# AbeelLab/phasm

Measured on AMD Instinct MI355X. Metric: overlaps_per_sec, higher is better.
Workload: dtype u64

## Files before the change

include/phasm_overlap.h:

```cpp
#ifndef PHASM_OVERLAP_H
#define PHASM_OVERLAP_H

#include <stddef.h>
#include <stdint.h>

#ifdef __cplusplus
extern "C" {
#endif

#define PO_ABI_VERSION 4

typedef enum {
    PO_OK = 0,
    PO_ERR_INVALID = 1,
    PO_ERR_NOMEM = 2,
    PO_ERR_HIP = 3,
    PO_ERR_CAPACITY = 4
} po_status;

typedef struct po_handle po_handle;
typedef struct po_result po_result;

typedef struct {
    uint32_t a_idx, b_idx;
// ... 192 lines not shown

typedef struct {
    uint64_t n_edges_in;
    uint64_t n_edges_out;
    uint64_t n_nodes;
    uint64_t n_nodes_removed;
    uint64_t n_candidates;
    uint64_t n_diamonds;
    uint64_t n_rounds;
    uint64_t n_invalid;
    float ms_setup, ms_rounds, ms_emit, ms_total;
} po_diamond_stats;

po_status po_layout_diamonds(po_handle* h, po_result* edges, const po_diamond_params* params, uint8_t* edge_flags_out,
                             po_result** kept_out);
po_status po_get_diamond_stats(const po_handle* h, po_diamond_stats* out);


typedef struct {
    uint32_t reserved;
} po_merge_params;

typedef struct {
    uint64_t n_edges_in;
    uint64_t n_edges_out;
    uint64_t n_nodes;
    uint64_t n_merged;
    uint64_t n_nodes_merged;
    uint64_t max_path_nodes;
    uint64_t n_self_loops;
    uint64_t n_cycle_nodes;
    uint64_t n_rounds;
    uint64_t n_overflow;
    uint64_t n_invalid;
    float ms_links, ms_rank, ms_number, ms_emit, ms_total;
} po_merge_stats;

po_status po_layout_merge(po_handle* h, po_result* edges, const po_merge_params* params, uint8_t* edge_flags_out,
                          po_result** merged_out);
po_status po_get_merge_stats(const po_handle* h, po_merge_stats* out);

po_status po_result_merged_paths(po_result* merged, uint64_t* n_paths, uint64_t* n_members, uint64_t* offsets_out,
                                 uint64_t cap_paths, uint32_t* members_out, int32_t* prefix_out, uint64_t cap_members,
                                 int64_t* lengths_out);


typedef struct {
    uint32_t reserved;
} po_coverage_params;

typedef struct {
    uint64_t read_length_sum;
    int64_t path_length;
} po_edge_coverage;

typedef struct {
    uint64_t n_rows, n_edges;
    uint64_t n_nodes;
    uint64_t n_pairs;
    uint64_t max_set;
    uint64_t n_zero_path;
    uint64_t n_invalid;
    float ms_sets, ms_edges, ms_total;
} po_coverage_stats;

po_status po_layout_coverage(po_handle* h, po_result* graph, po_result* rows, const po_coverage_params* params,
                             po_edge_coverage* coverage_out );
po_status po_get_coverage_stats(const po_handle* h, po_coverage_stats* out);


typedef struct {
    uint32_t reserved;
} po_components_params;

typedef struct {
    uint32_t first_node;
    uint32_t n_nodes;
    uint64_t n_edges;
} po_component;

typedef struct {
    uint64_t n_nodes;
    uint64_t n_edges;
    uint64_t n_components;
    uint64_t n_singletons;
    uint64_t max_component_nodes, max_component_edges;
    uint64_t n_invalid;
    uint32_t n_rounds;
    uint32_t n_batches;
    float ms_rounds, ms_label, ms_total;
} po_components_stats;

po_status po_layout_components(po_handle* h, po_result* graph, const po_components_params* params,
                               uint32_t* node_component_out, uint32_t* edge_component_out, po_component* components_out,
                               uint64_t* n_components_out);
po_status po_get_components_stats(const po_handle* h, po_components_stats* out);


typedef struct {
    uint32_t reserved;
} po_partition_params;

typedef struct {
    uint32_t first_node;
    uint32_t n_nodes;
    uint64_t n_edges;
    uint32_t n_r_in;
    uint32_t n_re_out;
} po_scc;

#define PO_PART_R_IN 1u
#define PO_PART_RE_OUT 2u
#define PO_PART_START 4u
#define PO_PART_SINK 8u

typedef struct {
    uint64_t n_nodes;
    uint64_t n_edges;
    uint64_t n_sccs, n_nonsingleton_sccs, n_singletons;
    uint64_t n_self_loops;
    uint64_t max_scc_nodes, max_scc_edges;
    uint64_t n_trimmed;
    uint64_t n_class[5];
    uint64_t n_invalid;
    uint32_t n_outer;
    uint32_t n_trim_rounds, n_forward_rounds, n_backward_rounds;
    uint32_t n_batches;
    float ms_ranks, ms_rounds, ms_label, ms_total;
} po_partition_stats;

po_status po_layout_partition(po_handle* h, po_result* graph, const po_partition_params* params, uint32_t* node_scc_out,
                              uint8_t* node_flags_out, uint8_t* edge_class_out, po_scc* sccs_out, uint64_t* n_sccs_out);
po_status po_get_partition_stats(const po_handle* h, po_partition_stats* out);

po_status po_graph_from_edges(po_handle* h, const po_edge* edges, uint64_t n_edges, const uint32_t* node_order,
                              uint64_t n_order, po_result** out);

po_status po_result_node_order(po_result* r, uint32_t* nodes_out, uint64_t cap, uint64_t* n_out);

typedef struct {
    uint64_t n_rows;
    float ms_first_contained;
    float ms_rank;
    float ms_total;
} po_node_order_stats;
po_status po_get_node_order_stats(const po_handle* h, po_node_order_stats* out);

uint64_t po_debug_host_ranges(uint64_t* out, uint64_t cap_entries);
uint64_t po_debug_store_words(const po_handle* h, int store, const uint64_t** words);
int po_debug_expand_records(const po_cand* records, uint64_t n, const uint32_t* lengths, uint32_t n_reads, uint32_t paired,
                            po_row* rows_out, uint64_t n_rows_expected);
int po_debug_expand_packed(const uint64_t* records, uint64_t n, uint32_t sh_b, uint32_t sh_p, const uint32_t* lengths, uint32_t n_reads,
                           uint32_t paired, po_row* rows_out, uint64_t n_rows_expected);
int po_debug_fault_backtrace(int fd);
int po_debug_pointer_info(const void* p, int32_t* hip_type, int32_t* hsa_type, uint64_t* base, uint64_t* bytes);

po_status po_get_stats(const po_handle* h, po_stats* out);
const char* po_last_error(const po_handle* h);
int po_abi_version(void);

#ifdef __cplusplus
}
#endif
#endif
```

phasm_amd/_lib.py:

```python
from __future__ import annotations

import ctypes
import os

import numpy as np

HERE = os.path.dirname(os.path.abspath(__file__))
LIB_PATH = os.environ.get("PHASM_LIB") or os.path.join(HERE, "libphasm_overlap.so")

PO_OK, PO_ERR_INVALID, PO_ERR_NOMEM, PO_ERR_HIP, PO_ERR_CAPACITY = range(5)

ROW_DTYPE = np.dtype([("a_idx", "<u4"), ("b_idx", "<u4"), ("astart", "<i4"),
                      ("aend", "<i4"), ("bstart", "<i4"), ("bend", "<i4")])


CAND_DTYPE = np.dtype([("a_idx", "<u4"), ("p", "<u4"), ("b_idx", "<u4"), ("type", "<u4")])


EDGE_DTYPE = np.dtype([("u", "<u4"), ("v", "<u4"), ("weight", "<i4"), ("overlap_len", "<i4")])
COVERAGE_DTYPE = np.dtype([("read_length_sum", "<u8"), ("path_length", "<i8")])
COMPONENT_DTYPE = np.dtype([("first_node", "<u4"), ("n_nodes", "<u4"), ("n_edges", "<u8")])
SCC_DTYPE = np.dtype([("first_node", "<u4"), ("n_nodes", "<u4"), ("n_edges", "<u8"), ("n_r_in", "<u4"), ("n_re_out", "<u4")])
PART_R_IN, PART_RE_OUT, PART_START, PART_SINK = 1, 2, 4, 8

# ... 85 lines not shown
    _fields_ = [("n_rows", ctypes.c_uint64), ("n_edges", ctypes.c_uint64), ("n_nodes", ctypes.c_uint64), ("n_pairs", ctypes.c_uint64),
                ("max_set", ctypes.c_uint64), ("n_zero_path", ctypes.c_uint64), ("n_invalid", ctypes.c_uint64),
                ("ms_sets", ctypes.c_float), ("ms_edges", ctypes.c_float), ("ms_total", ctypes.c_float)]

    def as_dict(self) -> dict:
        return {name: getattr(self, name) for name, _ in self._fields_}


class PoComponentsParams(ctypes.Structure):
    _fields_ = [("reserved", ctypes.c_uint32)]


class PoComponentsStats(ctypes.Structure):
    _fields_ = [("n_nodes", ctypes.c_uint64), ("n_edges", ctypes.c_uint64), ("n_components", ctypes.c_uint64),
                ("n_singletons", ctypes.c_uint64), ("max_component_nodes", ctypes.c_uint64), ("max_component_edges", ctypes.c_uint64),
                ("n_invalid", ctypes.c_uint64), ("n_rounds", ctypes.c_uint32), ("n_batches", ctypes.c_uint32),
                ("ms_rounds", ctypes.c_float), ("ms_label", ctypes.c_float), ("ms_total", ctypes.c_float)]

    def as_dict(self) -> dict:
        return {name: getattr(self, name) for name, _ in self._fields_}


class PoPartitionParams(ctypes.Structure):
    _fields_ = [("reserved", ctypes.c_uint32)]


class PoPartitionStats(ctypes.Structure):
    _fields_ = [("n_nodes", ctypes.c_uint64), ("n_edges", ctypes.c_uint64), ("n_sccs", ctypes.c_uint64),
                ("n_nonsingleton_sccs", ctypes.c_uint64), ("n_singletons", ctypes.c_uint64), ("n_self_loops", ctypes.c_uint64),
                ("max_scc_nodes", ctypes.c_uint64), ("max_scc_edges", ctypes.c_uint64), ("n_trimmed", ctypes.c_uint64),
                ("n_class", ctypes.c_uint64 * 5), ("n_invalid", ctypes.c_uint64), ("n_outer", ctypes.c_uint32),
                ("n_trim_rounds", ctypes.c_uint32), ("n_forward_rounds", ctypes.c_uint32), ("n_backward_rounds", ctypes.c_uint32),
                ("n_batches", ctypes.c_uint32),
                ("ms_ranks", ctypes.c_float), ("ms_rounds", ctypes.c_float), ("ms_label", ctypes.c_float), ("ms_total", ctypes.c_float)]

    def as_dict(self) -> dict:
        d = {name: getattr(self, name) for name, _ in self._fields_}
        d["n_class"] = list(self.n_class)
        return d


class PoNodeOrderStats(ctypes.Structure):
    _fields_ = [("n_rows", ctypes.c_uint64), ("ms_first_contained", ctypes.c_float), ("ms_rank", ctypes.c_float),
                ("ms_total", ctypes.c_float)]

    def as_dict(self) -> dict:
        return {name: getattr(self, name) for name, _ in self._fields_}


class PoStats(ctypes.Structure):
    _fields_ = [
        ("bits_per_base", ctypes.c_uint32), ("kmer", ctypes.c_uint32),
        ("paired", ctypes.c_uint32), ("wide_index", ctypes.c_uint32),
        ("n_reads", ctypes.c_uint64), ("n_eligible", ctypes.c_uint64),
        ("total_bases", ctypes.c_uint64), ("shard_bases", ctypes.c_uint64),
        ("n_tiles", ctypes.c_uint64), ("n_candidates", ctypes.c_uint64),
        ("n_verified", ctypes.c_uint64), ("n_rows", ctypes.c_uint64),
        ("sum_overlap_bases", ctypes.c_uint64), ("verify_bytes_algo", ctypes.c_uint64),
        ("ms_index", ctypes.c_float), ("ms_scan_count", ctypes.c_float),
        ("ms_scan_fill", ctypes.c_float), ("ms_verify", ctypes.c_float),
        ("ms_select", ctypes.c_float), ("ms_emit", ctypes.c_float),
        ("ms_total", ctypes.c_float), ("ms_upload", ctypes.c_float),
        ("ms_scan_probe", ctypes.c_float), ("ms_verify_kernel", ctypes.c_float),
        ("verify_bytes_exec", ctypes.c_uint64), ("dp_steps", ctypes.c_uint64), ("dp_stopped", ctypes.c_uint64),
        ("max_diff", ctypes.c_uint32), ("band", ctypes.c_uint32), ("index_reused", ctypes.c_uint32),
        ("dp_lanes", ctypes.c_uint32), ("upload_bytes", ctypes.c_uint64),
        ("streamed", ctypes.c_uint32), ("n_deferred", ctypes.c_uint32),
        ("fused_tail", ctypes.c_uint32), ("tail_fallback", ctypes.c_uint32),
        ("n_predicted", ctypes.c_uint32), ("home_record_bytes", ctypes.c_uint32),
    ]

    def as_dict(self) -> dict:
        return {name: getattr(self, name) for name, _ in self._fields_}


_P = ctypes.c_void_p
SYMBOLS = [
    ("po_abi_version", ctypes.c_int, []),
    ("po_create", ctypes.c_int, [ctypes.POINTER(_P)]),
    ("po_destroy", None, [_P]),
    ("po_set_device", ctypes.c_int, [_P, ctypes.c_int]),
    ("po_add_sequence", ctypes.c_int, [_P, ctypes.c_char_p, ctypes.c_size_t, ctypes.c_char_p, ctypes.c_size_t]),
    ("po_add_fasta", ctypes.c_int, [_P, ctypes.c_char_p, ctypes.c_int, ctypes.POINTER(ctypes.c_uint64)]),
    ("po_num_sequences", ctypes.c_uint32, [_P]),
    ("po_get_id", ctypes.c_int, [_P, ctypes.c_uint32, ctypes.POINTER(ctypes.c_void_p), ctypes.POINTER(ctypes.c_size_t)]),
    ("po_get_length", ctypes.c_uint32, [_P, ctypes.c_uint32]),
    ("po_upload", ctypes.c_int, [_P]),
    ("po_invalidate", ctypes.c_int, [_P]),
    ("po_upload_piece", ctypes.c_int, [_P, ctypes.c_uint32, ctypes.c_uint32, ctypes.c_void_p, ctypes.c_uint64,
                                       ctypes.POINTER(ctypes.c_uint64), ctypes.POINTER(ctypes.c_int)]),
    ("po_upload_assemble", ctypes.c_int, [_P, ctypes.c_void_p, ctypes.c_uint64, ctypes.c_uint32]),
    ("po_upload_piece_part", ctypes.c_int, [_P, ctypes.c_uint32, ctypes.c_uint32, ctypes.c_uint32, ctypes.c_uint32, ctypes.c_void_p,
                                            ctypes.c_uint64, ctypes.POINTER(ctypes.c_uint64), ctypes.POINTER(ctypes.c_int)]),
    ("po_upload_assemble_parts", ctypes.c_int, [_P, ctypes.c_void_p, ctypes.c_uint64, ctypes.c_uint32, ctypes.c_uint32]),
    ("po_overlaps", ctypes.c_int, [_P, ctypes.c_uint32, ctypes.POINTER(_P)]),
    ("po_overlaps_to_host", ctypes.c_int, [_P, ctypes.c_uint32, ctypes.POINTER(_P)]),
    ("po_overlaps_ex", ctypes.c_int, [_P, ctypes.c_uint32, ctypes.c_uint32, ctypes.c_uint32, ctypes.POINTER(_P)]),
    ("po_overlaps_shard", ctypes.c_int, [_P, ctypes.c_uint32, ctypes.c_uint32, ctypes.c_uint32, ctypes.POINTER(_P)]),
    ("po_candidates_shard", ctypes.c_int, [_P, ctypes.c_uint32, ctypes.c_uint32, ctypes.c_uint32, ctypes.POINTER(_P)]),
    ("po_expand", ctypes.c_int, [_P, ctypes.c_void_p, ctypes.c_uint64, ctypes.POINTER(_P)]),
    ("po_candidates_shard_into", ctypes.c_int, [_P, ctypes.c_uint32, ctypes.c_uint32, ctypes.c_uint32, ctypes.c_void_p,
                                               ctypes.c_uint64, ctypes.POINTER(ctypes.c_int), ctypes.POINTER(_P)]),
    ("po_index_slice_build", ctypes.c_int, [_P, ctypes.c_uint32, ctypes.c_uint32, ctypes.c_uint32, ctypes.POINTER(ctypes.c_uint32),
                                            ctypes.POINTER(ctypes.c_uint32), ctypes.POINTER(ctypes.c_uint64)]),
    ("po_index_chunk_bytes", ctypes.c_uint64, [ctypes.c_uint32, ctypes.c_uint64, ctypes.POINTER(ctypes.c_uint64)]),
    ("po_index_slice_export", ctypes.c_int, [_P, ctypes.c_void_p, ctypes.c_uint64]),
    ("po_candidates_shard_indexed", ctypes.c_int, [_P, ctypes.c_uint32, ctypes.c_uint32, ctypes.c_uint32, ctypes.c_void_p, ctypes.c_uint32,
                                                   ctypes.c_uint32, ctypes.c_uint64, ctypes.c_void_p, ctypes.c_uint64,
                                                   ctypes.POINTER(ctypes.c_int), ctypes.POINTER(_P)]),
    ("po_overlaps_shard_indexed", ctypes.c_int, [_P, ctypes.c_uint32, ctypes.c_uint32, ctypes.c_uint32, ctypes.c_void_p, ctypes.c_uint32,
                                                 ctypes.c_uint32, ctypes.c_uint64, ctypes.POINTER(_P)]),
    ("po_shard_range", ctypes.c_int, [_P, ctypes.c_uint32, ctypes.c_uint32, ctypes.POINTER(ctypes.c_uint32), ctypes.POINTER(ctypes.c_uint32)]),
    ("po_result_count", ctypes.c_uint64, [_P]),
    ("po_result_rows", ctypes.c_void_p, [_P]),
    ("po_result_rows_range", ctypes.c_void_p, [_P, ctypes.c_uint64, ctypes.c_uint64]),
    ("po_result_device_rows", ctypes.c_void_p, [_P]),
    ("po_result_copy_to_device", ctypes.c_int, [_P, ctypes.c_void_p]),
    ("po_result_copy_prefix_to_device", ctypes.c_int, [_P, ctypes.c_void_p, ctypes.c_uint64]),
    ("po_result_free", None, [_P]),
    ("po_write_gfa_edges", ctypes.c_int, [_P, ctypes.c_int, ctypes.POINTER(ctypes.c_uint64)]),
    ("po_write_gfa_segments", ctypes.c_int, [_P, ctypes.c_int, ctypes.POINTER(ctypes.c_uint64)]),
    ("po_add_segment", ctypes.c_int, [_P, ctypes.c_char_p, ctypes.c_size_t, ctypes.c_uint32]),
    ("po_result_from_rows", ctypes.c_int, [_P, ctypes.c_void_p, ctypes.c_uint64, ctypes.POINTER(_P)]),
    ("po_add_gfa", ctypes.c_int, [_P, ctypes.c_char_p, ctypes.POINTER(ctypes.c_uint64), ctypes.POINTER(_P)]),
    ("po_layout_edges", ctypes.c_int, [_P, _P, ctypes.POINTER(PoLayoutParams), ctypes.c_void_p, ctypes.POINTER(_P)]),
    ("po_get_layout_stats", ctypes.c_int, [_P, ctypes.POINTER(PoLayoutStats)]),
    ("po_layout_reduce", ctypes.c_int, [_P, _P, ctypes.POINTER(PoReduceParams), ctypes.c_void_p, ctypes.POINTER(_P)]),
    ("po_get_reduce_stats", ctypes.c_int, [_P, ctypes.POINTER(PoReduceStats)]),
    ("po_layout_tips", ctypes.c_int, [_P, _P, ctypes.POINTER(PoTipsParams), ctypes.c_void_p, ctypes.POINTER(_P)]),
    ("po_get_tips_stats", ctypes.c_int, [_P, ctypes.POINTER(PoTipsStats)]),
    ("po_layout_diamonds", ctypes.c_int, [_P, _P, ctypes.POINTER(PoDiamondParams), ctypes.c_void_p, ctypes.POINTER(_P)]),
    ("po_get_diamond_stats", ctypes.c_int, [_P, ctypes.POINTER(PoDiamondStats)]),
    ("po_layout_merge", ctypes.c_int, [_P, _P, ctypes.POINTER(PoMergeParams), ctypes.c_void_p, ctypes.POINTER(_P)]),
    ("po_get_merge_stats", ctypes.c_int, [_P, ctypes.POINTER(PoMergeStats)]),
    ("po_result_merged_paths", ctypes.c_int, [_P, ctypes.POINTER(ctypes.c_uint64), ctypes.POINTER(ctypes.c_uint64), ctypes.c_void_p,
                                              ctypes.c_uint64, ctypes.c_void_p, ctypes.c_void_p, ctypes.c_uint64, ctypes.c_void_p]),
    ("po_layout_coverage", ctypes.c_int, [_P, _P, _P, ctypes.POINTER(PoCoverageParams), ctypes.c_void_p]),
    ("po_get_coverage_stats", ctypes.c_int, [_P, ctypes.POINTER(PoCoverageStats)]),
    ("po_layout_components", ctypes.c_int, [_P, _P, ctypes.POINTER(PoComponentsParams), ctypes.c_void_p, ctypes.c_void_p, ctypes.c_void_p,
                                            ctypes.POINTER(ctypes.c_uint64)]),
    ("po_get_components_stats", ctypes.c_int, [_P, ctypes.POINTER(PoComponentsStats)]),
    ("po_layout_partition", ctypes.c_int, [_P, _P, ctypes.POINTER(PoPartitionParams), ctypes.c_void_p, ctypes.c_void_p, ctypes.c_void_p,
                                           ctypes.c_void_p, ctypes.POINTER(ctypes.c_uint64)]),
    ("po_get_partition_stats", ctypes.c_int, [_P, ctypes.POINTER(PoPartitionStats)]),
    ("po_graph_from_edges", ctypes.c_int, [_P, ctypes.c_void_p, ctypes.c_uint64, ctypes.c_void_p, ctypes.c_uint64, ctypes.POINTER(_P)]),
    ("po_result_node_order", ctypes.c_int, [_P, ctypes.c_void_p, ctypes.c_uint64, ctypes.POINTER(ctypes.c_uint64)]),
    ("po_get_node_order_stats", ctypes.c_int, [_P, ctypes.POINTER(PoNodeOrderStats)]),
    ("po_get_stats", ctypes.c_int, [_P, ctypes.POINTER(PoStats)]),
    ("po_last_error", ctypes.c_char_p, [_P]),
    ("po_debug_fault_backtrace", ctypes.c_int, [ctypes.c_int]),
    ("po_debug_store_words", ctypes.c_uint64, [_P, ctypes.c_int, ctypes.POINTER(ctypes.c_void_p)]),
    ("po_debug_expand_packed", ctypes.c_int, [ctypes.c_void_p, ctypes.c_uint64, ctypes.c_uint32, ctypes.c_uint32, ctypes.c_void_p, ctypes.c_uint32,
                                              ctypes.c_uint32, ctypes.c_void_p, ctypes.c_uint64]),
    ("po_debug_expand_records", ctypes.c_int, [ctypes.c_void_p, ctypes.c_uint64, ctypes.c_void_p, ctypes.c_uint32, ctypes.c_uint32,
                                               ctypes.c_void_p, ctypes.c_uint64]),
    ("po_debug_host_ranges", ctypes.c_uint64, [ctypes.POINTER(ctypes.c_uint64), ctypes.c_uint64]),
    ("po_debug_pointer_info", ctypes.c_int, [ctypes.c_void_p, ctypes.POINTER(ctypes.c_int32), ctypes.POINTER(ctypes.c_int32),
                                             ctypes.POINTER(ctypes.c_uint64), ctypes.POINTER(ctypes.c_uint64)]),
]

_lib = None


def _preload_torch_hip_runtime() -> None:
    import importlib.util
    if os.environ.get("PHASM_HIP_RUNTIME") == "system":
        return
    try:
        spec = importlib.util.find_spec("torch")
    except (ImportError, ValueError):
        spec = None
    if spec is None or not spec.submodule_search_locations:
        return
    path = os.path.join(list(spec.submodule_search_locations)[0], "lib", "libamdhip64.so")
    if os.path.exists(path):
        try:
            ctypes.CDLL(path, mode=ctypes.RTLD_GLOBAL)
        except OSError:
            pass


def load() -> ctypes.CDLL:
    global _lib
    if _lib is None:
        _preload_torch_hip_runtime()
        if not os.path.exists(LIB_PATH):
            raise ImportError(
                "%s not found: build it with `python -m phasm_amd.build` (hipcc, gfx950). "
                "phasm_amd has no CPU fallback." % LIB_PATH)
        lib = ctypes.CDLL(LIB_PATH)
        for name, restype, argtypes in SYMBOLS:
            fn = getattr(lib, name)
            fn.restype = restype
            fn.argtypes = argtypes
        _lib = lib
    return _lib
```

phasm_amd/csrc/c_api.hip:

```cpp
#include "../../include/phasm_overlap.h"

#include <hip/hip_runtime.h>

#include <dlfcn.h>
#include <execinfo.h>
#include <fcntl.h>
#include <signal.h>
#include <sys/mman.h>
#include <sys/stat.h>
#include <unistd.h>

#include <algorithm>
#include <array>
#include <atomic>
#include <chrono>
#include <cmath>
#include <condition_variable>
#include <cstdio>
#include <cstdlib>
#include <cstring>
#include <deque>
#include <functional>
#include <memory>
#include <mutex>
#include <new>
#include <string>
#include <system_error>
#include <thread>
#include <unordered_map>
#include <vector>

#include "kernels.hip.h"
#include "extend.hip.h"
#include "layout.hip.h"
#include "reduce.hip.h"
#include "tips.hip.h"
#include "diamond.hip.h"
#include "merge.hip.h"
#include "coverage.hip.h"
#include "components.hip.h"
#include "partition.hip.h"

namespace {

enum { RB_CNT, RB_DEG, RB_OFF, RB_CUR, RB_TKEY, RB_TTGT, RB_TEID, RB_CTGT, RB_CW, RB_CEID, RB_CIDPOS, RB_STGT, RB_SEID, RB_STATE,
       RB_FLAG1, RB_FLAGS, RB_KEEP, RB_KOFF, RB_N };
enum { TB_CNT, TB_OUTDEG, TB_OUTSUM, TB_INDEG, TB_INSUM, TB_MARK, TB_CAND, TB_CSTATE, TB_EFLAG, TB_FLAGS, TB_KEEP, TB_KOFF,
       TB_TKEY, TB_TVAL, TB_ALIVE, TB_RCNT, TB_N };
enum { MB_CNT, MB_RCNT, MB_OUTDEG, MB_INDEG, MB_OUTE, MB_INE, MB_LINK, MB_BACK, MB_JB0, MB_JB1, MB_HOPS0, MB_HOPS1, MB_WS0, MB_WS1,
       MB_HKEY, MB_HVAL, MB_HLEN, MB_HSUM, MB_PATHK, MB_LENS, MB_PSUM, MB_NPATH, MB_NPOS, MB_EFLAG, MB_KEEP, MB_KOFF, MB_TMP, MB_LEN,
       MB_N };
enum { VB_CNT, VB_USED, VB_NODEOF, VB_LEN, VB_TABLE, VB_SUM, VB_SETCNT, VB_OFF, VB_CUR, VB_LIST, VB_OUT, VB_N };
enum { RK_CNT, RK_RCNT, RK_KEY, RK_VAL, RK_RANKOF, RK_ENDS, RK_ROOT, RK_INDEX, RK_N };
enum { KB_P, KB_COMP, KB_ECOMP, KB_TABLE, KB_N };
enum { PB_LIVE, PB_SCC, PB_COLOUR, PB_MARK, PB_HASIN, PB_HASOUT, PB_NODESCC, PB_FLAGW, PB_FLAGS, PB_ECLASS, PB_TABLE, PB_N };
constexpr int EV_LAY_N = 38;
enum { EV_EDGES = 0, EV_REDUCE = 4, EV_TIPS = 9, EV_NODE_ORDER = 15, EV_DIAMONDS = 18, EV_MERGE = 22, EV_COVERAGE = 27, EV_COMPONENTS = 30,
       EV_PARTITION = 34 };
static_assert(EV_PARTITION + 4 == EV_LAY_N, "the four events of po_layout_partition are the last of the layout events");
constexpr int TIP_BATCH = 24;

struct DevBuf {
    void* p = nullptr;
    size_t cap = 0;
    bool arena = false;
    template <typename T> T* as() const { return static_cast<T*>(p); }
    void release() {
        if (p && !arena) (void)hipFree(p);
        p = nullptr;
        cap = 0;
        arena = false;
    }
};

struct PinNote {
    uint64_t base, bytes;
    uint32_t kind;
};
std::mutex g_pin_mu;
std::vector<PinNote> g_pins;
uint64_t g_pins_ever = 0;
constexpr size_t PIN_LOG_MAX = 1u << 16;
void pin_note(const void* p, size_t bytes, uint32_t kind) {
    if (!p) return;
    std::lock_guard<std::mutex> lock(g_pin_mu);
    ++g_pins_ever;
    for (PinNote& n : g_pins)
        if (n.base == (uint64_t)(uintptr_t)p && n.bytes == bytes && (n.kind & 0xFFu) == kind) {
            n.kind |= 0x100u;
            return;
        }
    if (g_pins.size() < PIN_LOG_MAX) g_pins.push_back(PinNote{(uint64_t)(uintptr_t)p, (uint64_t)bytes, kind | 0x100u});
}
void pin_drop(const void* p) {
    if (!p) return;
    std::lock_guard<std::mutex> lock(g_pin_mu);
    for (PinNote& n : g_pins)
        if (n.base == (uint64_t)(uintptr_t)p && (n.kind & 0x100u)) n.kind &= ~0x100u;
}

struct HostBuf {
    void* p = nullptr;
    size_t cap = 0;
    void release() {
        if (p) {
            pin_drop(p);
            (void)hipHostFree(p);
        }
        p = nullptr;
        cap = 0;
    }
};

inline int phase_events_env() {
    if (const char* e = getenv("PHASM_PHASE_EVENTS")) {
        const int v = atoi(e);
        return v == 1 ? 1 : v == 2 ? 2 : 0;
    }
    return getenv("PHASM_STREAM_TRACE") ? 1 : -1;
}
enum { EV_START = 0, EV_INDEX, EV_COUNT, EV_FILL, EV_VERIFY, EV_SELECT, EV_EMIT, EV_PROBE0, EV_PROBE1, EV_VER0, EV_VER1, EV_DONE, EV_N };

}

constexpr int PO_MAX_PIECES = 16;

struct RegHeader {
    size_t bytes;
    int registered;
};
constexpr size_t REG_PAGE = 4096;
thread_local bool g_reg_defer = false;
template <class T>
struct RegAlloc {
    using value_type = T;
    RegAlloc() = default;
    template <class U> RegAlloc(const RegAlloc<U>&) {}
    T* allocate(size_t n) {
        const size_t bytes = ((n * sizeof(T) + REG_PAGE - 1) / REG_PAGE) * REG_PAGE;
        void* base = nullptr;
        if (posix_memalign(&base, REG_PAGE, bytes + REG_PAGE) != 0 || !base) throw std::bad_alloc();
        RegHeader* hd = static_cast<RegHeader*>(base);
        hd->bytes = bytes;
        hd->registered = 0;
        char* data = static_cast<char*>(base) + REG_PAGE;
        if (getenv("PHASM_POISON_HOST")) std::memset(data, 0xA5, bytes);
        if (!g_reg_defer) reg_now(data);
        return reinterpret_cast<T*>(data);
    }
    static void reg_now(void* data) {
        RegHeader* hd = reinterpret_cast<RegHeader*>(static_cast<char*>(data) - REG_PAGE);
        if (hd->registered || hd->bytes < (1u << 20) || getenv("PHASM_NO_PIN")) return;
        if (hipHostRegister(data, hd->bytes, hipHostRegisterPortable) == hipSuccess) {
            hd->registered = 1;
            pin_note(data, hd->bytes, 2u);
        } else {
            (void)hipGetLastError();
        }
    }
    template <class U> void construct(U*) noexcept {}
    template <class U, class A0, class... Args> void construct(U* q, A0&& a0, Args&&... args) {
        ::new (static_cast<void*>(q)) U(std::forward<A0>(a0), std::forward<Args>(args)...);
    }
    void deallocate(T* p, size_t) {
        char* base = reinterpret_cast<char*>(p) - REG_PAGE;
        RegHeader* hd = reinterpret_cast<RegHeader*>(base);
        if (hd->registered) {
            pin_drop(p);
            (void)hipHostUnregister(p);
        }
        free(base);
    }
    template <class U> bool operator==(const RegAlloc<U>&) const { return true; }
    template <class U> bool operator!=(const RegAlloc<U>&) const { return false; }
};
using WordStore = std::vector<uint64_t, RegAlloc<uint64_t>>;
inline bool store_is_pinned(const WordStore& w) {
    if (w.capacity() == 0) return false;
    const RegHeader* hd = reinterpret_cast<const RegHeader*>(reinterpret_cast<const char*>(w.data()) - REG_PAGE);
    return hd->registered != 0;
}
constexpr size_t STAGE_MAX = 4u << 20;

struct po_handle {
    int device = 0;
// ... 251 lines not shown
        return fail(h, PO_ERR_NOMEM, "hipMalloc(" + std::to_string(want) + " bytes): " + hipGetErrorString(e));
    }
    b.cap = want;
    if (h && h->poison >= 0 && h->stream) (void)hipMemsetAsync(b.p, h->poison, want, h->stream);
    return PO_OK;
}

po_status ensure_piece(po_handle* h, DevBuf& b, size_t bytes) { return ensure(h, b, bytes, h->ws_scale); }

po_status ensure_host(po_handle* h, HostBuf& b, size_t bytes) {
    if (bytes <= b.cap) return PO_OK;
    AllocTrace tr("hipHostMalloc", bytes);
    b.release();
    const size_t want = bytes + bytes / 16 + 4096;
    hipError_t e = hipHostMalloc(&b.p, want, hipHostMallocDefault);
    if (e != hipSuccess) {
        b.p = nullptr;
        return fail(h, PO_ERR_NOMEM, "hipHostMalloc(" + std::to_string(want) + " bytes): " + hipGetErrorString(e));
    }
    b.cap = want;
    pin_note(b.p, want, 1u);
    return PO_OK;
}

void quiesce_store(po_handle* h) {
    if (!h->dev_ready) return;
    (void)hipSetDevice(h->device);
    (void)hipStreamSynchronize(h->stream);
    if (h->up_stream) (void)hipStreamSynchronize(h->up_stream);
    if (h->rc_stream) (void)hipStreamSynchronize(h->rc_stream);
}

po_status init_device(po_handle* h);

inline bool home_enabled() {
    const char* e = getenv("PHASM_HOME");
    return !(e && atoi(e) == 0);
}

void result_pool_grow(po_handle* h, uint64_t bases = 0) {
    if (!bases) bases = h->total_bases;
    h->pool_bases = bases + bases / 2;
    if (getenv("PHASM_NO_POOL")) return;
    if (!h->dev_ready && init_device(h) != PO_OK) h->err.clear();
    const uint64_t want = std::min<uint64_t>(h->pool_bases / 160 * sizeof(po_row), 4ull << 30);
    if (h->spare_host.cap >= want || h->live_results) return;
    int n = 0;
    if (hipGetDeviceCount(&n) != hipSuccess || n == 0) {
        (void)hipGetLastError();
        h->pool_bases = ~0ull;
        return;
    }
    AllocTrace tr("result pool", want);
    h->spare_host.release();
    if (hipHostMalloc(&h->spare_host.p, want, hipHostMallocPortable) == hipSuccess) {
        h->spare_host.cap = want;
        pin_note(h->spare_host.p, want, 1u);
        if (home_enabled() && h->home_stage.cap < want / 3) (void)ensure_host(h, h->home_stage, want / 3);
        if (h->dev_ready && h->up_stream && h->copy_stream && want >= (16u << 20) && !getenv("PHASM_NO_WARM")) {
            void* w = nullptr;
            const size_t nb = 8u << 20;
            if (hipMalloc(&w, nb) == hipSuccess) {
                (void)hipMemcpyAsync(w, h->spare_host.p, nb, hipMemcpyHostToDevice, h->up_stream);
                (void)hipStreamSynchronize(h->up_stream);
                (void)hipMemcpyAsync(static_cast<char*>(h->spare_host.p) + nb, w, nb, hipMemcpyDeviceToHost, h->copy_stream);
                (void)hipStreamSynchronize(h->copy_stream);
                (void)hipFree(w);
            }
            (void)hipGetLastError();
        }
    } else {
        (void)hipGetLastError();
        h->spare_host.p = nullptr;
        h->pool_bases = ~0ull;
    }
}

#define PO_TRY(expr)                    \
    do {                                \
        po_status s_ = (expr);          \
        if (s_ != PO_OK) return s_;     \
    } while (0)

struct DevKit {
    int device = -1;
    hipStream_t stream = nullptr, copy_stream = nullptr, up_stream = nullptr, rc_stream = nullptr;
    hipEvent_t ev_sets[2][EV_N] = {};
    hipEvent_t ev_up0 = nullptr, ev_up1 = nullptr, ev_meta = nullptr, ev_first = nullptr;
    hipEvent_t ev_piece[PO_MAX_PIECES] = {}, ev_rc[PO_MAX_PIECES] = {}, ev_lay[EV_LAY_N] = {};

    uint64_t* pinned = nullptr;
    uint64_t* pinned_dev = nullptr;
};
static_assert(sizeof(DevKit::ev_lay) == sizeof(po_handle::ev_lay), "a kit carries every layout event of a handle");
std::mutex g_kit_mu;
std::vector<DevKit> g_kits;
constexpr size_t KIT_POOL_MAX = 8;

bool kit_take(po_handle* h) {
    std::lock_guard<std::mutex> lock(g_kit_mu);
    for (size_t i = 0; i < g_kits.size(); ++i) {
        if (g_kits[i].device != h->device) continue;
        const DevKit k = g_kits[i];
        g_kits.erase(g_kits.begin() + (long)i);
        h->stream = k.stream;
        h->copy_stream = k.copy_stream;
        h->up_stream = k.up_stream;
        h->rc_stream = k.rc_stream;
        std::memcpy(h->ev_sets, k.ev_sets, sizeof(k.ev_sets));
        h->ev_up0 = k.ev_up0;
        h->ev_up1 = k.ev_up1;
        h->ev_meta = k.ev_meta;
        h->ev_first = k.ev_first;
        std::memcpy(h->ev_piece, k.ev_piece, sizeof(k.ev_piece));
        std::memcpy(h->ev_rc, k.ev_rc, sizeof(k.ev_rc));
        std::memcpy(h->ev_lay, k.ev_lay, sizeof(k.ev_lay));
        h->pinned = k.pinned;
        h->pinned_dev = k.pinned_dev;
        return true;
    }
    return false;
}

bool kit_give(po_handle* h) {
    if (getenv("PHASM_NO_KIT_POOL") || !h->stream || !h->copy_stream || !h->up_stream || !h->rc_stream || !h->pinned) return false;
    if (hipStreamSynchronize(h->stream) != hipSuccess || hipStreamSynchronize(h->copy_stream) != hipSuccess ||
        hipStreamSynchronize(h->up_stream) != hipSuccess || hipStreamSynchronize(h->rc_stream) != hipSuccess) {
        (void)hipGetLastError();
        return false;
    }
    DevKit k;
    k.device = h->device;
    k.stream = h->stream;
    k.copy_stream = h->copy_stream;
    k.up_stream = h->up_stream;
    k.rc_stream = h->rc_stream;
    std::memcpy(k.ev_sets, h->ev_sets, sizeof(k.ev_sets));
    k.ev_up0 = h->ev_up0;
    k.ev_up1 = h->ev_up1;
    k.ev_meta = h->ev_meta;
    k.ev_first = h->ev_first;
    std::memcpy(k.ev_piece, h->ev_piece, sizeof(k.ev_piece));
    std::memcpy(k.ev_rc, h->ev_rc, sizeof(k.ev_rc));
    std::memcpy(k.ev_lay, h->ev_lay, sizeof(k.ev_lay));
    k.pinned = h->pinned;
    k.pinned_dev = h->pinned_dev;
    std::lock_guard<std::mutex> lock(g_kit_mu);
    if (g_kits.size() >= KIT_POOL_MAX) return false;
    g_kits.push_back(k);
    return true;
}


unsigned cpu_share() {
    static const unsigned share = [] {
        unsigned n = std::thread::hardware_concurrency();
        n = n ? n : 4u;
        long long q = -1, per = 100000;
        if (FILE* f = std::fopen("/sys/fs/cgroup/cpu.max", "r")) {
            char buf[64] = {0};
            if (std::fscanf(f, "%63s %lld", buf, &per) >= 1 && std::strcmp(buf, "max") != 0) q = atoll(buf);
            std::fclose(f);
        } else if (FILE* g = std::fopen("/sys/fs/cgroup/cpu/cpu.cfs_quota_us", "r")) {
            if (std::fscanf(g, "%lld", &q) != 1) q = -1;
            std::fclose(g);
            if (FILE* g2 = std::fopen("/sys/fs/cgroup/cpu/cpu.cfs_period_us", "r")) {
                if (std::fscanf(g2, "%lld", &per) != 1) per = 100000;
                std::fclose(g2);
            }
        }
        if (q > 0 && per > 0) n = std::min<unsigned>(n, (unsigned)std::max<long long>(1, q / per));
        return n;
    }();
    return share;
}

namespace home {

constexpr uint32_t CHUNK = 4096;

struct Job {
    const void* rec = nullptr;
    uint32_t sh_b = 0, sh_p = 0;
    uint64_t n_rec = 0;
    po_row* out = nullptr;
    uint64_t n_rows = 0;
    const volatile uint32_t* flag = nullptr;
    uint32_t want = 0;
    uint32_t paired = 0, bits = 2;
};

struct Pool {
    std::vector<std::thread> thr;
    std::mutex mu;
    std::condition_variable cv_queue;
    std::condition_variable cv_job;
    std::mutex call_mu;
    std::deque<Job> queue;
    std::atomic<uint64_t> submitted{0}, finished{0};
    std::atomic<int> error{0};
    const uint32_t* len = nullptr;
    uint32_t n_reads = 0;
    std::atomic<uint64_t> sum_l{0}, sum_b{0}, sum_e{0};
    Job cur;
    uint64_t job_seq = 0;
    uint32_t n_chunks = 0;
    std::vector<uint64_t> chunk_off;
    std::atomic<uint32_t> next_count{0}, done_count{0}, next_write{0}, done_write{0};
    std::atomic<int> phase{0};
    std::atomic<int> inside{0};
    std::chrono::steady_clock::time_point t0;
    std::vector<std::array<double, 3>> trace;
    bool tracing = false;
};

Pool* g_pool = nullptr;
std::once_flag g_pool_once;

inline void cpu_pause() {
#if defined(__x86_64__) || defined(__i386__)
    __builtin_ia32_pause();
#endif
}

std::atomic<uint32_t> g_spin_limit{4096};
template <class Pred>
inline void spin_until(Pred pred) {
    const uint32_t limit = g_spin_limit.load(std::memory_order_relaxed);
    for (uint32_t n = 0; !pred(); ++n) {
        if (limit == 0 || n < limit) cpu_pause();
        else std::this_thread::yield();
    }
}

inline po::Cand load_rec(const Job& j, uint64_t i) {
    if (!j.sh_b) return static_cast<const po::Cand*>(j.rec)[i];
    return po::unpack_record(static_cast<const uint64_t*>(j.rec)[i], j.sh_b, j.sh_p);
}

inline uint32_t rows_of_rec(const po::Cand& c, uint32_t paired) {
    if (!paired) return (c.type & 1u) + ((c.type >> 1) & 1u);
    return ((c.type & 1u) ? (c.a == (c.b ^ 1u) ? 1u : 2u) : 0u) + ((c.type & 2u) ? 2u : 0u);
}

inline void put_row(uint64_t*& o, uint32_t a, uint32_t b, uint32_t astart, uint32_t aend, uint32_t bend) {
    __builtin_nontemporal_store((uint64_t)a | ((uint64_t)b << 32), o);
    __builtin_nontemporal_store((uint64_t)astart | ((uint64_t)aend << 32), o + 1);
    __builtin_nontemporal_store((uint64_t)bend << 32, o + 2);
    o += 3;
}

bool expand_records(Pool& P, uint64_t lo, uint64_t hi, po_row* out) {
    uint64_t* o = reinterpret_cast<uint64_t*>(out);
    const Job& job = P.cur;
    const uint32_t* len = P.len;
    const uint32_t paired = job.paired, n_reads = P.n_reads, bits = job.bits;
    auto pb = [bits](uint32_t l) -> uint64_t { return bits == 8u ? l : (l >> 2) + ((l & 3u) != 0u); };
    uint64_t sl = 0, sb = 0, se = 0;
    for (uint64_t i = lo; i < hi; ++i) {
        const po::Cand c = load_rec(job, i);
        if (c.a >= n_reads || c.b >= n_reads) return false;
        const uint32_t la = len[c.a], lb = len[c.b];
        se += 2 * pb((c.type & 1u) ? la - c.p : lb);
        if (c.type & 1u) {
            const uint32_t l = la - c.p;
            const bool twin = paired && c.a != (c.b ^ 1u);
            put_row(o, c.a, c.b, c.p, la, l);
            if (twin) put_row(o, c.b ^ 1u, c.a ^ 1u, lb - l, lb, l);
            const uint64_t k = twin ? 2 : 1;
            sl += k * l;
            sb += k * 2 * pb(l);
        }
        if (c.type & 2u) {
            put_row(o, c.a, c.b, c.p, c.p + lb, lb);
            if (paired) put_row(o, c.a ^ 1u, c.b ^ 1u, la - c.p - lb, la - c.p, lb);
            const uint64_t k = paired ? 2 : 1;
            sl += k * lb;
            sb += k * 2 * pb(lb);
        }
    }
    P.sum_l.fetch_add(sl, std::memory_order_relaxed);
    P.sum_b.fetch_add(sb, std::memory_order_relaxed);
    P.sum_e.fetch_add(se, std::memory_order_relaxed);
    return true;
}

void run_phases(Pool& P, bool lead) {
    const uint32_t nc = P.n_chunks;
    for (;;) {
        const uint32_t c = P.next_count.fetch_add(1, std::memory_order_relaxed);
        if (c >= nc) break;
        const uint64_t lo = (uint64_t)c * CHUNK, hi = std::min<uint64_t>(P.cur.n_rec, lo + CHUNK);
        uint64_t n = 0;
        const uint32_t paired = P.cur.paired;
        for (uint64_t i = lo; i < hi; ++i) n += rows_of_rec(load_rec(P.cur, i), paired);
        P.chunk_off[c + 1] = n;
        P.done_count.fetch_add(1, std::memory_order_release);
    }
    if (lead) {
        spin_until([&] { return P.done_count.load(std::memory_order_acquire) >= nc; });
        P.chunk_off[0] = 0;
        for (uint32_t c = 0; c < nc; ++c) P.chunk_off[c + 1] += P.chunk_off[c];
        if (P.chunk_off[nc] != P.cur.n_rows) P.error.store(1);
        P.phase.store(P.error.load() ? 0 : 2, std::memory_order_release);
    } else {
        spin_until([&] { return P.phase.load(std::memory_order_acquire) != 1; });
    }
    if (P.phase.load(std::memory_order_acquire) != 2) return;
    for (;;) {
        const uint32_t c = P.next_write.fetch_add(1, std::memory_order_relaxed);
        if (c >= nc) break;
        const uint64_t lo = (uint64_t)c * CHUNK, hi = std::min<uint64_t>(P.cur.n_rec, lo + CHUNK);
        if (!expand_records(P, lo, hi, P.cur.out + P.chunk_off[c])) P.error.store(2);
#if defined(__x86_64__)
        __builtin_ia32_sfence();
#endif
        P.done_write.fetch_add(1, std::memory_order_release);
    }
}

void helper(Pool* Pp) {
    Pool& P = *Pp;
    uint64_t seen = 0;
    for (;;) {
        {
            std::unique_lock<std::mutex> lock(P.mu);
            P.cv_job.wait(lock, [&] { return P.job_seq != seen; });
            seen = P.job_seq;
        }
        P.inside.fetch_add(1, std::memory_order_acq_rel);
        if (P.phase.load(std::memory_order_acquire) != 0) run_phases(P, false);
        P.inside.fetch_sub(1, std::memory_order_release);
    }
}

void leader(Pool* Pp) {
    Pool& P = *Pp;
    for (;;) {
        Job j;
        {
            std::unique_lock<std::mutex> lock(P.mu);
            P.cv_queue.wait(lock, [&] { return !P.queue.empty(); });
            j = P.queue.front();
            P.queue.pop_front();
        }
        if (j.flag)
            spin_until([&] { return *j.flag == j.want; });
        std::atomic_thread_fence(std::memory_order_acquire);
        const double t_ready = P.tracing ? std::chrono::duration<double, std::micro>(std::chrono::steady_clock::now() - P.t0).count() : 0.0;
        if (P.error.load() == 0 && j.n_rec) {
            spin_until([&] { return P.inside.load(std::memory_order_acquire) == 0; });
            P.cur = j;
            P.n_chunks = (uint32_t)((j.n_rec + CHUNK - 1) / CHUNK);
            if (P.chunk_off.size() < (size_t)P.n_chunks + 1) P.chunk_off.resize((size_t)P.n_chunks + 1);
            P.next_count.store(0);
            P.done_count.store(0);
            P.next_write.store(0);
            P.done_write.store(0);
            P.phase.store(1, std::memory_order_release);
            {
                std::lock_guard<std::mutex> lock(P.mu);
                ++P.job_seq;
            }
            P.cv_job.notify_all();
            run_phases(P, true);
            if (P.phase.load() == 2)
                spin_until([&] { return P.done_write.load(std::memory_order_acquire) >= P.n_chunks; });
            P.phase.store(0, std::memory_order_release);
            std::atomic_thread_fence(std::memory_order_seq_cst);
        }
        if (P.tracing)
            P.trace.push_back({t_ready, std::chrono::duration<double, std::micro>(std::chrono::steady_clock::now() - P.t0).count(), (double)j.n_rows});
        P.finished.fetch_add(1, std::memory_order_release);
    }
}

Pool* pool() {
    std::call_once(g_pool_once, [] {
        Pool* P = new Pool();
        unsigned n = cpu_share();
        n = std::max(1u, std::min(n * 3 / 4, 12u));
        if (const char* e = getenv("PHASM_HOME_THREADS")) n = (unsigned)std::max(1, std::min(64, atoi(e)));
        try {
            P->thr.emplace_back(leader, P);
            P->thr.back().detach();
            for (unsigned i = 1; i < n; ++i) {
                P->thr.emplace_back(helper, P);
                P->thr.back().detach();
            }
        } catch (const std::system_error&) {
        }
        if (P->thr.empty()) {
            delete P;
            P = nullptr;
        }
        g_pool = P;
    });
    return g_pool;
}

void begin(Pool* P, const uint32_t* len, uint32_t n_reads, bool tracing) {
    if (const char* e = getenv("PHASM_HOME_SPIN")) g_spin_limit.store((uint32_t)std::max(0, atoi(e)));
    else g_spin_limit.store(4096);
    P->len = len;
    P->n_reads = n_reads;
    P->error.store(0);
    P->submitted.store(0);
    P->finished.store(0);
    P->sum_l.store(0);
    P->sum_b.store(0);
    P->sum_e.store(0);
    P->tracing = tracing;
    P->trace.clear();
    P->t0 = std::chrono::steady_clock::now();
}

void submit(Pool* P, const Job& j) {
    {
        std::lock_guard<std::mutex> lock(P->mu);
        P->queue.push_back(j);
    }
    P->submitted.fetch_add(1, std::memory_order_release);
    P->cv_queue.notify_one();
}

void wait_all(Pool* P) {
    spin_until([&] { return P->finished.load(std::memory_order_acquire) >= P->submitted.load(std::memory_order_acquire); });
}

}

po_status init_device(po_handle* h) {
    if (h->dev_ready) {
        HIP_TRY(h, hipSetDevice(h->device));
        return PO_OK;
    }
    AllocTrace tr("init_device", 0);
    const auto ti0 = std::chrono::steady_clock::now();
    auto imark = [&](const char* what) {
        if (tr.on) std::fprintf(stderr, "[init] %s at %.1f ms\n", what, std::chrono::duration<double, std::milli>(std::chrono::steady_clock::now() - ti0).count());
    };
    int n = 0;
    hipError_t e = hipGetDeviceCount(&n);
    imark("runtime up (hipGetDeviceCount)");
    if (e != hipSuccess || n == 0)
        return fail(h, PO_ERR_HIP, "no HIP device available (libphasm_overlap has no CPU fallback)");
    if (h->device < 0 || h->device >= n) return fail(h, PO_ERR_INVALID, "device ordinal out of range");
    HIP_TRY(h, hipSetDevice(h->device));
    hipDeviceProp_t prop;
    HIP_TRY(h, hipGetDeviceProperties(&prop, h->device));
    h->n_cu = prop.multiProcessorCount > 0 ? prop.multiProcessorCount : 256;
    h->lds_max = prop.sharedMemPerBlock;
    if (const char* e = getenv("PHASM_POISON")) h->poison = (int)(strtol(e, nullptr, 0) & 0xFF);
    if (!getenv("PHASM_NO_KIT_POOL") && kit_take(h)) {
        h->ev = h->ev_sets[0];
        std::memset(h->pinned, 0, 1024);
        hipLaunchKernelGGL(po::k_fill_u32, dim3(1), dim3(64), 0, h->stream, reinterpret_cast<uint32_t*>(h->pinned_dev + 63), (uint64_t)1, 0u);
        (void)hipGetLastError();
        h->dev_ready = true;
        return PO_OK;
    }
    imark("device selected, properties read");
    HIP_TRY(h, hipStreamCreateWithFlags(&h->stream, hipStreamNonBlocking));
    imark("first stream made");
    for (int i = 0; i < 2 * EV_N; ++i) HIP_TRY(h, hipEventCreate(&h->ev_sets[i / EV_N][i % EV_N]));
    HIP_TRY(h, hipEventCreate(&h->ev_up0));
    HIP_TRY(h, hipEventCreate(&h->ev_up1));
    imark("first events made");
    HIP_TRY(h, hipHostMalloc(reinterpret_cast<void**>(&h->pinned), 1024, hipHostMallocDefault));
    pin_note(h->pinned, 1024, 1u);
    HIP_TRY(h, hipHostGetDevicePointer(reinterpret_cast<void**>(&h->pinned_dev), h->pinned, 0));
    imark("landing zone made");
    if (const char* e = getenv("PHASM_POISON")) h->poison = (int)(strtol(e, nullptr, 0) & 0xFF);
    HIP_TRY(h, hipStreamCreateWithFlags(&h->copy_stream, hipStreamNonBlocking));
    imark("copy stream made");
    HIP_TRY(h, hipStreamCreateWithFlags(&h->up_stream, hipStreamNonBlocking));
    HIP_TRY(h, hipStreamCreateWithFlags(&h->rc_stream, hipStreamNonBlocking));
    imark("other streams made");
    for (int k = 0; k < PO_MAX_PIECES; ++k) {
        HIP_TRY(h, hipEventCreate(&h->ev_piece[k]));
        HIP_TRY(h, hipEventCreateWithFlags(&h->ev_rc[k], hipEventDisableTiming));
    }
    HIP_TRY(h, hipEventCreateWithFlags(&h->ev_first, hipEventDisableTiming));
    HIP_TRY(h, hipEventCreateWithFlags(&h->ev_meta, hipEventDisableTiming));
    imark("streams and events made");
    hipLaunchKernelGGL(po::k_fill_u32, dim3(1), dim3(64), 0, h->stream, reinterpret_cast<uint32_t*>(h->pinned_dev + 63), (uint64_t)1, 0u);
    (void)hipGetLastError();
    imark("first launch queued (code object loaded)");
    if (!getenv("PHASM_NO_WARM")) {
        void* w = nullptr;
        if (hipMalloc(&w, 256) == hipSuccess) {
            uint32_t* wd = static_cast<uint32_t*>(w);
            (void)hipMemcpyAsync(wd, h->pinned + 62, 8, hipMemcpyHostToDevice, h->up_stream);
            hipLaunchKernelGGL(po::k_fill_u32, dim3(1), dim3(64), 0, h->up_stream, wd + 8, (uint64_t)1, 0u);
            (void)hipMemcpyAsync(wd + 16, h->pinned + 62, 8, hipMemcpyHostToDevice, h->stream);
            hipLaunchKernelGGL(po::k_fill_u32, dim3(1), dim3(64), 0, h->rc_stream, wd + 24, (uint64_t)1, 0u);
            hipLaunchKernelGGL(po::k_fill_u32, dim3(1), dim3(64), 0, h->copy_stream, wd + 32, (uint64_t)1, 0u);
            (void)hipMemcpyAsync(h->pinned + 61, wd + 32, 8, hipMemcpyDeviceToHost, h->copy_stream);
            (void)hipMemcpyAsync(h->pinned + 60, wd + 16, 8, hipMemcpyDeviceToHost, h->stream);
            (void)hipStreamSynchronize(h->up_stream);
            (void)hipStreamSynchronize(h->rc_stream);
            (void)hipStreamSynchronize(h->copy_stream);
            (void)hipStreamSynchronize(h->stream);
            (void)hipFree(w);
        }
        (void)hipGetLastError();
        imark("queues and copy paths warmed");
        static const void* const warm_kernels[] = {
            (const void*)po::k_abs_woff, (const void*)po::k_build_tiles, (const void*)po::k_revcomp_store, (const void*)po::k_scatter_first,
            (const void*)po::k_paired_check, (const void*)po::k_call_init, (const void*)po::k_call_reset, (const void*)po::k_table_insert,
            (const void*)po::k_chain_fill, (const void*)po::k_chain_sort_short<uint32_t>, (const void*)po::k_chain_sort_long<uint32_t>,
            (const void*)po::k_table_finalize, (const void*)po::k_ps_reduce<uint32_t>, (const void*)po::k_ps_spine, (const void*)po::k_ps_down<uint32_t>,
            (const void*)po::k_ps_reduce<uint8_t>, (const void*)po::k_ps_down<uint8_t>, (const void*)po::k_ps_chain<uint32_t>,
            (const void*)po::k_ps_chain<uint8_t>, (const void*)po::k_ps_small,
            (const void*)po::k_scan_probe<2, true, true>, (const void*)po::k_scan_probe<2, true, false>, (const void*)po::k_scan_fixup<2, true>,
            (const void*)po::k_scan_fixup<2, false>, (const void*)po::k_scan_fill<2, true>, (const void*)po::k_scan_fill<2, false>,
            (const void*)po::k_read_label, (const void*)po::k_read_sort, (const void*)po::k_read_invert, (const void*)po::k_defer_split,
            (const void*)po::k_verify_a<2, false, true, true>, (const void*)po::k_verify_a<2, false, true, false>,
            (const void*)po::k_verify_a<2, true, true, false>, (const void*)po::k_select_local, (const void*)po::k_tile_rows<true>,
            (const void*)po::k_tile_rows<false>, (const void*)po::k_tail, (const void*)po::k_tail_cands, (const void*)po::k_select,
            (const void*)po::k_emit, (const void*)po::k_verify_flat, (const void*)po::k_deferred_rowcnt, (const void*)po::k_emit_cands,
            (const void*)po::k_wide_insert<2, 1>, (const void*)po::k_wide_insert<2, 16>, (const void*)po::k_wide_chain_fill<2, 1>,
            (const void*)po::k_wide_chain_fill<2, 16>, (const void*)po::k_wide_finalize<2, 1>, (const void*)po::k_wide_finalize<2, 16>,
            (const void*)po::k_chain_sort_short<uint64_t>, (const void*)po::k_chain_sort_long<uint64_t>,
            (const void*)po::k_wide_scan<2, false, true, 1>, (const void*)po::k_wide_scan<2, true, true, 1>,
            (const void*)po::k_wide_scan<2, false, false, 16>, (const void*)po::k_wide_scan<2, true, false, 16>};
        for (const void* k : warm_kernels) {
            hipFuncAttributes fa;
            (void)hipFuncGetAttributes(&fa, k);
        }
        (void)hipGetLastError();
        imark("kernels looked up");
    }
    h->dev_ready = true;
    return PO_OK;
}

struct BaseLut {
    uint8_t v[256];
    BaseLut() {
        std::memset(v, 0x80, sizeof(v));
        v[(unsigned char)'A'] = 0;
        v[(unsigned char)'C'] = 1;
        v[(unsigned char)'G'] = 2;
        v[(unsigned char)'T'] = 3;
    }
};
const BaseLut g_lut;

bool append_packed(po_handle* h, const unsigned char* s, size_t n, int bits) {
    const size_t per = 64 / bits;
    WordStore& store = h->words[h->woff.size() & 1];
    const size_t old_size = store.size();
    const size_t off = (old_size + 1) & ~size_t(1);
    const size_t nw = (n + per - 1) / per;
    store.resize(off + nw + 1, 0);
    uint64_t* w = store.data() + off;
    if (bits == 2) {
        const uint8_t* lut = g_lut.v;
        uint8_t bad = 0;
        const size_t full = n / 32;
        for (size_t k = 0; k < full; ++k) {
            const unsigned char* q = s + k * 32;
            uint64_t acc = 0;
            for (int j = 0; j < 32; ++j) {
                const uint8_t c = lut[q[j]];
                bad |= c;
                acc |= (uint64_t)(c & 3) << (2 * j);
            }
            w[k] = acc;
        }
        if (full * 32 < n) {
            uint64_t acc = 0;
            for (size_t i = full * 32; i < n; ++i) {
                const uint8_t c = lut[s[i]];
                bad |= c;
                acc |= (uint64_t)(c & 3) << (2 * (i & 31));
            }
            w[full] = acc;
        }
        if (bad & 0x80) {
            size_t cnt = 0;
            for (size_t i = 0; i < n; ++i) cnt += lut[s[i]] >> 7;
// ... 684 lines not shown
        h->sl_entries = h->pinned[0];
        if (h->phase_events) (void)hipEventElapsedTime(&S.ms_index, h->ev[EV_START], h->ev[EV_INDEX]);
        return PO_OK;
    }
    if (ext_idx) {
        WA_ext = true;
    }
    if (h->idx_only) {
        h->idx_valid = true;
        h->idx_gen = h->upload_gen;
        h->idx_m = m;
        h->idx_wide = wide;
        h->idx_tbits = tbits;
        h->idx_bits = (uint32_t)BITS;
        h->idx_ww = ww;
        return PO_OK;
    }
    h->idx_valid = !ext_idx;
    h->idx_gen = h->upload_gen;
    h->idx_m = m;
    h->idx_wide = wide;
    h->idx_tbits = tbits;
    h->idx_bits = (uint32_t)BITS;
    h->idx_ww = ww;

    po::ScanArgs A = {};
    A.words = words;
    A.tiles = h->d_tiles.as<po::TileRec>();
    A.tile_begin = tile_begin;
    A.tile_end = tile_end;
    A.m = m;
    A.kmask = kmask;
    A.bloom = bloom;
    A.bloom_log2 = bloom_log2;
    A.table = table;
    A.tbits = tbits;
    A.chain = chain;
    A.len = len;
    A.paired = paired;
    A.selfrep = selfrep;
    A.n_selfrep = reinterpret_cast<uint32_t*>(scalars + 2);
    A.tile_count = h->d_tile_count.as<uint32_t>();
    A.tile_off = tile_off_p;
    A.truemask = h->d_truemask.as<uint32_t>();
#ifdef PO_STAMPS
    PO_TRY(ensure(h, h->d_flag, (size_t)4096 * 64));
    HIP_TRY(h, hipMemsetAsync(h->d_flag.p, 0, (size_t)4096 * 64, st));
    A.dbg = h->d_flag.as<unsigned long long>();
#endif
    uint32_t scan_waves = po::SCAN_BLOCK / 64;
    if (const char* e = getenv("PHASM_SCAN_WAVES")) scan_waves = std::max(1, std::min(16, atoi(e)));
    const uint32_t scan_grid = std::max<uint32_t>(1, std::min<uint32_t>((uint32_t)h->n_cu, cdiv(ntiles, scan_waves)));
    po::WideArgs WA = {};
    WA.words = words;
    WA.tiles = A.tiles;
    WA.tile_begin = tile_begin;
    WA.tile_end = tile_end;
    WA.m = m;
    WA.table = table;
    WA.tbits = tbits;
    WA.chain = h->d_chain.as<uint64_t>();
    WA.n_slices = 1;
    if (WA_ext) {
        WA.table = static_cast<const po::Slot*>(h->ext_index);
        WA.chain = nullptr;
        WA.n_slices = h->ext_slices;
        WA.chunk_slots = h->ext_chunk_slots;
        WA.chain_off_slots = h->ext_chain_off;
    }
    WA.len = len;
    WA.paired = paired;
    WA.tile_count = A.tile_count;
    WA.lane_slot = A.truemask;
    WA.tile_off = A.tile_off;
    if (wide) {
        if (h->pair_events) HIP_TRY(h, hipEventRecord(h->ev[EV_PROBE0], st));
        auto wscan = streamed ? (ww == 4 ? po::k_wide_scan<BITS, false, BITS == 2, 4> : po::k_wide_scan<BITS, false, BITS == 2, 1>)
                     : ww == 16 ? po::k_wide_scan<BITS, false, false, 16> : ww == 4 ? po::k_wide_scan<BITS, false, false, 4> : po::k_wide_scan<BITS, false, false, 1>;
        hipLaunchKernelGGL(wscan, dim3(cdiv(ntiles, 4)), dim3(256), 0, st, WA, po::CandGuard{nullptr, 0u});
        if (h->pair_events) HIP_TRY(h, hipEventRecord(h->ev[EV_PROBE1], st));
    } else {
        const size_t scan_lds = (size_t)scan_waves * po::SCAN_LDS_PER_WAVE + bloom_bytes;
        if (scan_lds > h->lds_max) return fail(h, PO_ERR_HIP, "device LDS too small for the scan kernel");
        constexpr bool CAN_STREAM = BITS == 2;
        auto probe_full = streamed ? po::k_scan_probe<BITS, true, CAN_STREAM> : po::k_scan_probe<BITS, true, false>;
        auto probe_part = streamed ? po::k_scan_probe<BITS, false, CAN_STREAM> : po::k_scan_probe<BITS, false, false>;
        HIP_TRY(h, hipFuncSetAttribute(reinterpret_cast<const void*>(probe_full), hipFuncAttributeMaxDynamicSharedMemorySize, (int)scan_lds));
        HIP_TRY(h, hipFuncSetAttribute(reinterpret_cast<const void*>(probe_part), hipFuncAttributeMaxDynamicSharedMemorySize, (int)scan_lds));
        const uint32_t n_scan_waves = scan_grid * scan_waves;
        PO_TRY(ensure(h, h->d_left, (size_t)n_scan_waves * po::LEFT_CAP * sizeof(uint2)));
        PO_TRY(ensure(h, h->d_left_cnt, (size_t)n_scan_waves * 4));
        PO_TRY(ensure(h, h->d_tile_extra, ((size_t)h->n_tiles + 1) * 4));
        self_clean = streamed && !getenv("PHASM_DEBUG_LEFT") && !getenv("PHASM_PIECE_RESET");
        if (fold_clear && self_clean && h->st_selfclean) {
        } else if (fold_clear) {
            const uint32_t te0 = self_clean ? 0u : tile_begin, ten = self_clean ? h->n_tiles : ntiles;
            hipLaunchKernelGGL(po::k_call_reset, dim3(cdiv(std::max(std::max(n, 16u), std::max(n_scan_waves, ten)), 256)), dim3(256), 0, st,
                               selfrep, n, self_clean ? h->d_scalars.as<unsigned long long>() : scalars, self_clean ? 16u : 8u,
                               h->d_left_cnt.as<uint32_t>(), n_scan_waves, h->d_tile_extra.as<uint32_t>() + te0, ten);
        } else {
            HIP_TRY(h, hipMemsetAsync(h->d_left_cnt.p, 0, (size_t)n_scan_waves * 4, st));
            HIP_TRY(h, hipMemsetAsync(h->d_tile_extra.as<uint32_t>() + tile_begin, 0, (size_t)ntiles * 4, st));
        }
        A.left = h->d_left.as<uint2>();
        A.left_cnt = h->d_left_cnt.as<uint32_t>();
        A.tile_extra = h->d_tile_extra.as<uint32_t>();
        if (h->pair_events) HIP_TRY(h, hipEventRecord(h->ev[EV_PROBE0], st));
        hipLaunchKernelGGL(K == W ? probe_full : probe_part, dim3(scan_grid), dim3(scan_waves * 64), scan_lds, st, A);
        if (h->pair_events) HIP_TRY(h, hipEventRecord(h->ev[EV_PROBE1], st));
        auto fixup = streamed ? po::k_scan_fixup<BITS, CAN_STREAM> : po::k_scan_fixup<BITS, false>;
        hipLaunchKernelGGL(fixup, dim3(n_scan_waves), dim3(256), 0, st, A, n_scan_waves, self_clean ? 1u : 0u);
        if (getenv("PHASM_DEBUG_LEFT")) {
            PO_TRY(ensure_host(h, h->scratch_host, (size_t)n_scan_waves * 4));
            HIP_TRY(h, hipMemcpyAsync(h->scratch_host.p, h->d_left_cnt.p, (size_t)n_scan_waves * 4, hipMemcpyDeviceToHost, st));
            HIP_TRY(h, hipStreamSynchronize(st));
            const uint32_t* lc = static_cast<const uint32_t*>(h->scratch_host.p);
            uint64_t sum = 0;
            uint32_t mx = 0;
            for (uint32_t k = 0; k < n_scan_waves; ++k) sum += lc[k], mx = std::max(mx, lc[k]);
            std::fprintf(stderr, "[left] %u scan waves deferred %llu positions (max %u per wave, cap %d)\n", n_scan_waves,
                         (unsigned long long)sum, mx, (int)po::LEFT_CAP);
        }
    }
    HIP_TRY(h, hipGetLastError());
#ifdef PO_STAMPS
    if (!wide) {
        std::vector<unsigned long long> dbg(4096 * 8);
        HIP_TRY(h, hipMemcpyAsync(dbg.data(), h->d_flag.p, dbg.size() * 8, hipMemcpyDeviceToHost, st));
        HIP_TRY(h, hipStreamSynchronize(st));
        double sum[6] = {0, 0, 0, 0, 0, 0};
        for (size_t w = 0; w < 4096; ++w) for (int k = 0; k < 6; ++k) sum[k] += (double)dbg[w * 8 + k];
        if (sum[5] > 0)
            std::fprintf(stderr, "[stamps] per pass (cycles): wait_rw %.0f  filter %.0f  wait_probe %.0f  consume %.0f  issue %.0f  (passes %.0f)\n",
                         sum[0] / sum[5], sum[1] / sum[5], sum[2] / sum[5], sum[3] / sum[5], sum[4] / sum[5], sum[5]);
    }
#endif
    const int zone = 64 + 16 * (int)(shard & 1u);
    uint32_t cap_c = 0;
    bool async_count = false, pred_order = true;
    if (streamed && h->st_harvest && h->st_pred_valid && !dp && !want_cands && !getenv("PHASM_SYNC_COUNT") && !getenv("PHASM_TAIL_CLASSIC")) {
        uint64_t pred = h->st_pred_cand[shard];
        uint64_t cap = pred + pred / 50 + 256;
        if (const char* e = getenv("PHASM_PRED_SCALE")) cap = pred = (uint64_t)((double)pred * atof(e));
        const uint64_t worst = cap * 4u;
        bool order = pred >= 400000 && (r_end - r_begin) >= 4096;
        if (const char* e = getenv("PHASM_VERIFY_ORDER")) order = atoi(e) != 0;
        pred_order = order;
        auto fits = [](const DevBuf& b, uint64_t bytes) { return b.p && b.cap >= bytes; };
        async_count = pred > 0 && cap < (16u << 20) && cdiv(cap, po::TAIL_TILE) <= po::TAIL_MAX_TILES &&
                      fits(h->d_cand_a, cap * 4) && fits(h->d_cand_p, cap * 4) && fits(h->d_cand_b, cap * 4) && fits(h->d_type, cap) &&
                      fits(h->d_rowcnt, cap) && fits(h->d_row_off, (cap + 1) * 4) &&
                      fits(h->spare_rows, h->home_on ? cap * sizeof(po::Cand) : worst * sizeof(po_row)) &&
                      (!order || (fits(h->d_vlabel, (uint64_t)(r_end - r_begin) * 4) && fits(h->d_vperm, (uint64_t)(r_end - r_begin) * 4) &&
                                  fits(h->d_vrank, (uint64_t)(r_end - r_begin) * 4))) && h->dev_words < 0xFFFFFFF0ull;
        cap_c = (uint32_t)cap;
    }
    volatile uint64_t* count_slot = async_count ? &h->pinned[zone + 8] : &h->pinned[1];
    volatile uint64_t* also_slot = async_count ? &h->pinned[zone + 9] : &h->pinned[8];
    if (ntiles <= po::PS_SMALL_MAX) {
        PO_TRY(prefix_sum_small(h, A.tile_count + tile_begin, wide ? nullptr : A.tile_extra + tile_begin, ntiles,
                                tile_off_p + tile_begin, count_slot,
                                reinterpret_cast<const uint64_t*>(scalars + 2), also_slot, st, reinterpret_cast<uint64_t*>(scalars)));
    } else {
        PO_TRY(prefix_sum<uint32_t>(h, A.tile_count + tile_begin, ntiles, tile_off_p + tile_begin, count_slot,
                                    reinterpret_cast<const uint64_t*>(scalars + 2), also_slot,
                                    wide ? nullptr : A.tile_extra + tile_begin, st, reinterpret_cast<uint64_t*>(scalars)));
    }
    if (h->phase_events) HIP_TRY(h, hipEventRecord(h->ev[EV_COUNT], st));
    po::CandGuard G = {nullptr, 0u};
    uint64_t n_cand64;
    uint32_t n_selfrep_reads;
    if (async_count) {
        n_cand64 = cap_c;
        n_selfrep_reads = 0;
        S.n_predicted = 1;
        G.n_dev = scalars;
        G.cap = cap_c;
    } else {
        if (h->st_pend.valid && h->st_harvest) {
            HIP_TRY(h, hipEventSynchronize(h->st_pend.ev[EV_DONE]));
            PO_TRY(h->st_harvest());
        }
        HIP_TRY(h, hipStreamSynchronize(st));
        n_cand64 = h->pinned[1];
        n_selfrep_reads = (uint32_t)h->pinned[8];
    }
    if (nshards > 1 || streamed || wide || dpE) n_selfrep_reads |= 1u;
    S.n_candidates = n_cand64;
    if (n_cand64 >= 0xFFFFFF00ull)
        return fail(h, PO_ERR_CAPACITY, "candidate count " + std::to_string(n_cand64) + " exceeds one call's capacity (2^32)");
    const uint32_t n_cand = (uint32_t)n_cand64;

    uint64_t n_rows64 = 0;
    po::PairSlot* ptab = nullptr;
    uint32_t pbits = 0;
    uint32_t* n_deferred = reinterpret_cast<uint32_t*>(scalars + 1) + 1;
    const uint32_t* gate = nullptr;
    const uint64_t worst_rows = (uint64_t)n_cand * (paired ? 4u : 2u);
    std::function<po_status()> classic_tail;
    const bool sel_in_verify = (nshards > 1 || streamed || wide) && !dp && !getenv("PHASM_SELECT_KERNEL");
    if (n_cand) {
        PO_TRY(ensure_piece(h, h->d_cand_a, (size_t)n_cand * 4));
        PO_TRY(ensure_piece(h, h->d_cand_p, (size_t)n_cand * 4));
        PO_TRY(ensure_piece(h, h->d_cand_b, (size_t)n_cand * 4));
        PO_TRY(ensure_piece(h, h->d_type, (size_t)n_cand));
        PO_TRY(ensure_piece(h, h->d_rowcnt, (size_t)n_cand));
        PO_TRY(ensure_piece(h, h->d_row_off, ((size_t)n_cand + 1) * 4));
        A.cand_a = h->d_cand_a.as<uint32_t>();
        A.cand_p = h->d_cand_p.as<uint32_t>();
        A.cand_b = h->d_cand_b.as<uint32_t>();
        if (wide) {
            WA.cand_a = A.cand_a;
            WA.cand_p = A.cand_p;
            WA.cand_b = A.cand_b;
            auto wfill = streamed ? (ww == 4 ? po::k_wide_scan<BITS, true, BITS == 2, 4> : po::k_wide_scan<BITS, true, BITS == 2, 1>)
                         : ww == 16 ? po::k_wide_scan<BITS, true, false, 16> : ww == 4 ? po::k_wide_scan<BITS, true, false, 4> : po::k_wide_scan<BITS, true, false, 1>;
            hipLaunchKernelGGL(wfill, dim3(cdiv(ntiles, 4)), dim3(256), 0, st, WA, G);
        } else {
            auto fill = streamed ? po::k_scan_fill<BITS, BITS == 2> : po::k_scan_fill<BITS, false>;
            hipLaunchKernelGGL(fill, dim3(cdiv(ntiles, 4 * po::FILL_TILES)), dim3(256), 0, st, A, G);
        }
        const bool use_order_early = [&]() {
            bool u = n_cand >= 400000 && (r_end - r_begin) >= 4096;
            if (const char* e = getenv("PHASM_VERIFY_ORDER")) u = atoi(e) != 0;
            if (async_count) u = pred_order;
            return u && !dp;
        }();
        const bool defer_needed = streamed && r_end < n;
        if (defer_needed && !use_order_early) {
            hipLaunchKernelGGL(po::k_defer_split, dim3(cdiv(n_cand, 256)), dim3(256), 0, st, A.cand_a, A.cand_p, A.cand_b, n_cand,
                               r_end, h->d_defer.as<po::Cand>(), h->st_defer_cap, h->d_defer.as<uint32_t>() + (size_t)h->st_defer_cap * 4, G);
        }
        HIP_TRY(h, hipGetLastError());
        if (h->phase_events) HIP_TRY(h, hipEventRecord(h->ev[EV_FILL], st));
        if (dp) {
            if (2ull * h->max_len + 64ull >= (1ull << 30))
                return fail(h, PO_ERR_CAPACITY, "po_overlaps_ex: reads of 2^29 bases or more are beyond the DP kernel");
            PO_TRY(ensure(h, h->d_end_a, (size_t)n_cand * 4));
            PO_TRY(ensure(h, h->d_end_b, (size_t)n_cand * 4));
            PO_TRY(ensure(h, h->d_dpcnt, 64));
            HIP_TRY(h, hipMemsetAsync(h->d_dpcnt.p, 0, 64, st));
            po::ExtArgs X = {};
            X.words = words;
            X.woff = woff;
            X.len = len;
            X.cand_a = A.cand_a;
            X.cand_p = A.cand_p;
            X.cand_b = A.cand_b;
            X.n_cand = n_cand;
            X.max_diff = dpE;
            X.band = dpW;
            X.paired = paired;
            X.exc_off = h->n_exc_uploaded ? h->d_exc_off.as<uint32_t>() : nullptr;
            X.exc_pos = h->d_exc_pos.as<uint32_t>();
            X.exc_byte = h->d_exc_byte.as<uint8_t>();
            X.type = h->d_type.as<uint8_t>();
            X.end_a = h->d_end_a.as<uint32_t>();
            X.end_b = h->d_end_b.as<uint32_t>();
            X.counters = h->d_dpcnt.as<unsigned long long>();
            bool lanes = BITS == 2 && dpW <= 15;
            bool bitvec = lanes;
            if (const char* e = getenv("PHASM_DP_KERNEL")) {
                if (!strcmp(e, "wave")) lanes = bitvec = false;
                if (!strcmp(e, "lanes")) bitvec = false;
                if ((!strcmp(e, "lanes") || !strcmp(e, "bits")) && !(BITS == 2 && dpW <= 15))
                    return fail(h, PO_ERR_INVALID, "PHASM_DP_KERNEL=lanes|bits needs 2-bit reads and band <= 15");
            }
            if (const char* e = getenv("PHASM_DP_KERNEL_SOFT"))
                if (!strcmp(e, "lanes")) bitvec = false;
            S.dp_lanes = bitvec ? 2u : lanes ? 1u : 0u;
            if (h->pair_events) HIP_TRY(h, hipEventRecord(h->ev[EV_VER0], st));
            if (lanes) {
                const uint32_t* perm = nullptr;
                bool sorted = n_cand >= 4096;
                if (const char* e = getenv("PHASM_DP_SORT")) sorted = atoi(e) != 0;
                if (sorted) {
                    const uint32_t max_bins = (uint32_t)((std::min<size_t>(h->lds_max, 160 * 1024) - 1024) / 4);
                    const uint32_t max_rows = h->max_len + dpW;
                    uint32_t shift = 0;
                    while ((max_rows >> shift) + 1 > max_bins) ++shift;
                    const uint32_t n_bins = (max_rows >> shift) + 1;
                    const size_t sort_lds = ((size_t)n_bins + po::SORT_BLOCK / 64) * 4;
                    PO_TRY(ensure(h, h->d_vlabel, (size_t)n_cand * 4));
                    PO_TRY(ensure(h, h->d_vrank, (size_t)n_cand * 4));
                    PO_TRY(ensure(h, h->d_vperm, (size_t)n_cand * 4));
                    hipLaunchKernelGGL(po::k_dp_rows, dim3(cdiv(n_cand, 256)), dim3(256), 0, st, A.cand_a, A.cand_p, A.cand_b, len, n_cand,
                                       dpW, h->d_vlabel.as<uint32_t>());
                    if (sort_lds > 48 * 1024)
                        HIP_TRY(h, hipFuncSetAttribute(reinterpret_cast<const void*>(po::k_read_sort),
                                                       hipFuncAttributeMaxDynamicSharedMemorySize, (int)sort_lds));
                    hipLaunchKernelGGL(po::k_read_sort, dim3(1), dim3(po::SORT_BLOCK), sort_lds, st, h->d_vlabel.as<uint32_t>(), n_cand,
                                       shift, n_bins, h->d_vrank.as<uint32_t>());
                    hipLaunchKernelGGL(po::k_read_invert, dim3(cdiv(n_cand, 256)), dim3(256), 0, st, h->d_vrank.as<uint32_t>(), n_cand, 0u,
                                       h->d_vperm.as<uint32_t>());
                    perm = h->d_vperm.as<uint32_t>();
                }
                auto kern = bitvec ? po::k_extend_bits : dpW <= 4 ? po::k_extend_lanes<4> : dpW <= 8 ? po::k_extend_lanes<8> : po::k_extend_lanes<15>;
                hipLaunchKernelGGL(kern, dim3(cdiv(n_cand, 256)), dim3(256), 0, st, X, perm);
            } else {
                hipLaunchKernelGGL((po::k_extend_dp<BITS>), dim3(cdiv(n_cand, 256 / po::WAVE)), dim3(256), 0, st, X);
            }
            if (h->pair_events) HIP_TRY(h, hipEventRecord(h->ev[EV_VER1], st));
            HIP_TRY(h, hipMemcpyAsync(h->pinned + 32, h->d_dpcnt.p, 16, hipMemcpyDeviceToHost, st));
            ver_timed = true;
        } else {
            const uint64_t need_words = ((uint64_t)h->max_len + W - 1) / W + 3;
            const uint32_t lds_words_raw = (uint32_t)std::min<uint64_t>(need_words, 8192 - 1100);
            const uint32_t n_a = r_end - r_begin;
            const uint32_t* perm = nullptr;
            const bool use_order = use_order_early;
            if (use_order) {
                const uint32_t max_bins = (uint32_t)((std::min<size_t>(h->lds_max, 160 * 1024) - 1024) / 4);
                uint32_t shift = 0, n_bins;
                while ((n >> shift) + 1 > max_bins) ++shift;
                n_bins = (n >> shift) + 1;
                const size_t sort_lds = ((size_t)n_bins + po::SORT_BLOCK / 64) * 4;
                PO_TRY(ensure(h, h->d_vlabel, (size_t)n_a * 4));
                PO_TRY(ensure(h, h->d_vperm, (size_t)n_a * 4));
                po::DeferOut dfo = {};
                if (defer_needed) {
                    dfo.cand_p = A.cand_p;
                    dfo.b_limit = r_end;
                    dfo.list = h->d_defer.as<uint4>();
                    dfo.cap = h->st_defer_cap;
                    dfo.counter = h->d_defer.as<uint32_t>() + (size_t)h->st_defer_cap * 4;
                }
                hipLaunchKernelGGL(po::k_read_label, dim3(cdiv((uint64_t)n_a * 16, 256)), dim3(256), 0, st,
                                   h->d_read_tile0.as<uint32_t>(), tile_off_p, A.cand_b, r_begin, n_a, paired,
                                   h->d_vlabel.as<uint32_t>(), dfo, G);
                if (sort_lds > 48 * 1024)
                    HIP_TRY(h, hipFuncSetAttribute(reinterpret_cast<const void*>(po::k_read_sort),
                                                   hipFuncAttributeMaxDynamicSharedMemorySize, (int)sort_lds));
                PO_TRY(ensure(h, h->d_vrank, (size_t)n_a * 4));
                hipLaunchKernelGGL(po::k_read_sort, dim3(1), dim3(po::SORT_BLOCK), sort_lds, st, h->d_vlabel.as<uint32_t>(), n_a,
                                   shift, n_bins, h->d_vrank.as<uint32_t>());
                hipLaunchKernelGGL(po::k_read_invert, dim3(cdiv(n_a, 256)), dim3(256), 0, st, h->d_vrank.as<uint32_t>(), n_a, r_begin,
                                   h->d_vperm.as<uint32_t>());
                perm = h->d_vperm.as<uint32_t>();
            }
            const uint32_t ver_grid = perm ? 8 * ((n_a + 7) / 8) : n_a;
            bool staged = h->dev_words < 0xFFFFFFF0ull;
            if (const char* e = getenv("PHASM_VERIFY_STAGED")) staged = staged && atoi(e) != 0;
            auto verify = paired == 2u ? (staged ? po::k_verify_a<BITS, true, true> : po::k_verify_a<BITS, true, false>)
                                       : (staged ? po::k_verify_a<BITS, false, true> : po::k_verify_a<BITS, false, false>);
            if (streamed) verify = staged ? po::k_verify_a<BITS, false, true, BITS == 2> : po::k_verify_a<BITS, false, false, BITS == 2>;
            const uint32_t lds_words = (lds_words_raw + 1u) & ~1u;
            const size_t ver_lds = (size_t)lds_words * 8 + (size_t)po::VREC_CAP * sizeof(po::VRec) + 16;
            if (ver_lds > 48 * 1024)
                HIP_TRY(h, hipFuncSetAttribute(reinterpret_cast<const void*>(verify), hipFuncAttributeMaxDynamicSharedMemorySize, (int)ver_lds));
            if (h->pair_events) HIP_TRY(h, hipEventRecord(h->ev[EV_VER0], st));
            hipLaunchKernelGGL(verify, dim3(ver_grid), dim3(po::VER_BLOCK), ver_lds, st,
                               words, woff, len, h->d_read_tile0.as<uint32_t>(), tile_off_p, A.cand_p,
                               A.cand_b, r_begin, lds_words, paired_ver,
                               h->n_exc_uploaded ? h->d_exc_off.as<uint32_t>() : nullptr, h->d_exc_pos.as<uint32_t>(),
                               h->d_exc_byte.as<uint8_t>(), h->d_type.as<uint8_t>(), perm, n_a, G,
                               sel_in_verify ? selfrep : nullptr, sel_in_verify ? n_deferred : nullptr);
            if (h->pair_events) HIP_TRY(h, hipEventRecord(h->ev[EV_VER1], st));
            ver_timed = true;
        }
        HIP_TRY(h, hipGetLastError());
#ifdef PO_VSTAMPS
        {
            unsigned long long v[64 * 8], z[64 * 8] = {};
            HIP_TRY(h, hipStreamSynchronize(st));
            HIP_TRY(h, hipMemcpyFromSymbol(v, HIP_SYMBOL(po::g_vstamps), sizeof(v)));
            HIP_TRY(h, hipMemcpyToSymbol(HIP_SYMBOL(po::g_vstamps), z, sizeof(z)));
            double sum[8] = {};
            for (int i = 0; i < 64; ++i) for (int k = 0; k < 8; ++k) sum[k] += (double)v[i * 8 + k];
            if (sum[6] > 0)
                std::fprintf(stderr, "[vstamps] per wave (shader clocks): setup %.0f  wait_b %.0f  lds+cmp %.0f  book+init %.0f  life %.0f | iterations %.1f  group-steps/iteration %.2f  waves %.0f\n",
                             sum[0] / sum[6], sum[1] / sum[6], sum[2] / sum[6], sum[3] / sum[6], sum[4] / sum[6], sum[5] / sum[6], sum[7] / sum[5], sum[6]);
        }
#endif
        if (h->phase_events) HIP_TRY(h, hipEventRecord(h->ev[EV_VERIFY], st));
        if ((nshards > 1 || streamed || wide || dpE) && !sel_in_verify) {
            static_assert(po::SEL_CAP == 512, "k_select_local hashes to 9 bits");
            hipLaunchKernelGGL(po::k_select_local, dim3(cdiv(r_end - r_begin, 256 / po::WAVE)), dim3(256), 0, st,
                               h->d_read_tile0.as<uint32_t>(), tile_off_p, A.cand_p, A.cand_b, h->d_type.as<uint8_t>(),
                               r_begin, r_end - r_begin, selfrep, n_deferred, G);
        }
        const bool home_tail_ok = h->home_on && !want_cands && !dpE && !getenv("PHASM_TAIL_CLASSIC") &&
                                  (!n_selfrep_reads || ((nshards > 1 || streamed || wide) && n_cand < (16u << 20))) &&
                                  cdiv(n_cand, po::TAIL_TILE) <= po::TAIL_MAX_TILES;
        if (home_tail_ok && !async_count && h->spare_rows.cap < (size_t)n_cand * sizeof(po::Cand))
            PO_TRY(ensure(h, h->spare_rows, (size_t)n_cand * sizeof(po::Cand) + (streamed ? 65536 : 0), 1.0, false));
        const bool compact_tail = home_tail_ok && h->spare_rows.p && h->spare_rows.cap >= (size_t)n_cand * sizeof(po::Cand);
        const bool can_tail = compact_tail ||
                              (!want_cands && !dpE && h->spare_rows.p && h->spare_rows.cap >= worst_rows * sizeof(po_row) &&
                               (!n_selfrep_reads || ((nshards > 1 || streamed || wide) && n_cand < (16u << 20))) &&
                               cdiv(n_cand, po::TAIL_TILE) <= (streamed || h->home_on ? po::TAIL_MAX_TILES : 4096u) && !getenv("PHASM_TAIL_CLASSIC"));
        if (async_count && !can_tail) return fail(h, PO_ERR_HIP, "internal: a piece with a predicted candidate count needs the fused tail");
        classic_tail = [&]() -> po_status {
        if (n_selfrep_reads) {
            uint32_t n_sus;
            if ((nshards > 1 || streamed || wide) && n_cand < (4u << 20)) {
                n_sus = n_cand;
                gate = n_deferred;
            } else {
                uint32_t* n_suspect = reinterpret_cast<uint32_t*>(scalars + 2) + 1;
                hipLaunchKernelGGL(po::k_count_suspects, dim3(std::min<uint32_t>(cdiv(n_cand, 256), (uint32_t)h->n_cu * 8)), dim3(256), 0,
                                   st, A.cand_b, h->d_type.as<uint8_t>(), n_cand, selfrep, n_suspect);
                HIP_TRY(h, hipMemcpyAsync(h->pinned + 8, scalars + 2, 8, hipMemcpyDeviceToHost, st));
                HIP_TRY(h, hipStreamSynchronize(st));
                n_sus = (uint32_t)(h->pinned[8] >> 32);
            }
            if (n_sus) {
                pbits = 4;
                while ((1ull << pbits) < 2ull * n_sus) ++pbits;
                PO_TRY(ensure_piece(h, h->d_pair_key, ((size_t)1 << pbits) * sizeof(po::PairSlot)));
                hipLaunchKernelGGL(po::k_fill_gated, dim3((uint32_t)h->n_cu * 8), dim3(256), 0, st, h->d_pair_key.as<uint4>(),
                                   (uint64_t)((size_t)1 << pbits) * sizeof(po::PairSlot) / 16, 0xFFFFFFFFu, gate);
                ptab = h->d_pair_key.as<po::PairSlot>();
                hipLaunchKernelGGL(po::k_select_mark, dim3(cdiv(n_cand, 256)), dim3(256), 0, st, A.cand_a, A.cand_p, A.cand_b,
                                   h->d_type.as<uint8_t>(), n_cand, selfrep, ptab, pbits, gate);
            }
        }
        if (want_cands) PO_TRY(ensure(h, h->d_flag, (size_t)n_cand));
        hipLaunchKernelGGL(po::k_select, dim3(cdiv(n_cand, 256)), dim3(256), 0, st, A.cand_a, A.cand_p, A.cand_b,
                           h->d_type.as<uint8_t>(), n_cand, selfrep, ptab, pbits, paired, h->d_rowcnt.as<uint8_t>(),
                           want_cands ? h->d_flag.as<uint8_t>() : nullptr, gate);
        HIP_TRY(h, hipGetLastError());
        if (!want_cands) {
            PO_TRY(prefix_sum<uint8_t>(h, h->d_rowcnt.as<uint8_t>(), n_cand, h->d_row_off.as<uint32_t>(), &h->pinned[2]));
            if (h->phase_events) HIP_TRY(h, hipEventRecord(h->ev[EV_SELECT], st));
            rows_late = h->spare_rows.p && h->spare_rows.cap >= worst_rows * sizeof(po_row);
            if (!rows_late) {
                HIP_TRY(h, hipStreamSynchronize(st));
                n_rows64 = h->pinned[2];
                if (n_rows64 >= 0xFFFFFF00ull) return fail(h, PO_ERR_CAPACITY, "row count exceeds one call's capacity (2^32)");
            }
        }
        if (want_cands) {
            PO_TRY(prefix_sum<uint8_t>(h, h->d_flag.as<uint8_t>(), n_cand, h->d_row_off.as<uint32_t>(), &h->pinned[3]));
            if (h->phase_events) HIP_TRY(h, hipEventRecord(h->ev[EV_SELECT], st));
            po::Cand* dst;
            uint64_t dst_cap;
            if (res->ext_dst && res->ext_cap && !getenv("PHASM_COMPACT_SYNC")) {
                dst = static_cast<po::Cand*>(res->ext_dst);
                dst_cap = res->ext_cap;
                cands_late = true;
                cands_ext = true;
            } else if (h->spare_cands.p && h->spare_cands.cap >= (size_t)n_cand * sizeof(po::Cand) && !getenv("PHASM_COMPACT_SYNC")) {
                res->d_rows = h->spare_cands;
                h->spare_cands = DevBuf();
                dst = res->d_rows.as<po::Cand>();
                dst_cap = n_cand;
                cands_late = true;
            } else {
                HIP_TRY(h, hipStreamSynchronize(st));
                const uint64_t n_ver = h->pinned[3];
                if (res->ext_dst && n_ver <= res->ext_cap) {
                    dst = static_cast<po::Cand*>(res->ext_dst);
                    res->wrote_ext = true;
                } else {
                    if (h->spare_cands.p && h->spare_cands.cap >= n_ver * sizeof(po::Cand)) {
                        res->d_rows = h->spare_cands;
                        h->spare_cands = DevBuf();
                    }
                    PO_TRY(ensure(h, res->d_rows, std::max<size_t>(n_ver * sizeof(po::Cand), 256), 1.0, false));
                    dst = res->d_rows.as<po::Cand>();
                }
                dst_cap = n_ver;
                n_rows64 = n_ver;
            }
            cands_cap = dst_cap;
            hipLaunchKernelGGL(po::k_compact, dim3(cdiv(n_cand, 256)), dim3(256), 0, st, A.cand_a, A.cand_p, A.cand_b,
                               h->d_type.as<uint8_t>(), h->d_flag.as<uint8_t>(), h->d_row_off.as<uint32_t>(), n_cand, dst,
                               (uint32_t)std::min<uint64_t>(dst_cap, 0xFFFFFFFFull));
            HIP_TRY(h, hipGetLastError());
            res->elem = sizeof(po::Cand);
        } else {
            if (rows_late || (h->spare_rows.cap >= n_rows64 * sizeof(po_row) && h->spare_rows.p)) {
                res->d_rows = h->spare_rows;
                h->spare_rows = DevBuf();
            } else {
                h->spare_rows.release();
            }
            if (!rows_late) {
                const size_t exact = n_rows64 * sizeof(po_row);
                size_t roomy = worst_rows * sizeof(po_row) <= (2ull << 30) ? (size_t)(worst_rows * sizeof(po_row)) : 0;
                if (roomy && streamed) roomy += 4096 * sizeof(po_row);
                PO_TRY(ensure(h, res->d_rows, std::max<size_t>(std::max(exact, roomy), 256), 1.0, false));
            }
            if (dpE)
                hipLaunchKernelGGL(po::k_emit_ex, dim3(std::min<uint32_t>(cdiv(n_cand, 256), (uint32_t)h->n_cu * 16)), dim3(256), 0,
                                   st, A.cand_a, A.cand_p, A.cand_b, h->d_type.as<uint8_t>(), h->d_end_a.as<uint32_t>(),
                                   h->d_end_b.as<uint32_t>(), h->d_row_off.as<uint32_t>(), n_cand, len,
                                   res->d_rows.as<po::Row>(), (uint32_t)BITS, scalars + 4);
            else
            hipLaunchKernelGGL(po::k_emit, dim3(std::min<uint32_t>(cdiv(n_cand, 256), (uint32_t)h->n_cu * 16)), dim3(256), 0,
// ... 1969 lines not shown
    h->asm_n = nshards;
    h->asm_parts = nparts;
    h->dirty = true;
    const uint64_t piece_bytes = h->upload_bytes;
    po_status st;
    try {
        st = upload(h);
    } catch (const std::bad_alloc&) {
        st = fail(h, PO_ERR_NOMEM, "out of host memory in po_upload_assemble");
    }
    h->asm_pieces = nullptr;
    h->asm_parts = 1;
    if (st != PO_OK && h->dev_ready) (void)hipStreamSynchronize(h->stream);
    if (st == PO_OK) {
        h->upload_bytes += piece_bytes;
        h->stats.upload_bytes = h->upload_bytes;
    }
    return st;
}

po_status po_upload_assemble(po_handle* h, const void* pieces_device, uint64_t slot_words, uint32_t nshards) {
    return po_upload_assemble_parts(h, pieces_device, slot_words, nshards, 1);
}

po_status po_invalidate(po_handle* h) {
    if (!h) return PO_ERR_INVALID;
    h->dirty = true;
    return PO_OK;
}

static po_status overlaps_common(po_handle* h, uint32_t min_length, uint32_t shard, uint32_t nshards, bool want_cands,
                                 po_result** out, void* ext_dst = nullptr, uint64_t ext_cap = 0) {
    if (!h || !out) return PO_ERR_INVALID;
    *out = nullptr;
    if (nshards == 0 || shard >= nshards) return fail(h, PO_ERR_INVALID, "shard must be < nshards");
    if (h->segments_only) return fail(h, PO_ERR_INVALID, "this handle holds GFA segments without sequences: nothing to overlap");
    po_result* r = new (std::nothrow) po_result();
    if (!r) return fail(h, PO_ERR_NOMEM, "out of host memory");
    r->h = h;
    r->ext_dst = ext_dst;
    r->ext_cap = ext_cap;
    po_status st;
    try {
        st = upload(h);
        if (st == PO_OK) st = h->bits == 2 ? run_overlaps<2>(h, min_length, shard, nshards, want_cands, r)
                                           : run_overlaps<8>(h, min_length, shard, nshards, want_cands, r);
    } catch (const std::bad_alloc&) {
        st = fail(h, PO_ERR_NOMEM, "out of host memory in po_overlaps");
    }
    if (st != PO_OK) {
        if (h->dev_ready) (void)hipStreamSynchronize(h->stream);
        r->d_rows.release();
        delete r;
        return st;
    }
    ++h->live_results;
    *out = r;
    return PO_OK;
}

po_status po_overlaps_shard(po_handle* h, uint32_t min_length, uint32_t shard, uint32_t nshards, po_result** out) {
    return overlaps_common(h, min_length, shard, nshards, false, out);
}

po_status po_candidates_shard(po_handle* h, uint32_t min_length, uint32_t shard, uint32_t nshards, po_result** out) {
    return overlaps_common(h, min_length, shard, nshards, true, out);
}

po_status po_candidates_shard_into(po_handle* h, uint32_t min_length, uint32_t shard, uint32_t nshards, void* dst_device,
                                   uint64_t capacity, int* written, po_result** out) {
    if (written) *written = 0;
    if (!dst_device && capacity) return PO_ERR_INVALID;
    const po_status st = overlaps_common(h, min_length, shard, nshards, true, out, dst_device, capacity);
    if (st == PO_OK && written) *written = (*out)->wrote_ext ? 1 : 0;
    return st;
}

po_status po_expand(po_handle* h, const void* candidates_device, uint64_t n_candidates, po_result** out) {
    if (!h || !out || (!candidates_device && n_candidates)) return PO_ERR_INVALID;
    *out = nullptr;
    if (h->segments_only) return fail(h, PO_ERR_INVALID, "this handle holds GFA segments without sequences");
    po_result* r = new (std::nothrow) po_result();
    if (!r) return fail(h, PO_ERR_NOMEM, "out of host memory");
    r->h = h;
    po_status st;
    try {
        st = upload(h);
        if (st == PO_OK) st = run_expand(h, candidates_device, n_candidates, r);
    } catch (const std::bad_alloc&) {
        st = fail(h, PO_ERR_NOMEM, "out of host memory in po_expand");
    }
    if (st != PO_OK) {
        if (h->dev_ready) (void)hipStreamSynchronize(h->stream);
        r->d_rows.release();
        delete r;
        return st;
    }
    ++h->live_results;
    *out = r;
    return PO_OK;
}

po_status po_overlaps(po_handle* h, uint32_t min_length, po_result** out) {
    return po_overlaps_shard(h, min_length, 0, 1, out);
}

extern "C++" {
namespace {

struct HostRows {
    HostBuf hb;
    uint64_t total = 0;
};

bool home_begin(po_handle* h) {
    h->home_on = false;
    if (!home_enabled()) return false;
    home::Pool* P = home::pool();
    if (!P) return false;
    P->call_mu.lock();
    home::begin(P, h->len.data(), (uint32_t)h->len.size(), getenv("PHASM_STREAM_TRACE") != nullptr || getenv("PHASM_HOME_TRACE") != nullptr);
    h->home_on = true;
    h->home_used = 0;
    h->home_seq = 0;
    if (h->home_pack_n != h->len.size() || h->home_pack_bases != h->total_bases) {
        uint32_t longest = 0;
        for (uint32_t l : h->len) longest = std::max(longest, l);
        uint32_t br = 1, bp = 1;
        while ((1ull << br) < (uint64_t)h->len.size()) ++br;
        while ((1ull << bp) < (uint64_t)longest + 1ull) ++bp;
        const bool fits = 2 * br + bp <= 62;
        h->home_pack_b = fits ? br : 0u;
        h->home_pack_p = fits ? 2 * br : 0u;
        h->home_pack_n = h->len.size();
        h->home_pack_bases = h->total_bases;
    }
    const char* pk = getenv("PHASM_HOME_PACK");
    const bool pack = !(pk && atoi(pk) == 0);
    h->home_sh_b = pack ? h->home_pack_b : 0u;
    h->home_sh_p = pack ? h->home_pack_p : 0u;
    return true;
}

void home_wait(po_handle* h) {
    if (h->home_on) home::wait_all(home::g_pool);
}

int home_end(po_handle* h, po_stats* sum = nullptr) {
    if (!h->home_on) return 0;
    home::Pool* P = home::g_pool;
    home::wait_all(P);
    const int err = P->error.load();
    if (sum) {
        sum->sum_overlap_bases += P->sum_l.load();
        sum->verify_bytes_algo += P->sum_b.load();
        sum->verify_bytes_exec += P->sum_e.load();
    }
    if (P->tracing)
        for (size_t i = 0; i < P->trace.size(); ++i)
            std::fprintf(stderr, "[home] piece %zu: records home at %.3f ms, %.0f rows written at %.3f ms (since the call set the pool up)\n", i,
                         P->trace[i][0] * 1e-3, P->trace[i][2], P->trace[i][1] * 1e-3);
    h->home_on = false;
    P->call_mu.unlock();
    return err;
}

po_status rows_room(po_handle* h, HostRows& R, uint64_t nk, uint32_t k, uint32_t n_chunks, double seen_share) {
    const size_t need = (size_t)(R.total + nk) * sizeof(po_row);
    if (need <= R.hb.cap) return PO_OK;
    uint64_t guess = std::max<uint64_t>(h->last_host_rows, (R.total + nk) * n_chunks / (k + 1));
    if (seen_share > 0.0) guess = std::max<uint64_t>(guess, (uint64_t)((double)(R.total + nk) / seen_share * 1.05));
    HostBuf bigger;
    PO_TRY(ensure_host(h, bigger, std::max<size_t>(need, (size_t)(guess + guess / 8) * sizeof(po_row))));
    home_wait(h);
    if (hipStreamSynchronize(h->copy_stream) != hipSuccess) {
        bigger.release();
        return fail(h, PO_ERR_HIP, "copy stream");
    }
    if (R.total) std::memcpy(bigger.p, R.hb.p, (size_t)R.total * sizeof(po_row));
    R.hb.release();
    R.hb = bigger;
    return PO_OK;
}

po_status append_home(po_handle* h, HostRows& R, const DevBuf& dev, uint64_t n_rec, uint64_t nk, uint32_t k, uint32_t n_chunks,
                      double seen_share = 0.0) {
    if (nk == 0) return PO_OK;
    home::Pool* P = home::g_pool;
    PO_TRY(rows_room(h, R, nk, k, n_chunks, seen_share));
    const size_t elem = h->home_sh_b ? sizeof(uint64_t) : sizeof(po::Cand);
    const size_t bytes = (size_t)n_rec * elem;
    constexpr uint64_t N_EV = 32;
    if (h->home_used + bytes > h->home_stage.cap || (h->home_seq && h->home_seq % N_EV == 0)) {
        home_wait(h);
        if (hipStreamSynchronize(h->copy_stream) != hipSuccess) return fail(h, PO_ERR_HIP, "copy stream");
        h->home_used = 0;
        if (bytes > h->home_stage.cap)
            PO_TRY(ensure_host(h, h->home_stage, std::max<size_t>({bytes * 2, (size_t)(h->home_last_bytes + h->home_last_bytes / 8), (size_t)8 << 20})));
    }
    const uint32_t slot = (uint32_t)(h->home_seq % N_EV);
    const uint32_t want = ++h->home_gen;
    char* dst = static_cast<char*>(h->home_stage.p) + h->home_used;
    HIP_TRY(h, hipMemcpyAsync(dst, dev.p, bytes, hipMemcpyDeviceToHost, h->copy_stream));
    hipLaunchKernelGGL(po::k_fill_u32, dim3(1), dim3(64), 0, h->copy_stream, reinterpret_cast<uint32_t*>(h->pinned_dev + 96 + slot), (uint64_t)1, want);
    HIP_TRY(h, hipGetLastError());
    home::Job j;
    j.rec = dst;
    j.sh_b = h->home_sh_b;
    j.sh_p = h->home_sh_p;
    j.n_rec = n_rec;
    j.out = static_cast<po_row*>(R.hb.p) + R.total;
    j.n_rows = nk;
    j.flag = reinterpret_cast<const volatile uint32_t*>(h->pinned + 96 + slot);
    j.want = want;
    j.paired = (h->bits == 2 && h->paired) ? 1u : 0u;
    j.bits = (uint32_t)h->bits;
    home::submit(P, j);
    ++h->home_seq;
    h->home_used += (bytes + 255) & ~size_t(255);
    h->home_last_bytes += bytes;
    R.total += nk;
    return PO_OK;
}

po_status append_rows(po_handle* h, HostRows& R, const DevBuf& dev, uint64_t nk, uint32_t k, uint32_t n_chunks, double seen_share = 0.0) {
    if (nk == 0) return PO_OK;
    PO_TRY(rows_room(h, R, nk, k, n_chunks, seen_share));
    HIP_TRY(h, hipMemcpyAsync(static_cast<char*>(R.hb.p) + (size_t)R.total * sizeof(po_row), dev.p, (size_t)nk * sizeof(po_row),
                              hipMemcpyDeviceToHost, h->copy_stream));
    R.total += nk;
    return PO_OK;
}

void add_stats(po_stats& sum, const po_stats& S) {
    sum.n_candidates += S.n_candidates;
    sum.n_verified += S.n_verified;
    sum.n_rows += S.n_rows;
    sum.sum_overlap_bases += S.sum_overlap_bases;
    sum.verify_bytes_algo += S.verify_bytes_algo;
    sum.verify_bytes_exec += S.verify_bytes_exec;
    sum.n_tiles += S.n_tiles;
    sum.shard_bases += S.shard_bases;
    sum.fused_tail += S.fused_tail;
    sum.tail_fallback += S.tail_fallback;
    sum.n_predicted += S.n_predicted;
    sum.ms_index += S.ms_index;
    sum.ms_scan_count += S.ms_scan_count;
    sum.ms_scan_fill += S.ms_scan_fill;
    sum.ms_verify += S.ms_verify;
    sum.ms_select += S.ms_select;
    sum.ms_emit += S.ms_emit;
    sum.ms_total += S.ms_total;
    sum.ms_scan_probe += S.ms_scan_probe;
    sum.ms_verify_kernel += S.ms_verify_kernel;
}

po_status run_chunk(po_handle* h, uint32_t min_length, uint32_t k, uint32_t n_chunks, uint64_t* nk) {
    po_result part;
    part.h = h;
    if (h->chunk_rows[k].p) {
        h->spare_rows.release();
        h->spare_rows = h->chunk_rows[k];
        h->chunk_rows[k] = DevBuf();
    }
    const po_status st = h->bits == 2 ? run_overlaps<2>(h, min_length, k, n_chunks, false, &part)
                                      : run_overlaps<8>(h, min_length, k, n_chunks, false, &part);
    h->chunk_rows[k] = part.d_rows;
    h->chunk_compact[k] = part.compact;
    part.d_rows = DevBuf();
    *nk = part.count;
    return st;
}

bool stream_eligible(const po_handle* h, uint32_t min_length) {
    const uint32_t n = (uint32_t)h->len.size();
    if (!h->dirty || h->bits != 2 || n < 4 || (n % 2) != 0 || !h->all_pairs_rcx) return false;
    if (h->asm_pieces || h->ex_on || h->sl_build_n > 1 || h->ext_index) return false;
    if (getenv("PHASM_FULL_UPLOAD") || getenv("PHASM_NO_MIRROR")) return false;
    bool want = n >= 4096 && h->words[0].size() * 8 >= (16ull << 20);
    if (const char* e = getenv("PHASM_STREAM")) want = atoi(e) != 0;
    if (!want) return false;
    const uint32_t m = min_length ? min_length : 1;
    const uint64_t n_elig = count_eligible(const_cast<po_handle*>(h), m);
    if (n_elig == 0) return false;
    return true;
}

std::vector<uint32_t> stream_bounds(const po_handle* h) {
    const uint32_t n = (uint32_t)h->len.size();
    const uint64_t bytes0 = (uint64_t)h->words[0].size() * 8;
    uint64_t max_pieces = h->chunk_rows[0].p ? 12 : 8;
    const bool big = bytes0 >= (512ull << 20) && h->chunk_rows[0].p;
    if (big) max_pieces = 15;
    if (const char* e = getenv("PHASM_STREAM_MAX_PIECES")) max_pieces = (uint64_t)std::max(2, std::min(PO_MAX_PIECES - 1, atoi(e)));
    const uint32_t n_pieces = (uint32_t)std::min<uint64_t>(max_pieces, std::max<uint64_t>(2, (bytes0 + (8ull << 20)) / (16ull << 20)));
    const double skew = big ? 1.6 : 1.25;
    std::vector<uint32_t> cuts;
    for (uint32_t i = 1; i < n_pieces; ++i) cuts.push_back((uint32_t)(1000.0 * (1.0 - std::pow(1.0 - (double)i / n_pieces, skew))));
    if (const char* e = getenv("PHASM_STREAM_CUTS")) {
        cuts.clear();
        for (const char* q = e; *q;) {
            char* endp = nullptr;
            const long v = strtol(q, &endp, 10);
            if (endp == q) break;
            if (v > 0 && v < 1000 && (cuts.empty() || (uint32_t)v > cuts.back()) && cuts.size() + 1 < (size_t)PO_MAX_PIECES) cuts.push_back((uint32_t)v);
            q = *endp ? endp + 1 : endp;
        }
    }
    std::vector<uint32_t> b{0};
    const uint64_t total = h->words[0].size();
    for (uint32_t c : cuts) {
        const uint64_t target = total * c / 1000;
        uint32_t lo = 0, hi = n / 2;
        while (lo < hi) {
            const uint32_t mid = (lo + hi) / 2;
// ... 156 lines not shown
        }
        return completed(k, h->st_pend.S, nk);
    };
    if (getenv("PHASM_STREAM_SYNC")) h->st_harvest = nullptr;
    for (uint32_t k = 0; k < P && st == PO_OK; ++k) {
        if (hipStreamWaitEvent(h->stream, h->ev_rc[k], 0) != hipSuccess) { st = fail(h, PO_ERR_HIP, "hipStreamWaitEvent"); break; }
        h->st_on = true;
        h->st_r_begin = bounds[k];
        h->st_r_end = bounds[k + 1];
        h->ws_scale = 1.0;
        {
            const double mine = (double)bounds[k + 1] * bounds[k + 1] - (double)bounds[k] * bounds[k];
            for (uint32_t j = k + 1; j < P; ++j)
                h->ws_scale = std::max(h->ws_scale, ((double)bounds[j + 1] * bounds[j + 1] - (double)bounds[j] * bounds[j]) / mine * 1.1);
        }
        h->ev = h->ev_sets[k & 1];
        uint64_t nk = 0;
        st = run_chunk(h, min_length, k, P, &nk);
        h->st_on = false;
        h->ws_scale = 1.0;
        if (st != PO_OK || tail_gave_up) break;
        if (h->st_pend.valid && h->st_pend.k == k) continue;
        if (h->st_pend.valid) {
            if (hipStreamSynchronize(h->stream) != hipSuccess) { st = fail(h, PO_ERR_HIP, "stream"); break; }
            st = h->st_harvest();
            if (st != PO_OK) break;
        }
        st = completed(k, h->stats, nk);
    }
    if (st == PO_OK && h->st_pend.valid && !tail_gave_up) {
        if (hipStreamSynchronize(h->stream) != hipSuccess) st = fail(h, PO_ERR_HIP, "stream");
        else st = h->st_harvest();
    }
    h->st_harvest = nullptr;
    h->st_pend.valid = false;
    h->ev = h->ev_sets[0];
    if (st == PO_OK && tail_gave_up) {
        (void)hipStreamSynchronize(h->stream);
        (void)hipStreamSynchronize(h->up_stream);
        (void)hipStreamSynchronize(h->rc_stream);
        h->dirty = true;
        h->st_tail_gave_up = true;
        h->st_pred_valid = false;
        *overflow = true;
        return PO_OK;
    }
    if (st != PO_OK) {
        (void)hipStreamSynchronize(h->up_stream);
        (void)hipStreamSynchronize(h->rc_stream);
        h->dirty = true;
        h->st_pred_valid = false;
        return st;
    }
    h->st_pred_sig = sig;
    std::memcpy(h->st_pred_cand, new_pred, sizeof(new_pred));
    h->st_pred_valid = true;
    float ms = 0;
    (void)hipEventSynchronize(h->ev_up1);
    (void)hipEventElapsedTime(&ms, h->ev_up0, h->ev_up1);
    h->stats.ms_upload = ms;
    HIP_TRY(h, hipMemcpyAsync(h->pinned + 40, h->d_defer.as<char>() + (size_t)h->st_defer_cap * sizeof(po::Cand), 8,
                              hipMemcpyDeviceToHost, h->stream));
    HIP_TRY(h, hipStreamSynchronize(h->stream));
    const uint32_t n_def = (uint32_t)h->pinned[40];
    h->defer_need = n_def;
    if (n_def > h->st_defer_cap) {
        *overflow = true;
        return PO_OK;
    }
    if (n_def) {
        hipStream_t s = h->stream;
        po::Cand* list = h->d_defer.as<po::Cand>();
        PO_TRY(ensure(h, h->d_rowcnt, (size_t)n_def));
        PO_TRY(ensure(h, h->d_row_off, ((size_t)n_def + 1) * 4));
        HIP_TRY(h, hipEventRecord(h->ev[EV_START], s));
        hipLaunchKernelGGL(po::k_verify_flat, dim3(cdiv((uint64_t)n_def * 64, 256)), dim3(256), 0, s, dw, h->d_woff.as<uint64_t>(),
                           h->d_len.as<uint32_t>(), list, n_def, h->n_exc_uploaded ? h->d_exc_off.as<uint32_t>() : nullptr,
                           h->d_exc_pos.as<uint32_t>(), h->d_exc_byte.as<uint8_t>());
        hipLaunchKernelGGL(po::k_deferred_rowcnt, dim3(cdiv(n_def, 256)), dim3(256), 0, s, list, n_def, 1u, h->d_rowcnt.as<uint8_t>());
        HIP_TRY(h, hipGetLastError());
        PO_TRY(prefix_sum<uint8_t>(h, h->d_rowcnt.as<uint8_t>(), n_def, h->d_row_off.as<uint32_t>(), &h->pinned[2]));
        HIP_TRY(h, hipStreamSynchronize(s));
        const uint64_t n_rows = h->pinned[2];
        if (n_rows) {
            PO_TRY(ensure(h, h->chunk_rows[P], n_rows * sizeof(po_row)));
            unsigned long long* scalars = h->d_scalars.as<unsigned long long>();
            HIP_TRY(h, hipMemsetAsync(scalars + 4, 0, 32, s));
            hipLaunchKernelGGL(po::k_emit_cands, dim3(std::min<uint32_t>(cdiv(n_def, 256), (uint32_t)h->n_cu * 16)), dim3(256), 0, s,
                               list, h->d_rowcnt.as<uint8_t>(), h->d_row_off.as<uint32_t>(), n_def, h->d_len.as<uint32_t>(),
                               h->chunk_rows[P].as<po::Row>(), 2u, 1u, scalars + 4);
            HIP_TRY(h, hipGetLastError());
            HIP_TRY(h, hipMemcpyAsync(h->pinned + 4, scalars + 4, 4 * sizeof(uint64_t), hipMemcpyDeviceToHost, s));
            HIP_TRY(h, hipEventRecord(h->ev[EV_EMIT], s));
            HIP_TRY(h, hipStreamSynchronize(s));
            float ms_def = 0;
            (void)hipEventElapsedTime(&ms_def, h->ev[EV_START], h->ev[EV_EMIT]);
            sum.n_verified += h->pinned[4];
            sum.sum_overlap_bases += h->pinned[5];
            sum.verify_bytes_algo += h->pinned[6];
            sum.verify_bytes_exec += h->pinned[7];
            sum.n_rows += n_rows;
            sum.ms_verify += ms_def;
            sum.ms_total += ms_def;
            PO_TRY(append_rows(h, R, h->chunk_rows[P], n_rows, P, P + 1));
        }
    }
    (void)n;
    if (trace) {
        std::fprintf(stderr, "[stream] deferred list settled at %.3f ms (%u candidates)\n", since(), n_def);
        (void)hipStreamSynchronize(h->copy_stream);
        std::fprintf(stderr, "[stream] last row home at %.3f ms\n", since());
    }
    return PO_OK;
}

}
}

po_status po_overlaps_to_host(po_handle* h, uint32_t min_length, po_result** out) {
    if (!h || !out) return PO_ERR_INVALID;
    *out = nullptr;
    if (h->segments_only) return fail(h, PO_ERR_INVALID, "this handle holds GFA segments without sequences: nothing to overlap");
    uint32_t n_chunks = (h->len.size() >= 8192 && h->total_bases >= (64ull << 20)) ? 4u : 1u;
    if (const char* e = getenv("PHASM_HOST_CHUNKS")) n_chunks = (uint32_t)std::max(1, std::min(4, atoi(e)));
    po_result* r = new (std::nothrow) po_result();
    if (!r) return fail(h, PO_ERR_NOMEM, "out of host memory");
    r->h = h;
    po_status st = PO_OK;
    HostRows R;
    po_stats sum = {};
    bool streamed = false, overflowed = false;
    float ms_upload = 0;
    try {
        st = init_device(h);
        if (st == PO_OK && !h->copy_stream && hipStreamCreateWithFlags(&h->copy_stream, hipStreamNonBlocking) != hipSuccess)
            st = fail(h, PO_ERR_HIP, "cannot create the copy stream");
        if (st == PO_OK && h->spare_host.p) {
            R.hb = h->spare_host;
            h->spare_host = HostBuf();
        }
        if (st == PO_OK) {
            (void)home_begin(h);
            h->home_last_bytes = 0;
        }
        if (st == PO_OK && stream_eligible(h, min_length)) {
            bool overflow = false;
            st = overlaps_streamed(h, min_length, R, sum, &overflow);
            ms_upload = h->stats.ms_upload;
            if (st == PO_OK && !overflow) {
                streamed = true;
            } else if (st == PO_OK) {
                overflowed = true;
                home_wait(h);
                if (h->home_on) {
                    home::g_pool->sum_l.store(0);
                    home::g_pool->sum_b.store(0);
                    home::g_pool->sum_e.store(0);
                }
                if (hipStreamSynchronize(h->copy_stream) != hipSuccess) st = fail(h, PO_ERR_HIP, "copy stream");
                R.total = 0;
                sum = po_stats();
            }
        }
        if (st == PO_OK && !streamed) st = upload(h);
        for (uint32_t k = 0; k < n_chunks && st == PO_OK && !streamed; ++k) {
            uint64_t nk = 0;
            st = run_chunk(h, min_length, k, n_chunks, &nk);
            if (st != PO_OK) break;
            add_stats(sum, h->stats);
            st = h->chunk_compact[k] ? append_home(h, R, h->chunk_rows[k], h->stats.n_verified, nk, k, n_chunks)
                                     : append_rows(h, R, h->chunk_rows[k], nk, k, n_chunks);
        }
    } catch (const std::bad_alloc&) {
        st = fail(h, PO_ERR_NOMEM, "out of host memory in po_overlaps_to_host");
    }
    h->st_on = false;
    h->st_harvest = nullptr;
    h->st_pend.valid = false;
    h->ev = h->ev_sets[0];
    if (h->dev_ready) (void)hipStreamSynchronize(h->stream);
    if (h->up_stream) (void)hipStreamSynchronize(h->up_stream);
    if (h->rc_stream) (void)hipStreamSynchronize(h->rc_stream);
    if (h->copy_stream && hipStreamSynchronize(h->copy_stream) != hipSuccess && st == PO_OK) st = fail(h, PO_ERR_HIP, "row copy device->host");
    {
        const int herr = home_end(h, &sum);
        if (herr && st == PO_OK)
            st = fail(h, PO_ERR_HIP, herr == 1 ? "internal: the host's row count of a piece differs from the device's"
                                     : herr == 2 ? "internal: a verified-candidate record names a read the handle does not hold"
                                                 : "the event behind a device->host copy of records failed");
    }
    if (st != PO_OK) {
        R.hb.release();
        delete r;
        return st;
    }
    po_stats& S = h->stats;
    S.n_candidates = sum.n_candidates;
    S.n_verified = sum.n_verified;
    S.n_rows = sum.n_rows;
    S.sum_overlap_bases = sum.sum_overlap_bases;
    S.verify_bytes_algo = sum.verify_bytes_algo;
    S.verify_bytes_exec = sum.verify_bytes_exec;
    S.n_tiles = sum.n_tiles;
    S.shard_bases = sum.shard_bases;
    S.ms_index = sum.ms_index;
    S.ms_scan_count = sum.ms_scan_count;
    S.ms_scan_fill = sum.ms_scan_fill;
    S.ms_verify = sum.ms_verify;
    S.ms_select = sum.ms_select;
    S.ms_emit = sum.ms_emit;
    S.ms_total = sum.ms_total;
    S.ms_scan_probe = sum.ms_scan_probe;
    S.ms_verify_kernel = sum.ms_verify_kernel;
    S.fused_tail = sum.fused_tail;
    S.n_predicted = sum.n_predicted;
    S.home_record_bytes = h->home_last_bytes ? (h->home_sh_b ? 8u : 16u) : 0u;
    S.tail_fallback = sum.tail_fallback + (h->st_tail_gave_up ? 1u : 0u);
    h->st_tail_gave_up = false;
    S.streamed = streamed ? 1u : 0u;
    S.n_deferred = (streamed || overflowed) ? h->defer_need : 0u;
    if (streamed) {
        S.ms_upload = ms_upload;
        S.upload_bytes = h->upload_bytes;
    }
    h->last_host_rows = R.total;
    r->count = R.total;
    r->unique_twins = h->bits == 2 && h->paired;
    if (R.total) {
        r->host = R.hb.p;
        r->host_cap = R.hb.cap;
    } else if (R.hb.p) {
        h->spare_host = R.hb;
    }
    ++h->live_results;
    *out = r;
    return PO_OK;
}

po_status po_index_slice_build(po_handle* h, uint32_t min_length, uint32_t slice, uint32_t n_slices, uint32_t* is_wide,
                               uint32_t* slice_bits, uint64_t* chain_entries) {
    if (!h || !is_wide || !slice_bits || !chain_entries) return PO_ERR_INVALID;
    if (n_slices < 2 || slice >= n_slices) return fail(h, PO_ERR_INVALID, "po_index_slice_build: need 2 or more slices and slice < n_slices");
    *is_wide = 0;
    *slice_bits = 0;
    *chain_entries = 0;
    h->sl_build_slice = slice;
    h->sl_build_n = n_slices;
    h->sl_is_wide = false;
    po_result* r = nullptr;
    const po_status st = overlaps_common(h, min_length, 0, 1, false, &r);
    h->sl_build_n = 0;
    if (r) po_result_free(r);
    if (st != PO_OK) return st;
    *is_wide = h->sl_is_wide ? 1u : 0u;
    if (h->sl_is_wide) {
        *slice_bits = h->sl_tbits;
        *chain_entries = h->sl_entries;
    }
    return PO_OK;
}

static bool slice_args_ok(uint32_t n_slices, uint32_t slice_bits, uint64_t chain_capacity) {
    return n_slices >= 2 && n_slices <= 4096 && slice_bits >= 1 && slice_bits <= 30 && chain_capacity < (1ull << 36);
}

uint64_t po_index_chunk_bytes(uint32_t slice_bits, uint64_t chain_capacity, uint64_t* chain_offset_bytes) {
    if (chain_offset_bytes) *chain_offset_bytes = 0;
    if (slice_bits < 1 || slice_bits > 30 || chain_capacity >= (1ull << 36)) return 0;
    const uint64_t off = ((((1ull << slice_bits) + 1ull) * sizeof(po::Slot)) + 255ull) & ~255ull;
    if (chain_offset_bytes) *chain_offset_bytes = off;
    return (off + chain_capacity * 8ull + 255ull) & ~255ull;
}

po_status po_index_slice_export(po_handle* h, void* dst_device, uint64_t chain_capacity) {
    if (!h || !dst_device) return PO_ERR_INVALID;
    if (!h->sl_is_wide || !h->dev_ready) return fail(h, PO_ERR_INVALID, "po_index_slice_export: no sub-table has been built on this handle");
    if (chain_capacity < h->sl_entries) return fail(h, PO_ERR_INVALID, "po_index_slice_export: chain capacity below this sub-table's entries");
    uint64_t off = 0;
    (void)po_index_chunk_bytes(h->sl_tbits, chain_capacity, &off);
    HIP_TRY(h, hipSetDevice(h->device));
    HIP_TRY(h, hipMemcpyAsync(dst_device, h->d_table.p, ((size_t)(1ull << h->sl_tbits) + 1) * sizeof(po::Slot), hipMemcpyDeviceToDevice, h->stream));
    if (h->sl_entries)
        HIP_TRY(h, hipMemcpyAsync(static_cast<char*>(dst_device) + off, h->d_chain.p, (size_t)h->sl_entries * 8, hipMemcpyDeviceToDevice, h->stream));
    HIP_TRY(h, hipStreamSynchronize(h->stream));
    return PO_OK;
}

po_status po_candidates_shard_indexed(po_handle* h, uint32_t min_length, uint32_t shard, uint32_t nshards,
                                      const void* index_device, uint32_t n_slices, uint32_t slice_bits, uint64_t chain_capacity,
                                      void* dst_device, uint64_t capacity, int* written, po_result** out) {
    if (written) *written = 0;
    if (!h || !out || !index_device) return PO_ERR_INVALID;
    if (!slice_args_ok(n_slices, slice_bits, chain_capacity))
        return fail(h, PO_ERR_INVALID, "sliced index: need 2..4096 slices of 2^1..2^30 slots (slice_bits as po_index_slice_build reported it)");
    if (!dst_device && capacity) return PO_ERR_INVALID;
    uint64_t off = 0;
    const uint64_t chunk = po_index_chunk_bytes(slice_bits, chain_capacity, &off);
    if ((chunk / 16) * n_slices >= 0xFFFFFFF0ull) return fail(h, PO_ERR_CAPACITY, "sliced index larger than 64 GB");
    h->ext_index = index_device;
    h->ext_slices = n_slices;
    h->ext_tbits = slice_bits;
    h->ext_chunk_slots = (uint32_t)(chunk / 16);
    h->ext_chain_off = (uint32_t)(off / 16);
    const po_status st = overlaps_common(h, min_length, shard, nshards, true, out, dst_device, capacity);
    h->ext_index = nullptr;
    if (st == PO_OK && written) *written = (*out)->wrote_ext ? 1 : 0;
    return st;
}

po_status po_overlaps_shard_indexed(po_handle* h, uint32_t min_length, uint32_t shard, uint32_t nshards, const void* index_device,
                                    uint32_t n_slices, uint32_t slice_bits, uint64_t chain_capacity, po_result** out) {
// ... 575 lines not shown
    return guarded_run(h, "po_layout_coverage", [&] { return run_coverage(h, graph, rows, coverage_out); });
}

po_status po_layout_components(po_handle* h, po_result* graph, const po_components_params* params, uint32_t* node_component_out,
                               uint32_t* edge_component_out, po_component* components_out, uint64_t* n_components_out) {
    return graph_call(h, graph, "po_layout_components", !params || params->reserved == 0, "components", n_components_out, [&] {
        return run_components(h, graph, node_component_out, edge_component_out, components_out, n_components_out);
    });
}

po_status po_layout_partition(po_handle* h, po_result* graph, const po_partition_params* params, uint32_t* node_scc_out,
                              uint8_t* node_flags_out, uint8_t* edge_class_out, po_scc* sccs_out, uint64_t* n_sccs_out) {
    return graph_call(h, graph, "po_layout_partition", !params || params->reserved == 0, "strongly connected components", n_sccs_out, [&] {
        return run_partition(h, graph, node_scc_out, node_flags_out, edge_class_out, sccs_out, n_sccs_out);
    });
}

po_status po_graph_from_edges(po_handle* h, const po_edge* edges, uint64_t n_edges, const uint32_t* node_order, uint64_t n_order,
                              po_result** out) {
    if (!h || !out || (!edges && n_edges) || (!node_order && n_order)) return PO_ERR_INVALID;
    *out = nullptr;
    if (n_edges >= 0x7FFFFF00ull) return fail(h, PO_ERR_CAPACITY, "po_graph_from_edges: too many edges for one call");
    const size_t n_ids = h->len.size();
    try {
        std::vector<uint8_t> in_order(n_ids, 0);
        for (uint64_t i = 0; i < n_order; ++i) {
            const uint32_t x = node_order[i];
            if (x >= n_ids) return fail(h, PO_ERR_INVALID, "po_graph_from_edges: the node order names a read the handle does not hold");
            if (in_order[x]) return fail(h, PO_ERR_INVALID, "po_graph_from_edges: a node appears twice in the node order");
            in_order[x] = 1;
        }
        std::vector<uint64_t> pairs(n_edges);
        for (uint64_t e = 0; e < n_edges; ++e) {
            const uint32_t u = edges[e].u, v = edges[e].v;
            if (u >= n_ids || v >= n_ids) return fail(h, PO_ERR_INVALID, "po_graph_from_edges: an edge names a read the handle does not hold");
            if (!in_order[u] || !in_order[v])
                return fail(h, PO_ERR_INVALID, "po_graph_from_edges: an edge has an end that is not in the node order");
            pairs[e] = ((uint64_t)u << 32) | v;
        }
        std::sort(pairs.begin(), pairs.end());
        if (std::adjacent_find(pairs.begin(), pairs.end()) != pairs.end())
            return fail(h, PO_ERR_INVALID, "po_graph_from_edges: an edge appears twice");
    } catch (const std::bad_alloc&) {
        return fail(h, PO_ERR_NOMEM, "out of host memory in po_graph_from_edges");
    }
    PO_TRY(init_device(h));
    return new_edge_result(h, "po_graph_from_edges", out, [&](po_result* r) {
        r->elem = sizeof(po_edge);
        r->kind_edges = true;
        r->host_graph = true;
        const size_t nrank_bytes = std::max<size_t>(n_ids * 8, 256);
        PO_TRY(ensure_nrank(h, r, nrank_bytes));
        PO_TRY(ensure_host(h, h->scratch_host, nrank_bytes));
        std::memset(h->scratch_host.p, 0xFF, nrank_bytes);
        uint64_t* words = static_cast<uint64_t*>(h->scratch_host.p);
        for (uint64_t i = 0; i < n_order; ++i) words[node_order[i]] = i;
        HIP_TRY(h, hipMemcpyAsync(r->d_nrank.p, words, nrank_bytes, hipMemcpyHostToDevice, h->stream));
        HIP_TRY(h, hipStreamSynchronize(h->stream));
        if (n_edges) {
            void* copy = std::malloc(n_edges * sizeof(po_edge));
            if (!copy) return fail(h, PO_ERR_NOMEM, "out of host memory for the edge array");
            std::memcpy(copy, edges, n_edges * sizeof(po_edge));
            r->host = copy;
            r->host_malloced = true;
        }
        r->count = n_edges;
        return PO_OK;
    });
}

po_status po_get_layout_stats(const po_handle* h, po_layout_stats* out) { return get_stats(h, &po_handle::lstats, out); }
po_status po_get_node_order_stats(const po_handle* h, po_node_order_stats* out) { return get_stats(h, &po_handle::nostats, out); }
po_status po_get_reduce_stats(const po_handle* h, po_reduce_stats* out) { return get_stats(h, &po_handle::rstats, out); }
po_status po_get_tips_stats(const po_handle* h, po_tips_stats* out) { return get_stats(h, &po_handle::tstats, out); }
po_status po_get_diamond_stats(const po_handle* h, po_diamond_stats* out) { return get_stats(h, &po_handle::dstats, out); }
po_status po_get_merge_stats(const po_handle* h, po_merge_stats* out) { return get_stats(h, &po_handle::mstats, out); }
po_status po_get_coverage_stats(const po_handle* h, po_coverage_stats* out) { return get_stats(h, &po_handle::cstats, out); }
po_status po_get_components_stats(const po_handle* h, po_components_stats* out) { return get_stats(h, &po_handle::ccstats, out); }
po_status po_get_partition_stats(const po_handle* h, po_partition_stats* out) { return get_stats(h, &po_handle::pstats, out); }

po_status po_result_merged_paths(po_result* r, uint64_t* n_paths, uint64_t* n_members, uint64_t* offsets_out, uint64_t cap_paths,
                                 uint32_t* members_out, int32_t* prefix_out, uint64_t cap_members, int64_t* lengths_out) {
    if (!r || !n_paths || !n_members) return PO_ERR_INVALID;
    *n_paths = *n_members = 0;
    po_handle* h = r->h;
    if (!h) return PO_ERR_INVALID;
    if (!r->merged) return fail(h, PO_ERR_INVALID, "po_result_merged_paths needs a po_layout_merge result");
    const uint64_t K = r->n_merged, m = r->n_members;
    *n_paths = K;
    *n_members = m;
    try {
        (void)hipSetDevice(h->device);
        HIP_TRY(h, hipStreamSynchronize(h->stream));
        if (offsets_out && cap_paths >= K) {
            std::vector<uint32_t> off(K);
            if (K) HIP_TRY(h, hipMemcpy(off.data(), r->d_moff.p, K * 4, hipMemcpyDeviceToHost));
            for (uint64_t k = 0; k < K; ++k) offsets_out[k] = off[k];
            offsets_out[K] = m;
        }
        if (lengths_out && cap_paths >= K && K) HIP_TRY(h, hipMemcpy(lengths_out, r->d_mlen.p, K * 8, hipMemcpyDeviceToHost));
        if (members_out && cap_members >= m && m) HIP_TRY(h, hipMemcpy(members_out, r->d_member.p, m * 4, hipMemcpyDeviceToHost));
        if (prefix_out && cap_members >= m && m) HIP_TRY(h, hipMemcpy(prefix_out, r->d_prefix.p, m * 4, hipMemcpyDeviceToHost));
    } catch (const std::bad_alloc&) {
        return fail(h, PO_ERR_NOMEM, "out of host memory in po_result_merged_paths");
    }
    return PO_OK;
}

po_status po_result_node_order(po_result* r, uint32_t* nodes_out, uint64_t cap, uint64_t* n_out) {
    if (!r || !n_out || (!nodes_out && cap)) return PO_ERR_INVALID;
    *n_out = 0;
    po_handle* h = r->h;
    if (!h) return PO_ERR_INVALID;
    if (!r->kind_edges || !r->d_nrank.p) return fail(h, PO_ERR_INVALID, "po_result_node_order needs an edge result");
    const size_t n_nodes = h->len.size() + (r->merged ? (size_t)r->n_merged : 0);
    try {
        std::vector<unsigned long long> rank(n_nodes);
        (void)hipSetDevice(h->device);
        HIP_TRY(h, hipStreamSynchronize(h->stream));
        if (n_nodes) HIP_TRY(h, hipMemcpy(rank.data(), r->d_nrank.p, n_nodes * 8, hipMemcpyDeviceToHost));
        std::vector<std::pair<unsigned long long, uint32_t>> order;
        for (size_t i = 0; i < n_nodes; ++i)
            if (rank[i] != po::NODE_NO_RANK) order.emplace_back(rank[i], (uint32_t)i);
        std::sort(order.begin(), order.end());
        *n_out = order.size();
        for (size_t i = 0; i < order.size() && i < cap; ++i) nodes_out[i] = order[i].second;
    } catch (const std::bad_alloc&) {
        return fail(h, PO_ERR_NOMEM, "out of host memory in po_result_node_order");
    }
    return PO_OK;
}

uint64_t po_debug_host_ranges(uint64_t* out, uint64_t cap_entries) {
    std::lock_guard<std::mutex> lock(g_pin_mu);
    const uint64_t n = std::min<uint64_t>(cap_entries, g_pins.size());
    for (uint64_t i = 0; out && i < n; ++i) {
        out[3 * i] = g_pins[i].base;
        out[3 * i + 1] = g_pins[i].bytes;
        out[3 * i + 2] = g_pins[i].kind;
    }
    return g_pins.size();
}

uint64_t po_debug_store_words(const po_handle* h, int store, const uint64_t** words) {
    if (!h || store < 0 || store > 1) return 0;
    if (words) *words = h->words[store].data();
    return h->words[store].size();
}

int po_debug_expand_records(const po_cand* records, uint64_t n, const uint32_t* lengths, uint32_t n_reads, uint32_t paired,
                            po_row* rows_out, uint64_t n_rows_expected) {
    home::Pool* P = home::pool();
    if (!P) return -1;
    std::lock_guard<std::mutex> call(P->call_mu);
    home::begin(P, lengths, n_reads, false);
    home::Job j;
    j.rec = records;
    j.n_rec = n;
    j.out = rows_out;
    j.n_rows = n_rows_expected;
    j.paired = paired ? 1u : 0u;
    home::submit(P, j);
    home::wait_all(P);
    return P->error.load();
}

int po_debug_expand_packed(const uint64_t* records, uint64_t n, uint32_t sh_b, uint32_t sh_p, const uint32_t* lengths, uint32_t n_reads,
                           uint32_t paired, po_row* rows_out, uint64_t n_rows_expected) {
    if (!sh_b || sh_p < sh_b || sh_p >= 62) return -2;
    home::Pool* P = home::pool();
    if (!P) return -1;
    std::lock_guard<std::mutex> call(P->call_mu);
    home::begin(P, lengths, n_reads, false);
    home::Job j;
    j.rec = records;
    j.sh_b = sh_b;
    j.sh_p = sh_p;
    j.n_rec = n;
    j.out = rows_out;
    j.n_rows = n_rows_expected;
    j.paired = paired ? 1u : 0u;
    home::submit(P, j);
    home::wait_all(P);
    return P->error.load();
}

static int g_fault_fd = 2;
static struct sigaction g_fault_prev[2];
static void fault_handler(int sig, siginfo_t* si, void* ctx) {
    char line[128];
    const int n = std::snprintf(line, sizeof(line), "[phasm] signal %d at address %p (code %d); native stack of the faulting thread:\n", sig,
                                si ? si->si_addr : nullptr, si ? si->si_code : 0);
    if (n > 0) (void)!::write(g_fault_fd, line, (size_t)n);
    void* frames[64];
    const int k = backtrace(frames, 64);
    backtrace_symbols_fd(frames, k, g_fault_fd);
    const struct sigaction& prev = g_fault_prev[sig == SIGBUS ? 1 : 0];
    if ((prev.sa_flags & SA_SIGINFO) && prev.sa_sigaction) {
        prev.sa_sigaction(sig, si, ctx);
        return;
    }
    if (prev.sa_handler != SIG_DFL && prev.sa_handler != SIG_IGN && prev.sa_handler) {
        prev.sa_handler(sig);
        return;
    }
    signal(sig, SIG_DFL);
    raise(sig);
}

int po_debug_fault_backtrace(int fd) {
    g_fault_fd = fd;
    struct sigaction sa;
    std::memset(&sa, 0, sizeof(sa));
    sa.sa_sigaction = fault_handler;
    sa.sa_flags = SA_SIGINFO | SA_NODEFER;
    sigemptyset(&sa.sa_mask);
    void* warm[4];
    (void)backtrace(warm, 4);
    return (sigaction(SIGSEGV, &sa, &g_fault_prev[0]) == 0 && sigaction(SIGBUS, &sa, &g_fault_prev[1]) == 0) ? 0 : -1;
}

int po_debug_pointer_info(const void* p, int32_t* hip_type, int32_t* hsa_type, uint64_t* base, uint64_t* bytes) {
    if (hip_type) *hip_type = -1;
    if (hsa_type) *hsa_type = -1;
    if (base) *base = 0;
    if (bytes) *bytes = 0;
    if (!p) return 0;
    int known = 0;
    {
        hipPointerAttribute_t at;
        std::memset(&at, 0, sizeof(at));
        const hipError_t e = hipPointerGetAttributes(&at, p);
        if (e == hipSuccess) {
            if (hip_type) *hip_type = (int32_t)at.type;
            if (at.type != hipMemoryTypeUnregistered) known = 1;
        } else {
            (void)hipGetLastError();
        }
    }
    {
        struct PtrInfo {
            uint32_t size;
            uint32_t type;
            void* agentBaseAddress;
            void* hostBaseAddress;
            size_t sizeInBytes;
            void* userData;
            uint64_t agentOwner;
            uint32_t global_flags;
        };
        using Fn = int (*)(const void*, PtrInfo*, void* (*)(size_t), uint32_t*, void**);
        static Fn fn = reinterpret_cast<Fn>(dlsym(RTLD_DEFAULT, "hsa_amd_pointer_info"));
        if (fn) {
            PtrInfo info;
            std::memset(&info, 0, sizeof(info));
            info.size = sizeof(info);
            if (fn(p, &info, nullptr, nullptr, nullptr) == 0) {
                if (hsa_type) *hsa_type = (int32_t)info.type;
                if (info.type != 0) {
                    known = 1;
                    if (base) *base = (uint64_t)(uintptr_t)(info.hostBaseAddress ? info.hostBaseAddress : info.agentBaseAddress);
                    if (bytes) *bytes = info.sizeInBytes;
                }
            }
        }
    }
    return known;
}

po_status po_get_stats(const po_handle* h, po_stats* out) {
    if (!h || !out) return PO_ERR_INVALID;
    *out = h->stats;
    return PO_OK;
}

const char* po_last_error(const po_handle* h) { return h ? h->err.c_str() : "null handle"; }

}
```

phasm_amd/csrc/kernels.hip.h:

```cpp
#pragma once
#include <hip/hip_runtime.h>
#include <stdint.h>

namespace po {

using u32x4 = __attribute__((ext_vector_type(4))) uint32_t;

constexpr uint32_t NO_SELFREP = 0xFFFFFFFFu;
constexpr uint64_t KEY_EMPTY = ~0ull;
constexpr int WAVE = 64;

#ifndef PO_VER_PAD
#define PO_VER_PAD 0
#endif
#ifndef PO_SCAN_PAD
#define PO_SCAN_PAD 0
#endif
template <int N>
__device__ __forceinline__ void valu_pad(uint32_t& r, uint32_t c) {
#pragma unroll
    for (int i = 0; i < N; ++i) asm volatile("v_xor_b32 %0, %0, %1" : "+v"(r) : "v"(c));
}

struct CandGuard {
    const unsigned long long* n_dev;
    uint32_t cap;
    __device__ __forceinline__ bool overflow() const { return n_dev && *n_dev > (unsigned long long)cap; }
};
#ifndef PO_FILTER_DEPTH
#define PO_FILTER_DEPTH 6
#endif
constexpr int SCAN_BLOCK = 1024;
constexpr int TILE_WORDS = 64;

struct __attribute__((aligned(16))) Slot {
    uint64_t key;
    uint32_t start;
    uint32_t count;
};
constexpr uint32_t SLOT_SINGLE = 0x80000000u;

struct Row {
    uint32_t a_idx, b_idx;
    int32_t astart, aend, bstart, bend;
};

struct __attribute__((aligned(32))) TileRec {
    uint64_t wabs;
    uint64_t wread;
    uint32_t read;
    uint32_t la;
    uint32_t word0;
    uint32_t pad;
};

__global__ void k_build_tiles(const uint64_t* __restrict__ woff, const uint32_t* __restrict__ len,
                              const uint32_t* __restrict__ read_tile0, uint32_t n_reads, uint32_t n_tiles,
                              TileRec* __restrict__ tiles) {
    const uint32_t t = blockIdx.x * blockDim.x + threadIdx.x;
    if (t >= n_tiles) return;
    uint32_t lo = 0, hi = n_reads;
    while (hi - lo > 1) {
        const uint32_t mid = (lo + hi) >> 1;
        if (read_tile0[mid] <= t) lo = mid; else hi = mid;
    }
    TileRec rec;
    rec.word0 = (t - read_tile0[lo]) * (uint32_t)TILE_WORDS;
    rec.wread = woff[lo];
    rec.wabs = rec.wread + rec.word0;
    rec.read = lo;
    rec.la = len[lo];
    rec.pad = 0;
    tiles[t] = rec;
}

__global__ void k_abs_woff(uint64_t* __restrict__ woff, uint32_t n_reads, uint64_t base1) {
    const uint32_t r = blockIdx.x * blockDim.x + threadIdx.x;
    if (r < n_reads && (r & 1u)) woff[r] += base1;
}

__global__ void k_count_diff(const uint64_t* __restrict__ a, const uint64_t* __restrict__ b, uint64_t n,
                             unsigned long long* __restrict__ n_diff) {
    unsigned long long d = 0;
    for (uint64_t i = (uint64_t)blockIdx.x * blockDim.x + threadIdx.x; i < n; i += (uint64_t)gridDim.x * blockDim.x)
        d += a[i] != b[i];
    if (d) atomicAdd(n_diff, d);
}

__host__ __device__ inline void kmer_hash(uint64_t k, uint32_t& h1, uint32_t& h2) {
    uint32_t lo = (uint32_t)k, hi = (uint32_t)(k >> 32);
    uint32_t x = lo ^ ((hi << 13) | (hi >> 19));
    h1 = x * 0x9E3779B1u;
    h2 = (x ^ (x >> 15) ^ (hi * 5u)) * 0x85EBCA77u;
}

__host__ __device__ inline void bloom_slot(uint64_t k, uint32_t bloom_log2, uint32_t& word, uint32_t& mask) {
    uint32_t h1, h2;
    kmer_hash(k, h1, h2);
    (void)h2;
    word = h1 >> (32 - (bloom_log2 - 5));
    mask = (1u << ((h1 >> 7) & 31)) | (1u << ((h1 >> 12) & 31)) | (1u << ((h1 >> 2) & 31));
}

__device__ inline void note_selfrep(uint32_t* __restrict__ selfrep, uint32_t a, uint32_t p, uint32_t* __restrict__ n_marked) {
    if (atomicMin(&selfrep[a], p) == NO_SELFREP) atomicAdd(n_marked, 1u);
}

__device__ inline uint32_t lane_id() { return threadIdx.x & (WAVE - 1); }

__device__ inline uint32_t wave_incl_scan(uint32_t v) {
    v += (uint32_t)__builtin_amdgcn_update_dpp(0, (int)v, 0x111, 0xf, 0xf, false);
    v += (uint32_t)__builtin_amdgcn_update_dpp(0, (int)v, 0x112, 0xf, 0xf, false);
    v += (uint32_t)__builtin_amdgcn_update_dpp(0, (int)v, 0x114, 0xf, 0xf, false);
    v += (uint32_t)__builtin_amdgcn_update_dpp(0, (int)v, 0x118, 0xf, 0xf, false);
    v += (uint32_t)__builtin_amdgcn_update_dpp(0, (int)v, 0x142, 0xa, 0xf, false);
    v += (uint32_t)__builtin_amdgcn_update_dpp(0, (int)v, 0x143, 0xc, 0xf, false);
    return v;
}

__device__ inline uint32_t read_last_lane(uint32_t v) { return __builtin_amdgcn_readlane(v, WAVE - 1); }

__device__ inline uint32_t wave_sum(uint32_t v) { return read_last_lane(wave_incl_scan(v)); }

__device__ inline uint64_t wave_sum64(uint64_t v) {
    const uint32_t lo = (uint32_t)v, hi = (uint32_t)(v >> 32);
    const uint64_t s0 = wave_sum(lo & 0xFFFFu), s1 = wave_sum(lo >> 16), s2 = wave_sum(hi & 0xFFFFu), s3 = wave_sum(hi >> 16);
    return s0 + (s1 << 16) + (s2 << 32) + (s3 << 48);
}

__device__ inline void wave_lds_fence() {
    __builtin_amdgcn_fence(__ATOMIC_ACQ_REL, "workgroup");
    __builtin_amdgcn_wave_barrier();
}

__device__ inline uint64_t funnel(uint64_t lo, uint64_t hi, uint32_t sh) {
    return sh ? (lo >> sh) | (hi << (64 - sh)) : lo;
}

__device__ inline uint32_t mirror_rank(uint32_t x, uint32_t paired) {
    const uint32_t scrambled = __brev(x >> 8) | (x & 0xFFu);
    return paired == 2u ? scrambled : x;
}
__device__ inline bool canonical_pair(uint32_t a, uint32_t c, uint32_t paired) {
    return mirror_rank(a, paired) <= mirror_rank(c, paired);
}
constexpr uint32_t PAIRED_STREAM_ALL = 0xFFFFFFFFu;
__device__ __host__ inline uint32_t paired_stream(uint32_t b_limit) { return 3u | (b_limit << 2); }

template <bool STREAM = false>
__device__ inline uint32_t keep_bits(uint32_t a, uint32_t b, uint32_t rem, uint32_t lb, uint32_t paired) {
    if (a == b) return 0;
    if constexpr (STREAM) {
        return ((rem <= lb && a >= (b ^ 1u)) ? 1u : 0u) | ((rem >= lb && (a & 1u) == 0u && b < (paired >> 2)) ? 2u : 0u);
    } else {
        return ((rem <= lb && (!paired || canonical_pair(a, b ^ 1u, paired))) ? 1u : 0u) |
// ... 913 lines not shown

template <int BITS, bool STREAM = false>
__global__ void k_scan_fixup(const ScanArgs A, uint32_t n_waves, uint32_t clean) {
    constexpr int W = 64 / BITS;
    const uint32_t wv = blockIdx.x;
    if (wv >= n_waves) return;
    const uint32_t cnt = min(A.left_cnt[wv], LEFT_CAP);
    const uint2* __restrict__ list = A.left + (size_t)wv * LEFT_CAP;
    for (uint32_t k = threadIdx.x; k < cnt; k += blockDim.x) {
        const uint2 e = list[k];
        const uint32_t t = e.x, ln = e.y >> 8, sft = e.y & 255u;
        if (t < A.tile_begin || t >= A.tile_end || ln >= (uint32_t)WAVE || sft >= (uint32_t)W) continue;
        const TileRec rec = A.tiles[t];
        const uint64_t w0 = A.words[rec.wabs + ln], w1 = A.words[rec.wabs + ln + 1];
        const uint64_t kmer = funnel(w0, w1, sft * BITS) & A.kmask;
        uint32_t z = 0, w = 0;
        table_probe(A.table, A.tbits, kmer, z, w);
        if (!w) continue;
        const uint32_t a = rec.read, p = (rec.word0 + ln) * W + sft;
        if (p > 0) {
            if (w & SLOT_SINGLE) {
                if (z == a) note_selfrep(A.selfrep, a, p, A.n_selfrep);
            } else {
                for (uint32_t j = 0; j < w; ++j)
                    if (A.chain[z + j] == a) note_selfrep(A.selfrep, a, p, A.n_selfrep);
            }
        }
        uint32_t n = 0;
        for_each_candidate<STREAM>(A.chain, A.len, A.paired, z, w, a, rec.la - p, [&](uint32_t, uint32_t, uint32_t) { ++n; });
        if (n) {
            atomicOr(&A.truemask[(size_t)t * WAVE + ln], 1u << sft);
            atomicAdd(&A.tile_count[t], n);
        }
    }
    if (clean) {
        __syncthreads();
        if (threadIdx.x == 0) A.left_cnt[wv] = 0;
    }
}

__global__ void k_add_extra(uint32_t* __restrict__ tile_count, const uint32_t* __restrict__ tile_extra, uint32_t t0, uint32_t t1) {
    const uint32_t t = t0 + blockIdx.x * blockDim.x + threadIdx.x;
    if (t < t1 && tile_extra[t]) tile_count[t] += tile_extra[t];
}

#ifndef PO_FILL_TILES
#define PO_FILL_TILES 8
#endif
constexpr int FILL_TILES = PO_FILL_TILES;

template <int BITS, bool STREAM = false>
__global__ __launch_bounds__(256) void k_scan_fill(const ScanArgs A, const CandGuard G) {
    constexpr int W = 64 / BITS;
    __shared__ uint32_t q_src[4 * WAVE];
    __shared__ TileRec q_rec[4 * FILL_TILES];
    if (G.overflow()) return;
    const uint32_t lane = lane_id(), wave = threadIdx.x >> 6;
    uint32_t* qs = q_src + wave * WAVE;
    TileRec* qr = q_rec + wave * FILL_TILES;
    const uint32_t t0 = __builtin_amdgcn_readfirstlane(A.tile_begin + (blockIdx.x * 4 + wave) * FILL_TILES);
    if (t0 >= A.tile_end) return;
    uint32_t hm[FILL_TILES], rk[FILL_TILES];
#pragma unroll
    for (int i = 0; i < FILL_TILES; ++i) hm[i] = t0 + i < A.tile_end ? A.truemask[(size_t)(t0 + i) * WAVE + lane] : 0u;
    if (lane < (uint32_t)FILL_TILES) qr[lane] = A.tiles[min(t0 + lane, A.tile_end - 1)];
    uint32_t out = A.tile_off[t0];
    uint32_t total = 0;
#pragma unroll
    for (int i = 0; i < FILL_TILES; ++i) {
        const uint32_t nh = __popc(hm[i]);
        const uint32_t incl = wave_incl_scan(nh);
        rk[i] = total + incl - nh;
        total += read_last_lane(incl);
    }
    if (total == 0) return;
    for (uint32_t r0 = 0; r0 < total; r0 += WAVE) {
#pragma unroll
        for (int i = 0; i < FILL_TILES; ++i) {
            while (hm[i] && rk[i] < r0 + WAVE) {
                const uint32_t sft = __ffs(hm[i]) - 1;
                hm[i] &= hm[i] - 1;
                qs[rk[i] - r0] = ((uint32_t)i << 16) | (lane << 8) | sft;
                ++rk[i];
            }
        }
        wave_lds_fence();
        const bool has = r0 + lane < total;
        const uint32_t src = has ? qs[lane] : 0u;
        const TileRec rec = qr[src >> 16];
        wave_lds_fence();
        const uint32_t ln = (src >> 8) & 255u, sft = src & 255u;
        uint32_t z = 0, w = 0;
        if (has) {
            const uint64_t w0 = A.words[rec.wabs + ln], w1 = A.words[rec.wabs + ln + 1];
            table_probe(A.table, A.tbits, funnel(w0, w1, sft * BITS) & A.kmask, z, w);
        }
        const uint32_t a = rec.read, la = rec.la;
        const uint32_t p = (rec.word0 + ln) * W + sft;
        uint32_t n = 0;
        if (w) for_each_candidate<STREAM>(A.chain, A.len, A.paired, z, w, a, la - p, [&](uint32_t, uint32_t, uint32_t) { ++n; });
        const uint32_t inc = wave_incl_scan(n);
        uint32_t off = out + inc - n;
        if (n) {
            for_each_candidate<STREAM>(A.chain, A.len, A.paired, z, w, a, la - p, [&](uint32_t b, uint32_t, uint32_t) {
                A.cand_a[off] = a;
                A.cand_p[off] = p;
                A.cand_b[off] = b;
                ++off;
            });
        }
        out += read_last_lane(inc);
    }
}

struct DeferOut {
    const uint32_t* cand_p;
    uint32_t b_limit;
    uint4* list;
    uint32_t cap;
    uint32_t* counter;
};
__global__ __launch_bounds__(256) void k_read_label(const uint32_t* __restrict__ read_tile0, const uint32_t* __restrict__ tile_off,
                                                    const uint32_t* __restrict__ cand_b, uint32_t r_begin, uint32_t n_reads,
                                                    uint32_t paired, uint32_t* __restrict__ label, const DeferOut defer,
                                                    const CandGuard G) {
    const uint32_t t = blockIdx.x * blockDim.x + threadIdx.x;
    const uint32_t i = t >> 4, sub = t & 15u;
    if (i >= n_reads) return;
    if (G.overflow()) {
        if (sub == 0) label[i] = r_begin + i;
        return;
    }
    const uint32_t a = r_begin + i;
    const uint32_t seg0 = tile_off[read_tile0[a]], seg1 = tile_off[read_tile0[a + 1]];
    const bool reversed = (paired & 3u) == 3u;
    auto rank = [&](uint32_t x) { return reversed ? ~x : mirror_rank(x, paired); };
    uint32_t best = rank(a);
    for (uint32_t c = seg0 + sub; c < seg1; c += 16) {
        const uint32_t b = cand_b[c];
        best = max(best, rank(b ^ 1u));
        if (defer.list && b >= defer.b_limit) {
            const uint32_t k = atomicAdd(defer.counter, 1u);
            if (k < defer.cap) defer.list[k] = uint4{a, defer.cand_p[c], b, 0u};
        }
    }
#pragma unroll
    for (int o = 8; o >= 1; o >>= 1) best = max(best, (uint32_t)__shfl_xor((int)best, o, 16));
    if (paired == 2u) best = (__brev(best & 0xFFFFFF00u) << 8) | (best & 0xFFu);
    if (reversed) best = ~best;
    if (sub == 0) label[i] = best;
}

constexpr int SORT_BLOCK = 1024;
__global__ __launch_bounds__(SORT_BLOCK) void k_read_sort(const uint32_t* __restrict__ label, uint32_t n_reads, uint32_t shift,
                                                          uint32_t n_bins, uint32_t* __restrict__ rank) {
    extern __shared__ uint32_t s_bin[];
    uint32_t* s_wave = s_bin + n_bins;
    const uint32_t tid = threadIdx.x;
    for (uint32_t b = tid; b < n_bins; b += SORT_BLOCK) s_bin[b] = 0;
    __syncthreads();
    constexpr uint32_t UN = 16;
    for (uint32_t base = tid; base < n_reads; base += UN * SORT_BLOCK) {
        uint32_t v[UN];
#pragma unroll
        for (uint32_t k = 0; k < UN; ++k) {
            const uint32_t i = base + k * SORT_BLOCK;
            v[k] = i < n_reads ? label[i] : ~0u;
        }
#pragma unroll
        for (uint32_t k = 0; k < UN; ++k)
            if (v[k] != ~0u) atomicAdd(&s_bin[v[k] >> shift], 1u);
    }
    __syncthreads();
    const uint32_t per = (n_bins + SORT_BLOCK - 1) / SORT_BLOCK;
    const uint32_t lo = min(tid * per, n_bins), hi = min(lo + per, n_bins);
    uint32_t sum = 0;
    for (uint32_t b = lo; b < hi; ++b) sum += s_bin[b];
    const uint32_t incl = wave_incl_scan(sum);
    if (lane_id() == WAVE - 1) s_wave[tid >> 6] = incl;
    __syncthreads();
    uint32_t run = incl - sum;
    for (uint32_t w = 0; w < (tid >> 6); ++w) run += s_wave[w];
    for (uint32_t b = lo; b < hi; ++b) {
        const uint32_t v = s_bin[b];
        s_bin[b] = run;
        run += v;
    }
    __syncthreads();
    for (uint32_t base = tid; base < n_reads; base += UN * SORT_BLOCK) {
        uint32_t v[UN];
#pragma unroll
        for (uint32_t k = 0; k < UN; ++k) {
            const uint32_t i = base + k * SORT_BLOCK;
            v[k] = i < n_reads ? label[i] : ~0u;
        }
#pragma unroll
        for (uint32_t k = 0; k < UN; ++k)
            if (v[k] != ~0u) rank[base + k * SORT_BLOCK] = atomicAdd(&s_bin[v[k] >> shift], 1u);
    }
}

__global__ void k_read_invert(const uint32_t* __restrict__ rank, uint32_t n_reads, uint32_t r_begin, uint32_t* __restrict__ perm) {
    const uint32_t i = blockIdx.x * blockDim.x + threadIdx.x;
    if (i < n_reads && rank[i] < n_reads) perm[rank[i]] = r_begin + i;
}

__device__ inline bool exceptions_equal(const uint32_t* __restrict__ exc_off, const uint32_t* __restrict__ exc_pos,
                                        const uint8_t* __restrict__ exc_byte, uint32_t a, uint32_t p, uint32_t b,
                                        uint32_t n) {
    uint32_t ia = exc_off[a];
    const uint32_t ea = exc_off[a + 1];
    uint32_t ib = exc_off[b];
    const uint32_t eb = exc_off[b + 1];
    if (ia == ea && ib == eb) return true;
    {
        uint32_t lo = ia, hi = ea;
        while (lo < hi) {
            const uint32_t mid = (lo + hi) >> 1;
            if (exc_pos[mid] < p) lo = mid + 1; else hi = mid;
        }
        ia = lo;
    }
    for (;;) {
        const bool ha = ia < ea && exc_pos[ia] - p < n;
        const bool hb = ib < eb && exc_pos[ib] < n;
        if (!ha && !hb) return true;
        if (ha != hb) return false;
        if (exc_pos[ia] - p != exc_pos[ib] || exc_byte[ia] != exc_byte[ib]) return false;
        ++ia;
        ++ib;
    }
}

#ifndef PO_VER_GROUP
#define PO_VER_GROUP 16
#endif
constexpr int VER_GROUP = PO_VER_GROUP;
#ifndef PO_VER_BLOCK
#define PO_VER_BLOCK 256
#endif
constexpr int VER_BLOCK = PO_VER_BLOCK;
#ifndef PO_VER_BLOCKS
#define PO_VER_BLOCKS 3
#endif
#ifndef PO_VER_FIRST
#define PO_VER_FIRST PO_VER_BLOCKS
#endif
constexpr int VER_BLOCKS = PO_VER_BLOCKS;

#ifdef PO_VSTAMPS
__device__ unsigned long long g_vstamps[64 * 8];
#define VST(...) __VA_ARGS__
#else
#define VST(...)
#endif

constexpr int VREC_CAP = 512;
constexpr uint32_t SEL_CAP = 512;
__device__ __forceinline__ void select_read_list(uint32_t seg0, uint32_t seg1, const uint32_t* __restrict__ cand_p,
                                                 const uint32_t* __restrict__ cand_b, uint8_t* __restrict__ type,
                                                 uint32_t* __restrict__ selfrep, uint32_t* __restrict__ n_deferred,
                                                 uint32_t* key, uint32_t* mn, uint32_t lane);
struct __attribute__((aligned(16))) VRec {
    uint32_t pk;
    uint32_t b;
    uint32_t nk;
    uint32_t wo;
};

__device__ __forceinline__ uint32_t lds_draw(uint32_t* counter) {
    typedef __attribute__((address_space(3))) uint32_t lds_u32;
    const uint32_t addr = (uint32_t)(uintptr_t)(lds_u32*)counter;
    uint32_t old, one = 1u;
    asm volatile("ds_add_rtn_u32 %0, %1, %2\n\ts_waitcnt lgkmcnt(0)" : "=v"(old) : "v"(addr), "v"(one) : "memory");
    return old;
}

__device__ __forceinline__ uint32_t group_bcast0(uint32_t v, uint32_t gshift) {
    if constexpr (VER_GROUP == 16) {
        (void)gshift;
        return (uint32_t)__builtin_amdgcn_update_dpp(0, (int)v, 0x150, 0xf, 0xf, false);
    } else {
        return (uint32_t)__shfl((int)v, (int)gshift);
    }
}

template <int BITS, bool SCRAMBLED, bool IN_LDS, bool STAGED, bool STREAM = false>
__device__ __forceinline__ void verify_run(const uint64_t* __restrict__ words, const uint64_t* __restrict__ woff,
                                           const uint32_t* __restrict__ len, const uint32_t* __restrict__ cand_p,
                                           const uint32_t* __restrict__ cand_b, uint32_t paired,
                                           const uint32_t* __restrict__ exc_off, const uint32_t* __restrict__ exc_pos,
                                           const uint8_t* __restrict__ exc_byte, uint8_t* __restrict__ type,
                                           const uint32_t* __restrict__ s_a, const uint32_t* __restrict__ ga32,
                                           const VRec* __restrict__ s_rec, uint32_t* s_next, uint32_t a, uint32_t la,
                                           uint32_t seg0, uint32_t seg1
                                           VST(, unsigned long long vt_start, unsigned long long (&vt)[8])) {
    constexpr int W = 64 / BITS;
    (void)W;
    const uint32_t sub = threadIdx.x & (VER_GROUP - 1);
    const uint32_t gshift = (lane_id() / VER_GROUP) * VER_GROUP;
    constexpr uint32_t NGROUPS = VER_BLOCK / VER_GROUP;

    uint32_t c = seg0;
    uint32_t cA = seg0 + threadIdx.x / VER_GROUP, cB = cA + NGROUPS;
    bool have = cA < seg1;
    uint32_t nbits = 0, sh = 0, q = 0, d = 0, keep = 0, nblk_var = 1, cur_p = 0, cur_b = 0;
    uint32_t nd = 0;
    constexpr bool UNIFORM_STEPS = PO_VER_FIRST == PO_VER_BLOCKS;
    const uint32_t* B = reinterpret_cast<const uint32_t*>(words);
    const uint32_t c_last = seg1 - 1;
    uint32_t m0p = 0, m0b = 0, m0l = 0, m1p = 0, m1b = 0;
    uint64_t m0w = 0;
    if constexpr (!STAGED) {
        const uint32_t c0 = min(cA, c_last), c1 = min(cB, c_last);
        m0p = cand_p[c0];
        m0b = cand_b[c0];
        m1p = cand_p[c1];
        m1b = cand_b[c1];
        m0l = len[m0b];
        m0w = woff[m0b];
    }
    auto init = [&]() __attribute__((always_inline)) {
        uint32_t p, b, lb;
        uint64_t wo;
        if constexpr (STAGED) {
            c = cA;
            const VRec r = s_rec[c - seg0];
            p = r.pk;
            b = r.b;
            lb = r.nk;
            wo = r.wo;
            uint32_t drawn = 0;
            if (sub == 0) drawn = lds_draw(s_next);
            cA = group_bcast0(drawn, gshift);
        } else {
            p = m0p;
            b = m0b;
            lb = m0l;
            wo = m0w;
            c = cA;
            cA = cB;
            m0p = m1p;
            m0b = m1b;
            m0l = len[m1b];
            m0w = woff[m1b];
            uint32_t drawn = 0;
            if (sub == 0) drawn = lds_draw(s_next);
            cB = group_bcast0(drawn, gshift);
            const uint32_t c2 = min(cB, c_last);
            m1p = cand_p[c2];
            m1b = cand_b[c2];
// ... 246 lines not shown
__global__ __launch_bounds__(256) void k_count_suspects(const uint32_t* __restrict__ cand_b, const uint8_t* __restrict__ type,
                                                        uint32_t n_cand, const uint32_t* __restrict__ selfrep,
                                                        uint32_t* __restrict__ n_suspect) {
    __shared__ uint32_t s_part[256 / WAVE];
    uint32_t n = 0;
    for (uint32_t i = blockIdx.x * blockDim.x + threadIdx.x; i < n_cand; i += gridDim.x * blockDim.x)
        n += ((type[i] & 1u) && selfrep[cand_b[i]] != NO_SELFREP) ? 1u : 0u;
    n = (uint32_t)wave_sum64(n);
    if (lane_id() == 0) s_part[threadIdx.x >> 6] = n;
    __syncthreads();
    if (threadIdx.x == 0) {
        uint32_t t = 0;
        for (int w = 0; w < 256 / WAVE; ++w) t += s_part[w];
        if (t) atomicAdd(n_suspect, t);
    }
}

__global__ void k_fill_gated(uint4* __restrict__ p, uint64_t n16, uint32_t v, const uint32_t* __restrict__ gate) {
    if (gate && *gate == 0u) return;
    for (uint64_t i = (uint64_t)blockIdx.x * blockDim.x + threadIdx.x; i < n16; i += (uint64_t)gridDim.x * blockDim.x)
        p[i] = uint4{v, v, v, v};
}

__global__ void k_select_mark(const uint32_t* __restrict__ cand_a, const uint32_t* __restrict__ cand_p, const uint32_t* __restrict__ cand_b,
                              const uint8_t* __restrict__ type, uint32_t n_cand, const uint32_t* __restrict__ selfrep,
                              PairSlot* __restrict__ ptab, uint32_t tbits, const uint32_t* __restrict__ gate) {
    if (gate && *gate == 0u) return;
    const uint32_t i = blockIdx.x * blockDim.x + threadIdx.x;
    if (i >= n_cand || !(type[i] & 1u)) return;
    const uint32_t a = cand_a[i], b = cand_b[i];
    if (selfrep[b] == NO_SELFREP) return;
    const unsigned long long key = ((unsigned long long)a << 32) | b;
    const uint32_t tmask = (1u << tbits) - 1u;
    uint32_t s = pair_slot(a, b, tbits);
    for (;;) {
        unsigned long long prev = ptab[s].key;
        if (prev == ~0ull) prev = atomicCAS(&ptab[s].key, ~0ull, key);
        if (prev == ~0ull || prev == key) break;
        s = (s + 1u) & tmask;
    }
    atomicMin(&ptab[s].min_idx, cand_p[i]);
}

__device__ inline uint32_t rows_of(uint32_t t, uint32_t a, uint32_t b, uint32_t paired) {
    if (!paired) return (t & 1u) + ((t >> 1) & 1u);
    return ((t & 1u) ? (a == (b ^ 1u) ? 1u : 2u) : 0u) + ((t & 2u) ? 2u : 0u);
}

__global__ void k_select(const uint32_t* __restrict__ cand_a, const uint32_t* __restrict__ cand_p, const uint32_t* __restrict__ cand_b,
                         uint8_t* __restrict__ type, uint32_t n_cand, const uint32_t* __restrict__ selfrep,
                         const PairSlot* __restrict__ ptab, uint32_t tbits,
                         uint32_t paired, uint8_t* __restrict__ rowcnt, uint8_t* __restrict__ flag,
                         const uint32_t* __restrict__ gate) {
    uint32_t i = blockIdx.x * blockDim.x + threadIdx.x;
    if (i >= n_cand) return;
    if (gate && *gate == 0u) ptab = nullptr;
    uint32_t t = type[i];
    if (t == 0) {
        rowcnt[i] = 0;
        if (flag) flag[i] = 0;
        return;
    }
    const uint32_t a = cand_a[i], b = cand_b[i];
    if (ptab && (t & 1u) && selfrep[b] != NO_SELFREP) {
        const unsigned long long key = ((unsigned long long)a << 32) | b;
        const uint32_t tmask = (1u << tbits) - 1u;
        uint32_t s = pair_slot(a, b, tbits);
        uint32_t first;
        for (;;) {
            const uint4 q = *reinterpret_cast<const uint4*>(&ptab[s]);
            if ((((unsigned long long)q.y << 32) | q.x) == key) {
                first = q.z;
                break;
            }
            s = (s + 1u) & tmask;
        }
        if (first != cand_p[i]) {
            t &= ~1u;
            type[i] = (uint8_t)t;
        }
    }
    rowcnt[i] = (uint8_t)rows_of(t, a, b, paired);
    if (flag) flag[i] = t != 0;
}

__device__ inline uint32_t packed_bytes(uint32_t l, uint32_t bits) { return bits == 8u ? l : (l >> 2) + ((l & 3u) != 0u); }

__device__ inline void write_rows(Row* __restrict__ rows, uint32_t off, uint32_t t, uint32_t a, uint32_t p, uint32_t b,
                                  uint32_t la, uint32_t lb, uint32_t bits, uint32_t paired, uint64_t& suml,
                                  uint64_t& sumb, uint64_t& sume) {
    sume += 2ull * packed_bytes((t & 1u) ? la - p : lb, bits);
    if (t & 1u) {
        const uint32_t l = la - p;
        const uint64_t two_pb = 2ull * packed_bytes(l, bits);
        rows[off++] = Row{a, b, (int32_t)p, (int32_t)la, 0, (int32_t)l};
        suml += l;
        sumb += two_pb;
        if (paired && a != (b ^ 1u)) {
            rows[off++] = Row{b ^ 1u, a ^ 1u, (int32_t)(lb - l), (int32_t)lb, 0, (int32_t)l};
            suml += l;
            sumb += two_pb;
        }
    }
    if (t & 2u) {
        const uint64_t two_pb = 2ull * packed_bytes(lb, bits);
        rows[off++] = Row{a, b, (int32_t)p, (int32_t)(p + lb), 0, (int32_t)lb};
        suml += lb;
        sumb += two_pb;
        if (paired) {
            rows[off++] = Row{a ^ 1u, b ^ 1u, (int32_t)(la - p - lb), (int32_t)(la - p), 0, (int32_t)lb};
            suml += lb;
            sumb += two_pb;
        }
    }
}

__device__ inline void flush_counters(uint64_t nver, uint64_t suml, uint64_t sumb, uint64_t sume,
                                      unsigned long long* __restrict__ counters) {
    __shared__ uint64_t s_red[4][1024 / WAVE];
    nver = wave_sum64(nver);
    suml = wave_sum64(suml);
    sumb = wave_sum64(sumb);
    sume = wave_sum64(sume);
    if (lane_id() == 0) {
        s_red[0][threadIdx.x >> 6] = nver;
        s_red[1][threadIdx.x >> 6] = suml;
        s_red[2][threadIdx.x >> 6] = sumb;
        s_red[3][threadIdx.x >> 6] = sume;
    }
    __syncthreads();
    if (threadIdx.x < 4) {
        uint64_t v = 0;
        for (uint32_t w = 0; w < blockDim.x / WAVE; ++w) v += s_red[threadIdx.x][w];
        if (v) atomicAdd(&counters[threadIdx.x], (unsigned long long)v);
    }
}

__global__ __launch_bounds__(256) void k_emit(const uint32_t* __restrict__ cand_a, const uint32_t* __restrict__ cand_p,
                                              const uint32_t* __restrict__ cand_b, const uint8_t* __restrict__ type,
                                              const uint32_t* __restrict__ row_off, uint32_t n_cand,
                                              const uint32_t* __restrict__ len, Row* __restrict__ rows, uint32_t bits,
                                              uint32_t paired, unsigned long long* __restrict__ counters) {
    uint64_t nver = 0, suml = 0, sumb = 0, sume = 0;
    for (uint32_t i = blockIdx.x * blockDim.x + threadIdx.x; i < n_cand; i += gridDim.x * blockDim.x) {
        const uint32_t t = type[i];
        if (t == 0) continue;
        nver += 1;
        const uint32_t a = cand_a[i], p = cand_p[i], b = cand_b[i];
        write_rows(rows, row_off[i], t, a, p, b, len[a], len[b], bits, paired, suml, sumb, sume);
    }
    flush_counters(nver, suml, sumb, sume, counters);
}

struct Cand {
    uint32_t a, p, b, type;
};

__host__ __device__ inline uint64_t pack_record(uint32_t a, uint32_t p, uint32_t b, uint32_t type, uint32_t sh_b, uint32_t sh_p) {
    return (uint64_t)a | ((uint64_t)b << sh_b) | ((uint64_t)p << sh_p) | ((uint64_t)type << 62);
}
__host__ __device__ inline Cand unpack_record(uint64_t v, uint32_t sh_b, uint32_t sh_p) {
    const uint64_t mr = (1ull << sh_b) - 1ull;
    return Cand{(uint32_t)(v & mr), (uint32_t)((v >> sh_p) & ((1ull << (62u - sh_p)) - 1ull)), (uint32_t)((v >> sh_b) & mr), (uint32_t)(v >> 62)};
}

__global__ void k_compact(const uint32_t* __restrict__ cand_a, const uint32_t* __restrict__ cand_p,
                          const uint32_t* __restrict__ cand_b, const uint8_t* __restrict__ type,
                          const uint8_t* __restrict__ flag, const uint32_t* __restrict__ flag_off, uint32_t n_cand,
                          Cand* __restrict__ out, uint32_t cap) {
    uint32_t i = blockIdx.x * blockDim.x + threadIdx.x;
    if (i >= n_cand || flag[i] == 0) return;
    const uint32_t o = flag_off[i];
    if (o < cap) out[o] = Cand{cand_a[i], cand_p[i], cand_b[i], type[i]};
}

__global__ void k_flag(const uint8_t* __restrict__ rowcnt, uint32_t n, uint8_t* __restrict__ flag) {
    uint32_t i = blockIdx.x * blockDim.x + threadIdx.x;
    if (i < n) flag[i] = rowcnt[i] != 0;
}

__global__ void k_cand_rowcnt(const Cand* __restrict__ cands, uint32_t n, uint32_t n_reads, uint32_t paired,
                              uint8_t* __restrict__ rowcnt, uint32_t* __restrict__ n_bad) {
    uint32_t i = blockIdx.x * blockDim.x + threadIdx.x;
    if (i >= n) return;
    const Cand c = cands[i];
    if ((c.a | c.p | c.b | c.type) == 0) {
        rowcnt[i] = 0;
        return;
    }
    if (c.a >= n_reads || c.b >= n_reads || c.a == c.b || c.type == 0 || c.type > 3) {
        rowcnt[i] = 0;
        atomicAdd(n_bad, 1u);
        return;
    }
    rowcnt[i] = (uint8_t)rows_of(c.type, c.a, c.b, paired);
}

__global__ __launch_bounds__(256) void k_emit_cands(const Cand* __restrict__ cands, const uint8_t* __restrict__ rowcnt,
                                                    const uint32_t* __restrict__ row_off, uint32_t n,
                                                    const uint32_t* __restrict__ len, Row* __restrict__ rows,
                                                    uint32_t bits, uint32_t paired,
                                                    unsigned long long* __restrict__ counters) {
    uint64_t nver = 0, suml = 0, sumb = 0, sume = 0;
    for (uint32_t i = blockIdx.x * blockDim.x + threadIdx.x; i < n; i += gridDim.x * blockDim.x) {
        if (rowcnt[i] == 0) continue;
        const Cand c = cands[i];
        nver += 1;
        write_rows(rows, row_off[i], c.type, c.a, c.p, c.b, len[c.a], len[c.b], bits, paired, suml, sumb, sume);
    }
    flush_counters(nver, suml, sumb, sume, counters);
}

__global__ __launch_bounds__(256) void k_paired_check(const uint64_t* __restrict__ words, const uint64_t* __restrict__ woff,
                                                      const uint32_t* __restrict__ len, uint32_t n_pairs,
                                                      const uint8_t* __restrict__ pair_state,
                                                      uint32_t* __restrict__ n_bad) {
    const uint32_t pair = (blockIdx.x * blockDim.x + threadIdx.x) >> 6;
    if (pair >= n_pairs) return;
    const uint32_t lane = lane_id();
    const uint32_t L = len[2 * pair];
    bool bad = false;
    const uint32_t hs = pair_state ? pair_state[pair] : 0u;
    if (hs != 0) {
        bad = hs == 2;
    } else if (len[2 * pair + 1] != L) {
        bad = true;
    } else {
        const uint64_t* __restrict__ R = words + woff[2 * pair];
        const uint64_t* __restrict__ S = words + woff[2 * pair + 1];
        const uint32_t nw = (L + 31) / 32;
        for (uint32_t w = lane; w < nw && !bad; w += WAVE) {
            const int64_t o = (int64_t)L - 32 * (int64_t)w - 32;
            uint64_t x;
            uint32_t valid = 32;
            if (o >= 0) {
                x = funnel(R[o >> 5], R[(o >> 5) + 1], (uint32_t)(o & 31) * 2);
            } else {
                valid = (uint32_t)(32 + o);
                x = R[0] << ((uint32_t)(-o) * 2);
            }
            uint64_t y = __brevll(x);
            y = ((y >> 1) & 0x5555555555555555ull) | ((y & 0x5555555555555555ull) << 1);
            y = ~y;
            const uint64_t mask = valid >= 32 ? ~0ull : ((1ull << (valid * 2)) - 1ull);
            bad = ((y ^ S[w]) & mask) != 0;
        }
    }
    if (__any(bad) && lane == 0) atomicAdd(n_bad, 1u);
}

__global__ __launch_bounds__(256) void k_revcomp_store(uint64_t* __restrict__ words, const uint64_t* __restrict__ woff,
                                                       const uint32_t* __restrict__ len, uint32_t pair0, uint32_t n_pairs,
                                                       const uint32_t* __restrict__ exc_off, const uint32_t* __restrict__ exc_pos) {
    const uint32_t pair = pair0 + ((blockIdx.x * blockDim.x + threadIdx.x) >> 6);
    if (pair >= n_pairs) return;
    const uint32_t e0 = exc_off ? exc_off[2 * pair + 1] : 0u, e1 = exc_off ? exc_off[2 * pair + 2] : 0u;
    const uint32_t lane = lane_id();
    const uint32_t L = len[2 * pair];
    const uint64_t* __restrict__ R = words + woff[2 * pair];
    uint64_t* __restrict__ S = words + woff[2 * pair + 1];
    const uint32_t nw = (L + 31) / 32;
    const uint32_t last = nw + (uint32_t)((woff[2 * pair + 1] + nw + 1) & 1ull);
    for (uint32_t w = lane; w <= last; w += WAVE) {
        uint64_t out = 0;
        if (w < nw) {
            const int64_t o = (int64_t)L - 32 * (int64_t)w - 32;
            uint64_t x;
            uint32_t valid = 32;
            if (o >= 0) {
                x = funnel(R[o >> 5], R[(o >> 5) + 1], (uint32_t)(o & 31) * 2);
            } else {
                valid = (uint32_t)(32 + o);
                x = R[0] << ((uint32_t)(-o) * 2);
            }
            uint64_t y = __brevll(x);
            y = ((y >> 1) & 0x5555555555555555ull) | ((y & 0x5555555555555555ull) << 1);
            y = ~y;
            out = valid >= 32 ? y : (y & ((1ull << (valid * 2)) - 1ull));
            for (uint32_t e = e0; e < e1; ++e) {
                const uint32_t pos = exc_pos[e];
                if ((pos >> 5) == w) out &= ~(3ull << ((pos & 31u) * 2u));
            }
        }
        S[w] = out;
    }
}

__global__ void k_scatter_first(uint64_t* __restrict__ words, const uint64_t* __restrict__ woff,
                                const ulonglong2* __restrict__ first, uint32_t r0, uint32_t n) {
    const uint32_t r = r0 + blockIdx.x * blockDim.x + threadIdx.x;
    if (r >= n) return;
    const ulonglong2 f = first[r];
    *reinterpret_cast<ulonglong2*>(words + woff[r]) = f;
}

__global__ void k_scatter_lead(uint64_t* __restrict__ words, const uint64_t* __restrict__ woff, const uint32_t* __restrict__ len,
                               const uint64_t* __restrict__ lead, uint32_t nw, uint32_t r0, uint32_t n) {
    const uint64_t t = (uint64_t)blockIdx.x * blockDim.x + threadIdx.x;
    const uint64_t r = r0 + t / nw;
    const uint32_t k = (uint32_t)(t % nw);
    if (r >= n) return;
    const uint32_t own = (len[r] + 31u) / 32u + 1u;
    if (k < own) words[woff[r] + k] = lead[r * nw + k];
}

__global__ void k_defer_split(const uint32_t* __restrict__ cand_a, const uint32_t* __restrict__ cand_p,
                              const uint32_t* __restrict__ cand_b, uint32_t n_cand, uint32_t b_limit, Cand* __restrict__ out,
                              uint32_t cap, uint32_t* __restrict__ counter, const CandGuard G) {
    const uint32_t i = blockIdx.x * blockDim.x + threadIdx.x;
    if (G.n_dev) {
        if (G.overflow()) return;
        n_cand = (uint32_t)*G.n_dev;
    }
    if (i >= n_cand) return;
    const uint32_t b = cand_b[i];
    if (b < b_limit) return;
    const uint32_t k = atomicAdd(counter, 1u);
// ... 656 lines not shown
```

Before: 1.560 billion.

## Move host expansion pool to header with per-thread sums and fused sort-permute

Moves the host-side record expansion thread pool into its own header and reworks it. Overlap sums are now accumulated per thread instead of through shared atomics, helpers get indices and claim arrays, and sleeping helpers are woken only when needed. Separately, the GPU read sort kernel can write the permutation directly for small read ranges, which removes the separate rank buffer and invert kernel. A debug entry point for multi-piece expansion is added. The pool synchronisation is now more complex and harder to get right.

```diff
diff --git a/include/phasm_overlap.h b/include/phasm_overlap.h
--- a/include/phasm_overlap.h
+++ b/include/phasm_overlap.h
@@ -368,6 +368,8 @@
                             po_row* rows_out, uint64_t n_rows_expected);
 int po_debug_expand_packed(const uint64_t* records, uint64_t n, uint32_t sh_b, uint32_t sh_p, const uint32_t* lengths, uint32_t n_reads,
                            uint32_t paired, po_row* rows_out, uint64_t n_rows_expected);
+int po_debug_expand_pieces(const void* records, const uint64_t* rec_begin, uint32_t n_pieces, uint32_t sh_b, uint32_t sh_p,
+                           const uint32_t* lengths, uint32_t n_reads, uint32_t paired, po_row* rows_out, const uint64_t* row_begin);
 int po_debug_fault_backtrace(int fd);
 int po_debug_pointer_info(const void* p, int32_t* hip_type, int32_t* hsa_type, uint64_t* base, uint64_t* bytes);
 
diff --git a/phasm_amd/_lib.py b/phasm_amd/_lib.py
--- a/phasm_amd/_lib.py
+++ b/phasm_amd/_lib.py
@@ -261,6 +261,8 @@
     ("po_debug_store_words", ctypes.c_uint64, [_P, ctypes.c_int, ctypes.POINTER(ctypes.c_void_p)]),
     ("po_debug_expand_packed", ctypes.c_int, [ctypes.c_void_p, ctypes.c_uint64, ctypes.c_uint32, ctypes.c_uint32, ctypes.c_void_p, ctypes.c_uint32,
                                               ctypes.c_uint32, ctypes.c_void_p, ctypes.c_uint64]),
+    ("po_debug_expand_pieces", ctypes.c_int, [ctypes.c_void_p, ctypes.c_void_p, ctypes.c_uint32, ctypes.c_uint32, ctypes.c_uint32, ctypes.c_void_p,
+                                              ctypes.c_uint32, ctypes.c_uint32, ctypes.c_void_p, ctypes.c_void_p]),
     ("po_debug_expand_records", ctypes.c_int, [ctypes.c_void_p, ctypes.c_uint64, ctypes.c_void_p, ctypes.c_uint32, ctypes.c_uint32,
                                                ctypes.c_void_p, ctypes.c_uint64]),
     ("po_debug_host_ranges", ctypes.c_uint64, [ctypes.POINTER(ctypes.c_uint64), ctypes.c_uint64]),
diff --git a/phasm_amd/csrc/c_api.hip b/phasm_amd/csrc/c_api.hip
--- a/phasm_amd/csrc/c_api.hip
+++ b/phasm_amd/csrc/c_api.hip
@@ -31,6 +31,7 @@
 #include <vector>
 
 #include "kernels.hip.h"
+#include "home_pool.h"
 #include "extend.hip.h"
 #include "layout.hip.h"
 #include "reduce.hip.h"
@@ -588,283 +589,7 @@
 }
 
 
-unsigned cpu_share() {
-    static const unsigned share = [] {
-        unsigned n = std::thread::hardware_concurrency();
-        n = n ? n : 4u;
-        long long q = -1, per = 100000;
-        if (FILE* f = std::fopen("/sys/fs/cgroup/cpu.max", "r")) {
-            char buf[64] = {0};
-            if (std::fscanf(f, "%63s %lld", buf, &per) >= 1 && std::strcmp(buf, "max") != 0) q = atoll(buf);
-            std::fclose(f);
-        } else if (FILE* g = std::fopen("/sys/fs/cgroup/cpu/cpu.cfs_quota_us", "r")) {
-            if (std::fscanf(g, "%lld", &q) != 1) q = -1;
-            std::fclose(g);
-            if (FILE* g2 = std::fopen("/sys/fs/cgroup/cpu/cpu.cfs_period_us", "r")) {
-                if (std::fscanf(g2, "%lld", &per) != 1) per = 100000;
-                std::fclose(g2);
-            }
-        }
-        if (q > 0 && per > 0) n = std::min<unsigned>(n, (unsigned)std::max<long long>(1, q / per));
-        return n;
-    }();
-    return share;
-}
-
-namespace home {
-
-constexpr uint32_t CHUNK = 4096;
-
-struct Job {
-    const void* rec = nullptr;
-    uint32_t sh_b = 0, sh_p = 0;
-    uint64_t n_rec = 0;
-    po_row* out = nullptr;
-    uint64_t n_rows = 0;
-    const volatile uint32_t* flag = nullptr;
-    uint32_t want = 0;
-    uint32_t paired = 0, bits = 2;
-};
-
-struct Pool {
-    std::vector<std::thread> thr;
-    std::mutex mu;
-    std::condition_variable cv_queue;
-    std::condition_variable cv_job;
-    std::mutex call_mu;
-    std::deque<Job> queue;
-    std::atomic<uint64_t> submitted{0}, finished{0};
-    std::atomic<int> error{0};
-    const uint32_t* len = nullptr;
-    uint32_t n_reads = 0;
-    std::atomic<uint64_t> sum_l{0}, sum_b{0}, sum_e{0};
-    Job cur;
-    uint64_t job_seq = 0;
-    uint32_t n_chunks = 0;
-    std::vector<uint64_t> chunk_off;
-    std::atomic<uint32_t> next_count{0}, done_count{0}, next_write{0}, done_write{0};
-    std::atomic<int> phase{0};
-    std::atomic<int> inside{0};
-    std::chrono::steady_clock::time_point t0;
-    std::vector<std::array<double, 3>> trace;
-    bool tracing = false;
-};
-
-Pool* g_pool = nullptr;
-std::once_flag g_pool_once;
-
-inline void cpu_pause() {
-#if defined(__x86_64__) || defined(__i386__)
-    __builtin_ia32_pause();
-#endif
-}
-
-std::atomic<uint32_t> g_spin_limit{4096};
-template <class Pred>
-inline void spin_until(Pred pred) {
-    const uint32_t limit = g_spin_limit.load(std::memory_order_relaxed);
-    for (uint32_t n = 0; !pred(); ++n) {
-        if (limit == 0 || n < limit) cpu_pause();
-        else std::this_thread::yield();
-    }
-}
-
-inline po::Cand load_rec(const Job& j, uint64_t i) {
-    if (!j.sh_b) return static_cast<const po::Cand*>(j.rec)[i];
-    return po::unpack_record(static_cast<const uint64_t*>(j.rec)[i], j.sh_b, j.sh_p);
-}
-
-inline uint32_t rows_of_rec(const po::Cand& c, uint32_t paired) {
-    if (!paired) return (c.type & 1u) + ((c.type >> 1) & 1u);
-    return ((c.type & 1u) ? (c.a == (c.b ^ 1u) ? 1u : 2u) : 0u) + ((c.type & 2u) ? 2u : 0u);
-}
-
-inline void put_row(uint64_t*& o, uint32_t a, uint32_t b, uint32_t astart, uint32_t aend, uint32_t bend) {
-    __builtin_nontemporal_store((uint64_t)a | ((uint64_t)b << 32), o);
-    __builtin_nontemporal_store((uint64_t)astart | ((uint64_t)aend << 32), o + 1);
-    __builtin_nontemporal_store((uint64_t)bend << 32, o + 2);
-    o += 3;
-}
-
-bool expand_records(Pool& P, uint64_t lo, uint64_t hi, po_row* out) {
-    uint64_t* o = reinterpret_cast<uint64_t*>(out);
-    const Job& job = P.cur;
-    const uint32_t* len = P.len;
-    const uint32_t paired = job.paired, n_reads = P.n_reads, bits = job.bits;
-    auto pb = [bits](uint32_t l) -> uint64_t { return bits == 8u ? l : (l >> 2) + ((l & 3u) != 0u); };
-    uint64_t sl = 0, sb = 0, se = 0;
-    for (uint64_t i = lo; i < hi; ++i) {
-        const po::Cand c = load_rec(job, i);
-        if (c.a >= n_reads || c.b >= n_reads) return false;
-        const uint32_t la = len[c.a], lb = len[c.b];
-        se += 2 * pb((c.type & 1u) ? la - c.p : lb);
-        if (c.type & 1u) {
-            const uint32_t l = la - c.p;
-            const bool twin = paired && c.a != (c.b ^ 1u);
-            put_row(o, c.a, c.b, c.p, la, l);
-            if (twin) put_row(o, c.b ^ 1u, c.a ^ 1u, lb - l, lb, l);
-            const uint64_t k = twin ? 2 : 1;
-            sl += k * l;
-            sb += k * 2 * pb(l);
-        }
-        if (c.type & 2u) {
-            put_row(o, c.a, c.b, c.p, c.p + lb, lb);
-            if (paired) put_row(o, c.a ^ 1u, c.b ^ 1u, la - c.p - lb, la - c.p, lb);
-            const uint64_t k = paired ? 2 : 1;
-            sl += k * lb;
-            sb += k * 2 * pb(lb);
-        }
-    }
-    P.sum_l.fetch_add(sl, std::memory_order_relaxed);
-    P.sum_b.fetch_add(sb, std::memory_order_relaxed);
-    P.sum_e.fetch_add(se, std::memory_order_relaxed);
-    return true;
-}
-
-void run_phases(Pool& P, bool lead) {
-    const uint32_t nc = P.n_chunks;
-    for (;;) {
-        const uint32_t c = P.next_count.fetch_add(1, std::memory_order_relaxed);
-        if (c >= nc) break;
-        const uint64_t lo = (uint64_t)c * CHUNK, hi = std::min<uint64_t>(P.cur.n_rec, lo + CHUNK);
-        uint64_t n = 0;
-        const uint32_t paired = P.cur.paired;
-        for (uint64_t i = lo; i < hi; ++i) n += rows_of_rec(load_rec(P.cur, i), paired);
-        P.chunk_off[c + 1] = n;
-        P.done_count.fetch_add(1, std::memory_order_release);
-    }
-    if (lead) {
-        spin_until([&] { return P.done_count.load(std::memory_order_acquire) >= nc; });
-        P.chunk_off[0] = 0;
-        for (uint32_t c = 0; c < nc; ++c) P.chunk_off[c + 1] += P.chunk_off[c];
-        if (P.chunk_off[nc] != P.cur.n_rows) P.error.store(1);
-        P.phase.store(P.error.load() ? 0 : 2, std::memory_order_release);
-    } else {
-        spin_until([&] { return P.phase.load(std::memory_order_acquire) != 1; });
-    }
-    if (P.phase.load(std::memory_order_acquire) != 2) return;
-    for (;;) {
-        const uint32_t c = P.next_write.fetch_add(1, std::memory_order_relaxed);
-        if (c >= nc) break;
-        const uint64_t lo = (uint64_t)c * CHUNK, hi = std::min<uint64_t>(P.cur.n_rec, lo + CHUNK);
-        if (!expand_records(P, lo, hi, P.cur.out + P.chunk_off[c])) P.error.store(2);
-#if defined(__x86_64__)
-        __builtin_ia32_sfence();
-#endif
-        P.done_write.fetch_add(1, std::memory_order_release);
-    }
-}
-
-void helper(Pool* Pp) {
-    Pool& P = *Pp;
-    uint64_t seen = 0;
-    for (;;) {
-        {
-            std::unique_lock<std::mutex> lock(P.mu);
-            P.cv_job.wait(lock, [&] { return P.job_seq != seen; });
-            seen = P.job_seq;
-        }
-        P.inside.fetch_add(1, std::memory_order_acq_rel);
-        if (P.phase.load(std::memory_order_acquire) != 0) run_phases(P, false);
-        P.inside.fetch_sub(1, std::memory_order_release);
-    }
-}
-
-void leader(Pool* Pp) {
-    Pool& P = *Pp;
-    for (;;) {
-        Job j;
-        {
-            std::unique_lock<std::mutex> lock(P.mu);
-            P.cv_queue.wait(lock, [&] { return !P.queue.empty(); });
-            j = P.queue.front();
-            P.queue.pop_front();
-        }
-        if (j.flag)
-            spin_until([&] { return *j.flag == j.want; });
-        std::atomic_thread_fence(std::memory_order_acquire);
-        const double t_ready = P.tracing ? std::chrono::duration<double, std::micro>(std::chrono::steady_clock::now() - P.t0).count() : 0.0;
-        if (P.error.load() == 0 && j.n_rec) {
-            spin_until([&] { return P.inside.load(std::memory_order_acquire) == 0; });
-            P.cur = j;
-            P.n_chunks = (uint32_t)((j.n_rec + CHUNK - 1) / CHUNK);
-            if (P.chunk_off.size() < (size_t)P.n_chunks + 1) P.chunk_off.resize((size_t)P.n_chunks + 1);
-            P.next_count.store(0);
-            P.done_count.store(0);
-            P.next_write.store(0);
-            P.done_write.store(0);
-            P.phase.store(1, std::memory_order_release);
-            {
-                std::lock_guard<std::mutex> lock(P.mu);
-                ++P.job_seq;
-            }
-            P.cv_job.notify_all();
-            run_phases(P, true);
-            if (P.phase.load() == 2)
-                spin_until([&] { return P.done_write.load(std::memory_order_acquire) >= P.n_chunks; });
-            P.phase.store(0, std::memory_order_release);
-            std::atomic_thread_fence(std::memory_order_seq_cst);
-        }
-        if (P.tracing)
-            P.trace.push_back({t_ready, std::chrono::duration<double, std::micro>(std::chrono::steady_clock::now() - P.t0).count(), (double)j.n_rows});
-        P.finished.fetch_add(1, std::memory_order_release);
-    }
-}
-
-Pool* pool() {
-    std::call_once(g_pool_once, [] {
-        Pool* P = new Pool();
-        unsigned n = cpu_share();
-        n = std::max(1u, std::min(n * 3 / 4, 12u));
-        if (const char* e = getenv("PHASM_HOME_THREADS")) n = (unsigned)std::max(1, std::min(64, atoi(e)));
-        try {
-            P->thr.emplace_back(leader, P);
-            P->thr.back().detach();
-            for (unsigned i = 1; i < n; ++i) {
-                P->thr.emplace_back(helper, P);
-                P->thr.back().detach();
-            }
-        } catch (const std::system_error&) {
-        }
-        if (P->thr.empty()) {
-            delete P;
-            P = nullptr;
-        }
-        g_pool = P;
-    });
-    return g_pool;
-}
-
-void begin(Pool* P, const uint32_t* len, uint32_t n_reads, bool tracing) {
-    if (const char* e = getenv("PHASM_HOME_SPIN")) g_spin_limit.store((uint32_t)std::max(0, atoi(e)));
-    else g_spin_limit.store(4096);
-    P->len = len;
-    P->n_reads = n_reads;
-    P->error.store(0);
-    P->submitted.store(0);
-    P->finished.store(0);
-    P->sum_l.store(0);
-    P->sum_b.store(0);
-    P->sum_e.store(0);
-    P->tracing = tracing;
-    P->trace.clear();
-    P->t0 = std::chrono::steady_clock::now();
-}
-
-void submit(Pool* P, const Job& j) {
-    {
-        std::lock_guard<std::mutex> lock(P->mu);
-        P->queue.push_back(j);
-    }
-    P->submitted.fetch_add(1, std::memory_order_release);
-    P->cv_queue.notify_one();
-}
-
-void wait_all(Pool* P) {
-    spin_until([&] { return P->finished.load(std::memory_order_acquire) >= P->submitted.load(std::memory_order_acquire); });
-}
-
-}
+using home::cpu_share;
 
 po_status init_device(po_handle* h) {
     if (h->dev_ready) {
@@ -1855,7 +1580,8 @@
                       fits(h->d_rowcnt, cap) && fits(h->d_row_off, (cap + 1) * 4) &&
                       fits(h->spare_rows, h->home_on ? cap * sizeof(po::Cand) : worst * sizeof(po_row)) &&
                       (!order || (fits(h->d_vlabel, (uint64_t)(r_end - r_begin) * 4) && fits(h->d_vperm, (uint64_t)(r_end - r_begin) * 4) &&
-                                  fits(h->d_vrank, (uint64_t)(r_end - r_begin) * 4))) && h->dev_words < 0xFFFFFFF0ull;
+                                  ((r_end - r_begin) <= po::SORT_PERM_MAX || fits(h->d_vrank, (uint64_t)(r_end - r_begin) * 4)))) &&
+                      h->dev_words < 0xFFFFFFF0ull;
         cap_c = (uint32_t)cap;
     }
     volatile uint64_t* count_slot = async_count ? &h->pinned[zone + 8] : &h->pinned[1];
@@ -1993,7 +1719,7 @@
                         HIP_TRY(h, hipFuncSetAttribute(reinterpret_cast<const void*>(po::k_read_sort),
                                                        hipFuncAttributeMaxDynamicSharedMemorySize, (int)sort_lds));
                     hipLaunchKernelGGL(po::k_read_sort, dim3(1), dim3(po::SORT_BLOCK), sort_lds, st, h->d_vlabel.as<uint32_t>(), n_cand,
-                                       shift, n_bins, h->d_vrank.as<uint32_t>());
+                                       shift, n_bins, h->d_vrank.as<uint32_t>(), (uint32_t*)nullptr, 0u);
                     hipLaunchKernelGGL(po::k_read_invert, dim3(cdiv(n_cand, 256)), dim3(256), 0, st, h->d_vrank.as<uint32_t>(), n_cand, 0u,
                                        h->d_vperm.as<uint32_t>());
                     perm = h->d_vperm.as<uint32_t>();
@@ -2034,11 +1760,16 @@
                 if (sort_lds > 48 * 1024)
                     HIP_TRY(h, hipFuncSetAttribute(reinterpret_cast<const void*>(po::k_read_sort),
                                                    hipFuncAttributeMaxDynamicSharedMemorySize, (int)sort_lds));
-                PO_TRY(ensure(h, h->d_vrank, (size_t)n_a * 4));
-                hipLaunchKernelGGL(po::k_read_sort, dim3(1), dim3(po::SORT_BLOCK), sort_lds, st, h->d_vlabel.as<uint32_t>(), n_a,
-                                   shift, n_bins, h->d_vrank.as<uint32_t>());
-                hipLaunchKernelGGL(po::k_read_invert, dim3(cdiv(n_a, 256)), dim3(256), 0, st, h->d_vrank.as<uint32_t>(), n_a, r_begin,
-                                   h->d_vperm.as<uint32_t>());
+                if (n_a <= po::SORT_PERM_MAX) {
+                    hipLaunchKernelGGL(po::k_read_sort, dim3(1), dim3(po::SORT_BLOCK), sort_lds, st, h->d_vlabel.as<uint32_t>(), n_a,
+                                       shift, n_bins, (uint32_t*)nullptr, h->d_vperm.as<uint32_t>(), r_begin);
+                } else {
+                    PO_TRY(ensure(h, h->d_vrank, (size_t)n_a * 4));
+                    hipLaunchKernelGGL(po::k_read_sort, dim3(1), dim3(po::SORT_BLOCK), sort_lds, st, h->d_vlabel.as<uint32_t>(), n_a,
+                                       shift, n_bins, h->d_vrank.as<uint32_t>(), (uint32_t*)nullptr, 0u);
+                    hipLaunchKernelGGL(po::k_read_invert, dim3(cdiv(n_a, 256)), dim3(256), 0, st, h->d_vrank.as<uint32_t>(), n_a, r_begin,
+                                       h->d_vperm.as<uint32_t>());
+                }
                 perm = h->d_vperm.as<uint32_t>();
             }
             const uint32_t ver_grid = perm ? 8 * ((n_a + 7) / 8) : n_a;
@@ -4314,15 +4045,17 @@
     home::wait_all(P);
     const int err = P->error.load();
     if (sum) {
-        sum->sum_overlap_bases += P->sum_l.load();
-        sum->verify_bytes_algo += P->sum_b.load();
-        sum->verify_bytes_exec += P->sum_e.load();
+        const home::Sums t = home::sums(P);
+        sum->sum_overlap_bases += t.l;
+        sum->verify_bytes_algo += t.b;
+        sum->verify_bytes_exec += t.e;
     }
     if (P->tracing)
         for (size_t i = 0; i < P->trace.size(); ++i)
             std::fprintf(stderr, "[home] piece %zu: records home at %.3f ms, %.0f rows written at %.3f ms (since the call set the pool up)\n", i,
                          P->trace[i][0] * 1e-3, P->trace[i][2], P->trace[i][1] * 1e-3);
     h->home_on = false;
+    home::end(P);
     P->call_mu.unlock();
     return err;
 }
@@ -4785,11 +4518,7 @@
             } else if (st == PO_OK) {
                 overflowed = true;
                 home_wait(h);
-                if (h->home_on) {
-                    home::g_pool->sum_l.store(0);
-                    home::g_pool->sum_b.store(0);
-                    home::g_pool->sum_e.store(0);
-                }
+                if (h->home_on) home::reset_sums(home::g_pool);
                 if (hipStreamSynchronize(h->copy_stream) != hipSuccess) st = fail(h, PO_ERR_HIP, "copy stream");
                 R.total = 0;
                 sum = po_stats();
@@ -5671,17 +5400,7 @@
                             po_row* rows_out, uint64_t n_rows_expected) {
     home::Pool* P = home::pool();
     if (!P) return -1;
-    std::lock_guard<std::mutex> call(P->call_mu);
-    home::begin(P, lengths, n_reads, false);
-    home::Job j;
-    j.rec = records;
-    j.n_rec = n;
-    j.out = rows_out;
-    j.n_rows = n_rows_expected;
-    j.paired = paired ? 1u : 0u;
-    home::submit(P, j);
-    home::wait_all(P);
-    return P->error.load();
+    return home::expand_once(P, records, n, 0, 0, lengths, n_reads, paired, rows_out, n_rows_expected);
 }
 
 int po_debug_expand_packed(const uint64_t* records, uint64_t n, uint32_t sh_b, uint32_t sh_p, const uint32_t* lengths, uint32_t n_reads,
@@ -5689,19 +5408,15 @@
     if (!sh_b || sh_p < sh_b || sh_p >= 62) return -2;
     home::Pool* P = home::pool();
     if (!P) return -1;
-    std::lock_guard<std::mutex> call(P->call_mu);
-    home::begin(P, lengths, n_reads, false);
-    home::Job j;
-    j.rec = records;
-    j.sh_b = sh_b;
-    j.sh_p = sh_p;
-    j.n_rec = n;
-    j.out = rows_out;
-    j.n_rows = n_rows_expected;
-    j.paired = paired ? 1u : 0u;
-    home::submit(P, j);
-    home::wait_all(P);
-    return P->error.load();
+    return home::expand_once(P, records, n, sh_b, sh_p, lengths, n_reads, paired, rows_out, n_rows_expected);
+}
+
+int po_debug_expand_pieces(const void* records, const uint64_t* rec_begin, uint32_t n_pieces, uint32_t sh_b, uint32_t sh_p,
+                           const uint32_t* lengths, uint32_t n_reads, uint32_t paired, po_row* rows_out, const uint64_t* row_begin) {
+    if (sh_b && (sh_p < sh_b || sh_p >= 62)) return -2;
+    home::Pool* P = home::pool();
+    if (!P) return -1;
+    return home::expand_pieces(P, records, rec_begin, n_pieces, sh_b, sh_p, lengths, n_reads, paired, rows_out, row_begin);
 }
 
 static int g_fault_fd = 2;
diff --git a/phasm_amd/csrc/home_pool.h b/phasm_amd/csrc/home_pool.h
--- /dev/null
+++ b/phasm_amd/csrc/home_pool.h
@@ -0,0 +1,420 @@
+#pragma once
+
+#include "../../include/phasm_overlap.h"
+#include "record.h"
+
+#include <algorithm>
+#include <array>
+#include <atomic>
+#include <chrono>
+#include <condition_variable>
+#include <cstdint>
+#include <cstdio>
+#include <cstdlib>
+#include <cstring>
+#include <deque>
+#include <memory>
+#include <mutex>
+#include <system_error>
+#include <thread>
+#include <vector>
+
+namespace home {
+
+inline unsigned cpu_share() {
+    static const unsigned share = [] {
+        unsigned n = std::thread::hardware_concurrency();
+        n = n ? n : 4u;
+        long long q = -1, per = 100000;
+        if (FILE* f = std::fopen("/sys/fs/cgroup/cpu.max", "r")) {
+            char buf[64] = {0};
+            if (std::fscanf(f, "%63s %lld", buf, &per) >= 1 && std::strcmp(buf, "max") != 0) q = atoll(buf);
+            std::fclose(f);
+        } else if (FILE* g = std::fopen("/sys/fs/cgroup/cpu/cpu.cfs_quota_us", "r")) {
+            if (std::fscanf(g, "%lld", &q) != 1) q = -1;
+            std::fclose(g);
+            if (FILE* g2 = std::fopen("/sys/fs/cgroup/cpu/cpu.cfs_period_us", "r")) {
+                if (std::fscanf(g2, "%lld", &per) != 1) per = 100000;
+                std::fclose(g2);
+            }
+        }
+        if (q > 0 && per > 0) n = std::min<unsigned>(n, (unsigned)std::max<long long>(1, q / per));
+        return n;
+    }();
+    return share;
+}
+
+constexpr uint32_t CHUNK = 4096;
+constexpr unsigned MAX_THREADS = 64;
+
+constexpr int64_t HELPER_POLL_NS = 300 * 1000;
+
+struct Job {
+    const void* rec = nullptr;
+    uint32_t sh_b = 0, sh_p = 0;
+    uint64_t n_rec = 0;
+    po_row* out = nullptr;
+    uint64_t n_rows = 0;
+    const volatile uint32_t* flag = nullptr;
+    uint32_t want = 0;
+    uint32_t paired = 0, bits = 2;
+};
+
+struct alignas(64) Sums {
+    uint64_t l = 0, b = 0, e = 0;
+};
+
+struct Pool {
+    std::vector<std::thread> thr;
+    unsigned n_thr = 0;
+    std::mutex mu;
+    std::condition_variable cv_queue;
+    std::condition_variable cv_job;
+    std::mutex call_mu;
+    std::deque<Job> queue;
+    std::atomic<uint64_t> submitted{0}, finished{0};
+    std::atomic<int> error{0};
+    const uint32_t* len = nullptr;
+    uint32_t n_reads = 0;
+    Sums sums[MAX_THREADS];
+    Job cur;
+    alignas(64) std::atomic<uint64_t> job_seq{0};
+    std::atomic<bool> in_call{false};
+    alignas(64) int sleepers = 0;
+    uint32_t n_chunks = 0;
+    uint64_t gen = 0;
+    std::vector<uint64_t> chunk_off;
+    std::unique_ptr<std::atomic<uint64_t>[]> claim[2];
+    size_t claim_cap = 0;
+    std::atomic<uint32_t> next_count{0}, done_count{0}, next_write{0}, done_write{0};
+    std::atomic<int> phase{0};
+    std::atomic<int> inside{0};
+    std::chrono::steady_clock::time_point t0;
+    std::vector<std::array<double, 3>> trace;
+    bool tracing = false;
+};
+
+inline Pool* g_pool = nullptr;
+inline std::once_flag g_pool_once;
+
+inline void cpu_pause() {
+#if defined(__x86_64__) || defined(__i386__)
+    __builtin_ia32_pause();
+#endif
+}
+
+inline std::atomic<uint32_t> g_spin_limit{4096};
+template <class Pred>
+inline void spin_until(Pred pred) {
+    const uint32_t limit = g_spin_limit.load(std::memory_order_relaxed);
+    for (uint32_t n = 0; !pred(); ++n) {
+        if (limit == 0 || n < limit) cpu_pause();
+        else std::this_thread::yield();
+    }
+}
+
+inline po::Cand load_rec(const Job& j, uint64_t i) {
+    if (!j.sh_b) return static_cast<const po::Cand*>(j.rec)[i];
+    return po::unpack_record(static_cast<const uint64_t*>(j.rec)[i], j.sh_b, j.sh_p);
+}
+
+inline uint32_t rows_of_rec(const po::Cand& c, uint32_t paired) {
+    if (!paired) return (c.type & 1u) + ((c.type >> 1) & 1u);
+    return ((c.type & 1u) ? (c.a == (c.b ^ 1u) ? 1u : 2u) : 0u) + ((c.type & 2u) ? 2u : 0u);
+}
+
+inline void put_row(uint64_t*& o, uint32_t a, uint32_t b, uint32_t astart, uint32_t aend, uint32_t bend) {
+    __builtin_nontemporal_store((uint64_t)a | ((uint64_t)b << 32), o);
+    __builtin_nontemporal_store((uint64_t)astart | ((uint64_t)aend << 32), o + 1);
+    __builtin_nontemporal_store((uint64_t)bend << 32, o + 2);
+    o += 3;
+}
+
+inline bool expand_records(Pool& P, uint64_t lo, uint64_t hi, po_row* out, Sums& sums) {
+    uint64_t* o = reinterpret_cast<uint64_t*>(out);
+    const Job& job = P.cur;
+    const uint32_t* len = P.len;
+    const uint32_t paired = job.paired, n_reads = P.n_reads, bits = job.bits;
+    auto pb = [bits](uint32_t l) -> uint64_t { return bits == 8u ? l : (l >> 2) + ((l & 3u) != 0u); };
+    uint64_t sl = 0, sb = 0, se = 0;
+    for (uint64_t i = lo; i < hi; ++i) {
+        const po::Cand c = load_rec(job, i);
+        if (c.a >= n_reads || c.b >= n_reads) return false;
+        const uint32_t la = len[c.a], lb = len[c.b];
+        se += 2 * pb((c.type & 1u) ? la - c.p : lb);
+        if (c.type & 1u) {
+            const uint32_t l = la - c.p;
+            const bool twin = paired && c.a != (c.b ^ 1u);
+            put_row(o, c.a, c.b, c.p, la, l);
+            if (twin) put_row(o, c.b ^ 1u, c.a ^ 1u, lb - l, lb, l);
+            const uint64_t k = twin ? 2 : 1;
+            sl += k * l;
+            sb += k * 2 * pb(l);
+        }
+        if (c.type & 2u) {
+            put_row(o, c.a, c.b, c.p, c.p + lb, lb);
+            if (paired) put_row(o, c.a ^ 1u, c.b ^ 1u, la - c.p - lb, la - c.p, lb);
+            const uint64_t k = paired ? 2 : 1;
+            sl += k * lb;
+            sb += k * 2 * pb(lb);
+        }
+    }
+    sums.l += sl;
+    sums.b += sb;
+    sums.e += se;
+    return true;
+}
+
+struct ChunkWalk {
+    Pool& P;
+    std::atomic<uint64_t>* claim;
+    std::atomic<uint32_t>& shared;
+    const uint64_t gen;
+    const uint32_t nc, stride;
+    uint32_t own;
+    bool next(uint32_t& c) {
+        for (; own < nc; own += stride)
+            if (claim[own].exchange(gen, std::memory_order_relaxed) != gen) {
+                c = own;
+                own += stride;
+                return true;
+            }
+        for (;;) {
+            const uint32_t s = shared.fetch_add(1, std::memory_order_relaxed);
+            if (s >= nc) return false;
+            if (claim[s].exchange(gen, std::memory_order_relaxed) != gen) {
+                c = s;
+                return true;
+            }
+        }
+    }
+};
+
+inline void run_phases(Pool& P, unsigned me) {
+    const bool lead = me == 0;
+    const uint32_t nc = P.n_chunks;
+    const uint32_t stride = std::max(1u, P.n_thr);
+    const uint64_t gen = P.gen;
+    ChunkWalk count{P, P.claim[0].get(), P.next_count, gen, nc, stride, me};
+    for (uint32_t c; count.next(c);) {
+        const uint64_t lo = (uint64_t)c * CHUNK, hi = std::min<uint64_t>(P.cur.n_rec, lo + CHUNK);
+        uint64_t n = 0;
+        const uint32_t paired = P.cur.paired;
+        for (uint64_t i = lo; i < hi; ++i) n += rows_of_rec(load_rec(P.cur, i), paired);
+        P.chunk_off[c + 1] = n;
+        P.done_count.fetch_add(1, std::memory_order_release);
+    }
+    if (lead) {
+        spin_until([&] { return P.done_count.load(std::memory_order_acquire) >= nc; });
+        P.chunk_off[0] = 0;
+        for (uint32_t c = 0; c < nc; ++c) P.chunk_off[c + 1] += P.chunk_off[c];
+        if (P.chunk_off[nc] != P.cur.n_rows) P.error.store(1);
+        P.phase.store(P.error.load() ? 0 : 2, std::memory_order_release);
+    } else {
+        spin_until([&] { return P.phase.load(std::memory_order_acquire) != 1; });
+    }
+    if (P.phase.load(std::memory_order_acquire) != 2) return;
+    ChunkWalk write{P, P.claim[1].get(), P.next_write, gen, nc, stride, me};
+    for (uint32_t c; write.next(c);) {
+        const uint64_t lo = (uint64_t)c * CHUNK, hi = std::min<uint64_t>(P.cur.n_rec, lo + CHUNK);
+        if (!expand_records(P, lo, hi, P.cur.out + P.chunk_off[c], P.sums[me])) P.error.store(2);
+#if defined(__x86_64__)
+        __builtin_ia32_sfence();
+#endif
+        P.done_write.fetch_add(1, std::memory_order_release);
+    }
+}
+
+inline void helper(Pool* Pp, unsigned me) {
+    Pool& P = *Pp;
+    uint64_t seen = 0;
+    bool worked = false;
+    for (;;) {
+        bool have = false;
+        if (worked && P.in_call.load(std::memory_order_acquire)) {
+            const auto until = std::chrono::steady_clock::now() + std::chrono::nanoseconds(HELPER_POLL_NS);
+            uint32_t n = 0;
+            bool expired = false;
+            spin_until([&] {
+                if (P.job_seq.load(std::memory_order_acquire) != seen) return true;
+                if ((++n & 63u) == 0 && (!P.in_call.load(std::memory_order_acquire) || std::chrono::steady_clock::now() >= until)) expired = true;
+                return expired;
+            });
+            have = P.job_seq.load(std::memory_order_acquire) != seen;
+        }
+        if (!have) {
+            std::unique_lock<std::mutex> lock(P.mu);
+            ++P.sleepers;
+            P.cv_job.wait(lock, [&] { return P.job_seq.load(std::memory_order_relaxed) != seen; });
+            --P.sleepers;
+        }
+        seen = P.job_seq.load(std::memory_order_acquire);
+        P.inside.fetch_add(1, std::memory_order_acq_rel);
+        worked = P.phase.load(std::memory_order_acquire) != 0;
+        if (worked) run_phases(P, me);
+        P.inside.fetch_sub(1, std::memory_order_release);
+    }
+}
+
+inline void leader(Pool* Pp) {
+    Pool& P = *Pp;
+    for (;;) {
+        Job j;
+        {
+            std::unique_lock<std::mutex> lock(P.mu);
+            P.cv_queue.wait(lock, [&] { return !P.queue.empty(); });
+            j = P.queue.front();
+            P.queue.pop_front();
+        }
+        if (j.flag)
+            spin_until([&] { return *j.flag == j.want; });
+        std::atomic_thread_fence(std::memory_order_acquire);
+        const double t_ready = P.tracing ? std::chrono::duration<double, std::micro>(std::chrono::steady_clock::now() - P.t0).count() : 0.0;
+        if (P.error.load() == 0 && j.n_rec) {
+            spin_until([&] { return P.inside.load(std::memory_order_acquire) == 0; });
+            P.cur = j;
+            P.n_chunks = (uint32_t)((j.n_rec + CHUNK - 1) / CHUNK);
+            if (P.chunk_off.size() < (size_t)P.n_chunks + 1) P.chunk_off.resize((size_t)P.n_chunks + 1);
+            if (P.claim_cap < P.n_chunks) {
+                P.claim_cap = std::max<size_t>(2 * (size_t)P.n_chunks, 256);
+                for (auto& cl : P.claim) {
+                    cl.reset(new std::atomic<uint64_t>[P.claim_cap]);
+                    for (size_t c = 0; c < P.claim_cap; ++c) cl[c].store(0, std::memory_order_relaxed);
+                }
+            }
+            P.next_count.store(0);
+            P.done_count.store(0);
+            P.next_write.store(0);
+            P.done_write.store(0);
+            P.gen = P.job_seq.load(std::memory_order_relaxed) + 1;
+            bool wake;
+            {
+                std::lock_guard<std::mutex> lock(P.mu);
+                P.phase.store(1, std::memory_order_release);
+                P.job_seq.fetch_add(1, std::memory_order_release);
+                wake = P.sleepers > 0;
+            }
+            if (wake) P.cv_job.notify_all();
+            run_phases(P, 0);
+            if (P.phase.load() == 2)
+                spin_until([&] { return P.done_write.load(std::memory_order_acquire) >= P.n_chunks; });
+            P.phase.store(0, std::memory_order_release);
+            std::atomic_thread_fence(std::memory_order_seq_cst);
+        }
+        if (P.tracing)
+            P.trace.push_back({t_ready, std::chrono::duration<double, std::micro>(std::chrono::steady_clock::now() - P.t0).count(), (double)j.n_rows});
+        P.finished.fetch_add(1, std::memory_order_release);
+    }
+}
+
+inline Pool* pool() {
+    std::call_once(g_pool_once, [] {
+        Pool* P = new Pool();
+        unsigned n = cpu_share();
+        n = std::max(1u, std::min(n * 3 / 4, 12u));
+        if (const char* e = getenv("PHASM_HOME_THREADS")) n = (unsigned)std::max(1, std::min((int)MAX_THREADS, atoi(e)));
+        try {
+            P->thr.emplace_back(leader, P);
+            P->thr.back().detach();
+            for (unsigned i = 1; i < n; ++i) {
+                P->thr.emplace_back(helper, P, i);
+                P->thr.back().detach();
+            }
+        } catch (const std::system_error&) {
+        }
+        P->n_thr = (unsigned)P->thr.size();
+        if (P->thr.empty()) {
+            delete P;
+            P = nullptr;
+        }
+        g_pool = P;
+    });
+    return g_pool;
+}
+
+inline void reset_sums(Pool* P) {
+    for (Sums& s : P->sums) s = Sums();
+}
+
+inline Sums sums(const Pool* P) {
+    Sums t;
+    for (const Sums& s : P->sums) {
+        t.l += s.l;
+        t.b += s.b;
+        t.e += s.e;
+    }
+    return t;
+}
+
+inline void begin(Pool* P, const uint32_t* len, uint32_t n_reads, bool tracing) {
+    if (const char* e = getenv("PHASM_HOME_SPIN")) g_spin_limit.store((uint32_t)std::max(0, atoi(e)));
+    else g_spin_limit.store(4096);
+    P->len = len;
+    P->n_reads = n_reads;
+    P->error.store(0);
+    P->submitted.store(0);
+    P->finished.store(0);
+    reset_sums(P);
+    P->tracing = tracing;
+    P->trace.clear();
+    P->t0 = std::chrono::steady_clock::now();
+    P->in_call.store(true, std::memory_order_release);
+}
+
+inline void submit(Pool* P, const Job& j) {
+    {
+        std::lock_guard<std::mutex> lock(P->mu);
+        P->queue.push_back(j);
+    }
+    P->submitted.fetch_add(1, std::memory_order_release);
+    P->cv_queue.notify_one();
+}
+
+inline void wait_all(Pool* P) {
+    spin_until([&] { return P->finished.load(std::memory_order_acquire) >= P->submitted.load(std::memory_order_acquire); });
+}
+
+inline void end(Pool* P) {
+    P->in_call.store(false, std::memory_order_release);
+}
+
+inline int expand_once(Pool* P, const void* records, uint64_t n, uint32_t sh_b, uint32_t sh_p, const uint32_t* lengths, uint32_t n_reads,
+                       uint32_t paired, po_row* rows_out, uint64_t n_rows_expected) {
+    std::lock_guard<std::mutex> call(P->call_mu);
+    begin(P, lengths, n_reads, false);
+    Job j;
+    j.rec = records;
+    j.sh_b = sh_b;
+    j.sh_p = sh_p;
+    j.n_rec = n;
+    j.out = rows_out;
+    j.n_rows = n_rows_expected;
+    j.paired = paired ? 1u : 0u;
+    submit(P, j);
+    wait_all(P);
+    end(P);
+    return P->error.load();
+}
+
+inline int expand_pieces(Pool* P, const void* records, const uint64_t* rec_begin, uint32_t n_pieces, uint32_t sh_b, uint32_t sh_p,
+                         const uint32_t* lengths, uint32_t n_reads, uint32_t paired, po_row* rows_out, const uint64_t* row_begin) {
+    std::lock_guard<std::mutex> call(P->call_mu);
+    begin(P, lengths, n_reads, false);
+    const size_t elem = sh_b ? sizeof(uint64_t) : sizeof(po::Cand);
+    for (uint32_t k = 0; k < n_pieces; ++k) {
+        Job j;
+        j.rec = static_cast<const char*>(records) + rec_begin[k] * elem;
+        j.sh_b = sh_b;
+        j.sh_p = sh_p;
+        j.n_rec = rec_begin[k + 1] - rec_begin[k];
+        j.out = rows_out + row_begin[k];
+        j.n_rows = row_begin[k + 1] - row_begin[k];
+        j.paired = paired ? 1u : 0u;
+        submit(P, j);
+    }
+    wait_all(P);
+    end(P);
+    return P->error.load();
+}
+
+}
diff --git a/phasm_amd/csrc/kernels.hip.h b/phasm_amd/csrc/kernels.hip.h
--- a/phasm_amd/csrc/kernels.hip.h
+++ b/phasm_amd/csrc/kernels.hip.h
@@ -1,6 +1,8 @@
 #pragma once
 #include <hip/hip_runtime.h>
 #include <stdint.h>
+
+#include "record.h"
 
 namespace po {
 
@@ -1220,8 +1222,10 @@
 }
 
 constexpr int SORT_BLOCK = 1024;
+constexpr uint32_t SORT_PERM_MAX = 16384;
 __global__ __launch_bounds__(SORT_BLOCK) void k_read_sort(const uint32_t* __restrict__ label, uint32_t n_reads, uint32_t shift,
-                                                          uint32_t n_bins, uint32_t* __restrict__ rank) {
+                                                          uint32_t n_bins, uint32_t* __restrict__ rank, uint32_t* __restrict__ perm,
+                                                          uint32_t r_begin) {
     extern __shared__ uint32_t s_bin[];
     uint32_t* s_wave = s_bin + n_bins;
     const uint32_t tid = threadIdx.x;
@@ -1264,7 +1268,11 @@
         }
 #pragma unroll
         for (uint32_t k = 0; k < UN; ++k)
-            if (v[k] != ~0u) rank[base + k * SORT_BLOCK] = atomicAdd(&s_bin[v[k] >> shift], 1u);
+            if (v[k] != ~0u) {
+                const uint32_t r = atomicAdd(&s_bin[v[k] >> shift], 1u);
+                if (perm) perm[r] = r_begin + base + k * SORT_BLOCK;
+                else rank[base + k * SORT_BLOCK] = r;
+            }
     }
 }
 
@@ -1817,17 +1825,6 @@
     flush_counters(nver, suml, sumb, sume, counters);
 }
 
-struct Cand {
-    uint32_t a, p, b, type;
-};
-
-__host__ __device__ inline uint64_t pack_record(uint32_t a, uint32_t p, uint32_t b, uint32_t type, uint32_t sh_b, uint32_t sh_p) {
-    return (uint64_t)a | ((uint64_t)b << sh_b) | ((uint64_t)p << sh_p) | ((uint64_t)type << 62);
-}
-__host__ __device__ inline Cand unpack_record(uint64_t v, uint32_t sh_b, uint32_t sh_p) {
-    const uint64_t mr = (1ull << sh_b) - 1ull;
-    return Cand{(uint32_t)(v & mr), (uint32_t)((v >> sh_p) & ((1ull << (62u - sh_p)) - 1ull)), (uint32_t)((v >> sh_b) & mr), (uint32_t)(v >> 62)};
-}
 
 __global__ void k_compact(const uint32_t* __restrict__ cand_a, const uint32_t* __restrict__ cand_p,
                           const uint32_t* __restrict__ cand_b, const uint8_t* __restrict__ type,
diff --git a/phasm_amd/csrc/record.h b/phasm_amd/csrc/record.h
--- /dev/null
+++ b/phasm_amd/csrc/record.h
@@ -0,0 +1,25 @@
+#pragma once
+
+#include <cstdint>
+
+#if defined(__HIPCC__)
+#define PO_HOST_DEVICE __host__ __device__
+#else
+#define PO_HOST_DEVICE
+#endif
+
+namespace po {
+
+struct Cand {
+    uint32_t a, p, b, type;
+};
+
+PO_HOST_DEVICE inline uint64_t pack_record(uint32_t a, uint32_t p, uint32_t b, uint32_t type, uint32_t sh_b, uint32_t sh_p) {
+    return (uint64_t)a | ((uint64_t)b << sh_b) | ((uint64_t)p << sh_p) | ((uint64_t)type << 62);
+}
+PO_HOST_DEVICE inline Cand unpack_record(uint64_t v, uint32_t sh_b, uint32_t sh_p) {
+    const uint64_t mr = (1ull << sh_b) - 1ull;
+    return Cand{(uint32_t)(v & mr), (uint32_t)((v >> sh_p) & ((1ull << (62u - sh_p)) - 1ull)), (uint32_t)((v >> sh_b) & mr), (uint32_t)(v >> 62)};
+}
+
+}
```

Result: slower. 1.521 billion (-2.5%).
